# facebookresearch/seamless_communication

Hardware: AMD Instinct MI355X
Metric: S2ST utterances/sec (and real-time factor), seamlessM4T_v2_large, 10 s audio (higher is better)
Workload: dtype f32 activations x f16 weights, f32 accumulate

## Files before the change

include/seamless_hip_internal.h:

```cpp
#ifndef SEAMLESS_HIP_INTERNAL_H_
#define SEAMLESS_HIP_INTERNAL_H_

#include "seamless_hip.h"

#ifdef __cplusplus
extern "C" {
#endif

int sc_decoder_step_family(sc_model* m, int rows, int caller);

int sc_op_knob(const char* name, int dflt);

int sc_op_force_general_gemm(int on);
int sc_op_single_plane(int on);
int sc_op_layernorm(const float* d_x, const float* d_gamma, const float* d_beta, float* d_y, int32_t rows, int32_t C,
                    int32_t act);
int sc_op_linear(const float* d_x, const void* d_w_f16, const float* d_bias, const float* d_res, float* d_y,
                 int32_t M, int32_t N, int32_t K, int32_t act, float alpha, int32_t split, int32_t force_gemv);
int sc_op_skinny_linear(const float* d_x, const void* d_w_f16, const float* d_bias, const float* d_res, float* d_y,
                        int32_t M, int32_t N, int32_t K, int32_t act, float alpha);
int sc_op_skinny_res_ln(const float* d_in, const void* d_w_f16, const float* d_bias, float* d_x_inout,
                        const float* d_gamma, const float* d_beta, float* d_h, int32_t M, int32_t N, int32_t K,
                        int32_t splits);
int sc_op_skinny_argmax(const float* d_x, const void* d_w_f16, int32_t M, int32_t N, int32_t K, int32_t step,
                        int32_t min_step_for_eos, int32_t force_eos_step, int32_t pad_idx, int32_t eos_idx,
                        int32_t unk_idx, float unk_penalty, int32_t* d_idx, float* d_lprob);

int sc_op_dstep_res_ln(const float* d_in, const void* d_w_f16, const float* d_bias, float* d_x_inout, const float* d_gamma,
                       const float* d_beta, float* d_h, int32_t M, int32_t N, int32_t K, int32_t splits);
int sc_op_dstep_linear_planes(const float* d_x, const void* d_w_f16, const float* d_bias, float* d_y, int32_t M, int32_t N, int32_t K,
                              int32_t act);
int sc_op_dstep_argmax(const float* d_x, const void* d_w_f16, int32_t M, int32_t N, int32_t K, int32_t step,
                       int32_t min_step_for_eos, int32_t force_eos_step, int32_t pad_idx, int32_t eos_idx, int32_t unk_idx,
                       float unk_penalty, int32_t ntl, int32_t* d_idx, float* d_lprob);
int sc_op_dstep_attention(const float* d_proj, int32_t S, const float* d_bias, float* d_kcache, float* d_vcache, int32_t cap,
                          int32_t pos, const int32_t* d_lens, int32_t cross, int32_t nb, int32_t heads, float* d_out);
int sc_op_dstep3_gemv(int32_t mode, const float* d_x, const void* d_w_f16, const float* d_bias, const float* d_gamma,
                      const float* d_beta, const float* d_res, float* d_y, float* d_h, int32_t M, int32_t N, int32_t K, int32_t act,
                      int32_t rg, int32_t shape);
int sc_op_dstep3_argmax(const float* d_x, const void* d_w_f16, int32_t M, int32_t N, int32_t K, int32_t step,
                        int32_t min_step_for_eos, int32_t force_eos_step, int32_t pad_idx, int32_t eos_idx, int32_t unk_idx,
                        float unk_penalty, int32_t* d_idx, float* d_lprob);
int sc_op_chain_bench(int32_t kind, int32_t rows, int32_t n, int32_t reps, float* us_per_kernel);
int sc_op_conv1d(const float* d_x, const void* d_w_f16_packed, const float* d_bias, const float* d_res, float* d_y,
                 int32_t nb, int32_t t_in, int32_t cin, int32_t cout, int32_t k, int32_t stride, int32_t pad,
                 int32_t dil, const int32_t* d_in_lens, int32_t in_act, int32_t act);
int sc_op_pack_conv_weight(const void* d_w_f16, void* d_dst_f16, int32_t cout, int32_t cin, int32_t k);
int sc_op_conv_transpose1d(const float* d_x, const void* d_v_f16, const void* d_g_f16, const float* d_bias,
                           float* d_y, int32_t nb, int32_t t_in, int32_t cin, int32_t cout, int32_t k,
                           int32_t stride, int32_t pad, int32_t in_act);
int sc_op_linear_presplit(const float* d_x, const void* d_w_f16, const float* d_bias, const float* d_res, float* d_y,
                          void* d_yh_f16, void* d_yl_f16, int32_t M, int32_t N, int32_t K, int32_t act, float alpha);
int sc_op_linear_presplit_argmax(const float* d_x, const void* d_w_f16, const float* d_bias, int32_t* d_idx, int32_t M, int32_t N,
                                 int32_t K);
int sc_op_conv1d_presplit(const float* d_x, const void* d_w_f16_packed, const float* d_bias, const float* d_res, float* d_y,
                          void* d_yh_f16, void* d_yl_f16, int32_t nb, int32_t t, int32_t cin, int32_t cout, int32_t k, int32_t pad,
                          int32_t dil, const unsigned char* d_row_valid, int32_t act);
int sc_op_resblock_pair_ps(const float* d_x, const void* d_w1_packed, const float* d_b1, const void* d_w2_packed, const float* d_b2,
                           float* d_out, int32_t nb, int32_t T, int32_t C, int32_t k, int32_t dil);
int sc_op_resblock_pair(const float* d_x, const void* d_w1_packed, const float* d_b1, const void* d_w2_packed,
                        const float* d_b2, float* d_out, int32_t nb, int32_t T, int32_t C, int32_t k, int32_t dil,
                        float slope, const float* d_avg_a, const float* d_avg_b);
int sc_op_mrf_fused(const float* d_x, const void* const* d_w1_packed, const float* const* d_b1, const void* const* d_w2_packed,
                    const float* const* d_b2, float* d_out, int32_t nb, int32_t T, int32_t C, const int32_t* k, const int32_t* dil,
                    float slope);
int sc_op_attention(const float* d_q, const float* d_k, const float* d_v, float* d_out, int32_t nb, int32_t heads,
// ... 42 lines not shown
```

seamless_communication_amd/_lib.py:

```python
from __future__ import annotations

import ctypes as C
from pathlib import Path
from typing import Optional

import os

_VARIANT = os.environ.get("SC_LIB_VARIANT", "")
LIB_PATH = Path(__file__).resolve().parent / (f"libseamless_hip.{_VARIANT}.so" if _VARIANT else "libseamless_hip.so")

SC_ABI_VERSION = 10
SC_MAX_UPSAMPLES = 8
SC_MAX_RESBLOCK_KERNELS = 4
SC_MAX_RESBLOCK_DILATIONS = 4
SC_F16, SC_F32, SC_I32 = 0, 1, 2


class SeamlessHipError(RuntimeError):
    pass


class sc_tensor_desc(C.Structure):
    _fields_ = [
        ("name", C.c_char_p),
# ... 65 lines not shown


_P = C.c_void_p
_PI = C.POINTER(C.c_int32)

SIGNATURES = {
    "sc_last_error": (C.c_char_p, []),
    "sc_abi_version": (C.c_int, []),
    "sc_load": (_P, [C.POINTER(sc_tensor_desc), C.c_size_t, C.POINTER(sc_config), C.c_int]),
    "sc_fork": (_P, [_P]),
    "sc_free": (None, [_P]),
    "sc_synchronize": (C.c_int, [_P]),
    "sc_wait_stream": (C.c_int, [_P, _P]),
    "sc_decoder_step_family": (C.c_int, [_P, C.c_int, C.c_int]),
    "sc_set_nar_tables": (C.c_int, [_P, _i, _P, _P, _P, _P, _P]),
    "sc_fbank": (C.c_int, [_P, _P, _i, C.c_int64, _P, _i, _P, _i, _P]),
    "sc_fbank_rate": (C.c_int, [_P, _P, _i, C.c_int64, _P, _i, _i, _P, _i, _P]),
    "sc_fbank_frames": (_i, [C.c_int64, _i]),
    "sc_encoder_out_len": (_i, [_P, _i]),
    "sc_encode_speech": (C.c_int, [_P, _P, _i, _i, _P, _P, _P]),
    "sc_encode_text": (C.c_int, [_P, _P, C.c_int32, C.c_int32, _P, _P]),
    "sc_mma_begin": (C.c_int, [_P, _P, C.c_int32, C.c_int32]),
    "sc_mma_step": (C.c_int, [_P, _P, C.c_int32, _P, C.c_int32, _P, _P, _P]),
    "sc_text_max_len": (_i, [_P, C.POINTER(sc_gen_opts), _i]),
    "sc_generate_text": (C.c_int, [_P, _P, _i, _i, _P, C.POINTER(sc_gen_opts), _P, _i, _P, _P, _P, _P]),
    "sc_generate_text_banned": (C.c_int, [_P, _P, _i, _i, _P, C.POINTER(sc_gen_opts), _P, _i, _P, _P, _P, _P, _P, _P, _i]),
    "sc_generate_text_capture": (C.c_int, [_P, _P, _i, _i, _P, C.POINTER(sc_gen_opts), _P, _i, _P, _P, _P, _P, _P, _P]),
    "sc_decode_text": (C.c_int, [_P, _P, _i, _i, _P, _P, _i, _P]),
    "sc_engine_create": (_P, [_P, C.POINTER(sc_engine_opts)]),
    "sc_engine_free": (None, [_P]),
    "sc_engine_attach": (C.c_int, [_P, _P]),
    "sc_engine_expect": (C.c_int, [_P, _i]),
    "sc_engine_get_stats": (C.c_int, [_P, C.POINTER(sc_engine_stats), _i]),
    "sc_t2u_nar": (C.c_int, [_P, _P, _i, _i, _P, _P, C.c_float, _P, _PI, _PI]),
    "sc_get_units": (C.c_int, [_P, _P]),
    "sc_get_durations": (C.c_int, [_P, _P, _P, _P]),
    "sc_vocoder_hop": (_i, [_P]),
    "sc_vocode": (C.c_int, [_P, _P, _i, _i, _P, _P, _P]),
    "sc_vocode_ragged": (C.c_int, [_P, _P, _i, _i, _P, _P, _P, _P]),
    "sc_vocoder_durations": (C.c_int, [_P, _P, _i, _i, _P]),
    "sc_t2u_ar": (C.c_int, [_P, _P, _i, _i, _P, C.POINTER(sc_gen_opts), _P, _i, _P, _i, _P, _P]),
    "sc_t2u_ar_max_len": (_i, [_P, C.POINTER(sc_gen_opts), _i]),
    "sc_last_padding": (C.c_int, [_P, _P, _P, _P]),
    "sc_s2st": (C.c_int, [_P, _P, _i, _i, _P, C.POINTER(sc_gen_opts), _P, _i, C.c_float, _P, _P, _P, _i, _P, _P, _i, _P, _P, _P]),
    "sc_prof_enable": (C.c_int, [C.c_int]),
    "sc_prof_reset": (C.c_int, []),
    "sc_prof_report": (C.c_int64, [C.c_char_p, C.c_int64]),
    "sc_text_to_char_seqs": (C.c_int32, [C.c_int32, _P, _P, _P, _P, _P, C.c_int32, C.c_int32, C.c_int32, _P, C.c_int32, C.c_int32,
                                         _P, _P, C.c_int32, _P]),
    "sc_ngram_blocked_tokens": (C.c_int32, [_PI, C.c_int32, C.c_int32, _PI, C.c_int32]),
    "sc_banned_blocked_tokens": (C.c_int32, [_PI, C.c_int32, _PI, _PI, C.c_int32, _PI, C.c_int32]),
    "sc_op_knob": (C.c_int, [C.c_char_p, C.c_int]),
    "sc_op_force_general_gemm": (C.c_int, [C.c_int]),
    "sc_op_single_plane": (C.c_int, [C.c_int]),
    "sc_op_layernorm": (C.c_int, [_P, _P, _P, _P, _i, _i, _i]),
    "sc_op_linear": (C.c_int, [_P, _P, _P, _P, _P, _i, _i, _i, _i, C.c_float, _i, _i]),
    "sc_op_skinny_linear": (C.c_int, [_P, _P, _P, _P, _P, _i, _i, _i, _i, C.c_float]),
    "sc_op_skinny_res_ln": (C.c_int, [_P, _P, _P, _P, _P, _P, _P, _i, _i, _i, _i]),
    "sc_op_skinny_argmax": (C.c_int, [_P, _P, _i, _i, _i, _i, _i, _i, _i, _i, _i, C.c_float, _P, _P]),
    "sc_op_dstep_res_ln": (C.c_int, [_P, _P, _P, _P, _P, _P, _P, _i, _i, _i, _i]),
    "sc_op_dstep_linear_planes": (C.c_int, [_P, _P, _P, _P, _i, _i, _i, _i]),
    "sc_op_dstep_argmax": (C.c_int, [_P, _P, _i, _i, _i, _i, _i, _i, _i, _i, _i, C.c_float, _i, _P, _P]),
    "sc_op_resblock_pair_ps": (C.c_int, [_P, _P, _P, _P, _P, _P, _i, _i, _i, _i, _i]),
    "sc_op_glu_dwconv_ln": (C.c_int, [_P, _P, _P, _P, _i, _P, _P, _i, _i, _i, _i, _P, _i]),
    "sc_op_layernorm2": (C.c_int, [_P, _P, _P, _P, _P, _P, _P, _P, _i, _i, _i]),
    "sc_op_dstep3_gemv": (C.c_int, [_i, _P, _P, _P, _P, _P, _P, _P, _P, _i, _i, _i, _i, _i, _i]),
    "sc_op_dstep3_argmax": (C.c_int, [_P, _P, _i, _i, _i, _i, _i, _i, _i, _i, _i, C.c_float, _P, _P]),
    "sc_op_chain_bench": (C.c_int, [_i, _i, _i, _i, _P]),
    "sc_op_dstep_attention": (C.c_int, [_P, _i, _P, _P, _P, _i, _i, _P, _i, _i, _i, _P]),
    "sc_op_conv1d": (C.c_int, [_P, _P, _P, _P, _P, _i, _i, _i, _i, _i, _i, _i, _i, _P, _i, _i]),
    "sc_op_pack_conv_weight": (C.c_int, [_P, _P, _i, _i, _i]),
    "sc_op_conv_transpose1d": (C.c_int, [_P, _P, _P, _P, _P, _i, _i, _i, _i, _i, _i, _i, _i]),
    "sc_op_linear_presplit": (C.c_int, [_P, _P, _P, _P, _P, _P, _P, _i, _i, _i, _i, C.c_float]),
    "sc_op_linear_presplit_argmax": (C.c_int, [_P, _P, _P, _P, _i, _i, _i]),
    "sc_op_conv1d_presplit": (C.c_int, [_P, _P, _P, _P, _P, _P, _P, _i, _i, _i, _i, _i, _i, _i, _P, _i]),
    "sc_op_mrf_fused": (C.c_int, [_P, _P, _P, _P, _P, _P, _i, _i, _i, _P, _P, C.c_float]),
    "sc_op_resblock_pair": (C.c_int, [_P, _P, _P, _P, _P, _P, _i, _i, _i, _i, _i, C.c_float, _P, _P]),
    "sc_op_attention": (C.c_int, [_P, _P, _P, _P, _i, _i, _i, _i, C.c_int64, C.c_int64, C.c_int64, C.c_int64, _P, _i,
                                  _P, _i, _i]),
    "sc_op_attention_ex": (C.c_int, [_P, _P, _P, _P, _i, _i, _i, _i, C.c_int64, C.c_int64, C.c_int64, C.c_int64, _P, _i,
                                     _P, _i, _i, _P, _P, C.c_int64, _P, _P, _P, _P, C.c_int64]),
    "sc_op_glu_dwconv": (C.c_int, [_P, _P, _P, _i, _i, _i, _i, _P]),
    "sc_op_argmax": (C.c_int, [_P, _i, _i, _P, _P]),
    "sc_op_beam_candidates": (C.c_int, [_P, C.c_int64, _i, _i, _i, _P, _i, _i, _i, _i, _i, _i, C.c_float, _i, _P, _P, _P, _i, _i, _i,
                                        _P, _P, _i]),
    "sc_op_beam_candidates_banned": (C.c_int, [_P, C.c_int64, _i, _i, _i, _P, _i, _i, _i, _i, _i, _i, C.c_float, _i, _P, _P, _P, _i, _i,
                                               _i, _P, _P, _i, _P, _P, _i]),
    "sc_op_beam_select": (C.c_int, [_P, _P, _P, _P, _P, _P, _P, _P, _P, _P, _P, _P, _P, _P, _i, _P, _P, _i, _i, _i, _i, _i, _i, _i, _i,
                                    _i, C.c_float]),
    "sc_op_beam_compact": (C.c_int, [_P, _P, _P, _P, _P, _P, _P, _P, _P, _i, _i, _i, _i, _i, _i]),
    "sc_op_gather_cache": (C.c_int, [_P, _P, _P, _i, _i, _i, _i, _i, C.c_int64]),
    "sc_op_row_token_lprob": (C.c_int, [_P, C.c_int64, _i, _i, _i, _i, _P]),
}

_lib: Optional[C.CDLL] = None


def load_library() -> C.CDLL:
    global _lib
    if _lib is not None:
        return _lib
    if not LIB_PATH.exists():
        raise SeamlessHipError(
            f"{LIB_PATH} is missing: build it with `python -m seamless_communication_amd.build` "
            "(there is no CPU fallback for the HIP path)"
        )
# ... 79 lines not shown
```

seamless_communication_amd/csrc/api.hip:

```cpp
#include <atomic>
#include <cstring>
#include <map>
#include <mutex>
#include <set>

#include "../../include/seamless_hip_internal.h"
#include "engine.h"
#include "model.h"

using namespace sc;

struct sc_model {
    Model m;
};

struct sc_engine {
    std::unique_ptr<Engine> e;
    int device = 0;
    const void* weights = nullptr;
    std::set<sc_model*> attached;
};

static std::mutex g_attach_mu;
static std::map<Engine*, sc_engine*> g_engine_owner;
// ... 496 lines not shown
                 "sc_text_to_char_seqs: null argument");
        return text_to_char_seqs_host(vocab, h_tok_len, h_starts_space, h_is_punct, h_char_offsets, h_char_ids, pad_idx, unk_idx,
                                      eos_idx, h_text_seqs, n, s_text, h_char_lens, h_out_char_ids, cap, h_char_seq_lens);
    } catch (const sc::Error& e) {
        return e.code;
    } catch (const std::exception& e) {
        sc::set_error("unexpected C++ exception: %s", e.what());
        return SC_ERR_INTERNAL;
    }
}

int32_t sc_ngram_blocked_tokens(const int32_t* h_seq, int32_t len, int32_t ngram_size, int32_t* h_out, int32_t cap) {
    try {
        SC_CHECK(len >= 0 && ngram_size >= 1 && cap >= 0 && (h_seq || len == 0) && (h_out || cap == 0),
                 "sc_ngram_blocked_tokens: bad argument");
        std::vector<int32_t> out;
        sc::ngram_blocked_tokens(h_seq, len, ngram_size, out);
        for (size_t i = 0; i < out.size() && i < (size_t)cap; ++i) h_out[i] = out[i];
        return (int32_t)out.size();
    } catch (const sc::Error& e) {
        return e.code;
    } catch (const std::exception& e) {
        sc::set_error("unexpected C++ exception: %s", e.what());
        return SC_ERR_INTERNAL;
    }
}

int32_t sc_banned_blocked_tokens(const int32_t* h_seq, int32_t len, const int32_t* h_banned_tokens, const int32_t* h_banned_offsets,
                                 int32_t n_banned, int32_t* h_out, int32_t cap) {
    try {
        SC_CHECK(len >= 0 && cap >= 0 && (h_seq || len == 0) && (h_out || cap == 0), "sc_banned_blocked_tokens: bad argument");
        sc::validate_banned_host(h_banned_tokens, h_banned_offsets, n_banned, -1, nullptr);
        sc::BannedHost b;
        b.tokens = h_banned_tokens, b.offsets = h_banned_offsets, b.n = n_banned;
        std::vector<int32_t> out;
        sc::banned_blocked_tokens(h_seq, len, b, out);
        for (size_t i = 0; i < out.size() && i < (size_t)cap; ++i) h_out[i] = out[i];
        return (int32_t)out.size();
    } catch (const sc::Error& e) {
        return e.code;
    } catch (const std::exception& e) {
        sc::set_error("unexpected C++ exception: %s", e.what());
        return SC_ERR_INTERNAL;
    }
}

int sc_op_knob(const char* name, int dflt) { return sc::knob::known(name) ? sc::knob::value(name, dflt) : dflt; }

static std::atomic<int> g_op_single{0};
int sc_op_single_plane(int on) {
    g_op_single.store(on ? 1 : 0);
    return SC_OK;
}

int sc_op_force_general_gemm(int on) {
    sc::g_force_general_gemm.store(on ? 1 : 0);
    return SC_OK;
}

int sc_op_layernorm(const float* d_x, const float* d_gamma, const float* d_beta, float* d_y, int32_t rows, int32_t C,
                    int32_t act) {
    SC_API_BEGIN
    launch_layernorm(d_x, C, d_gamma, d_beta, d_y, C, rows, C, act, nullptr, 1, g_op_stream);
    SC_HIP(hipStreamSynchronize(g_op_stream));
    SC_API_END
}

int sc_op_linear(const float* d_x, const void* d_w_f16, const float* d_bias, const float* d_res, float* d_y, int32_t M,
                 int32_t N, int32_t K, int32_t act, float alpha, int32_t split, int32_t force_gemv) {
    SC_API_BEGIN
    if (force_gemv) {
        launch_gemv(d_x, K, static_cast<const __half*>(d_w_f16), K, d_bias, d_res, N, d_y, N, M, N, K, act, alpha, g_op_stream);
    } else {
        GemmArgs a;
        a.A = d_x;
        a.lda = K;
        a.W = static_cast<const __half*>(d_w_f16);
        a.ldw = K;
        a.bias = d_bias;
        a.res = d_res;
        a.ldr = N;
        a.C = d_y;
        a.ldc = N;
        a.M = M;
        a.N = N;
        a.K = K;
        a.rows_per_batch = M;
        a.t_in = M;
        a.t_out = M;
        a.taps = 1;
        a.cin = K;
        a.act = act;
        a.alpha = alpha;
        a.split = split;
        launch_gemm(a, g_op_stream);
    }
    SC_HIP(hipStreamSynchronize(g_op_stream));
    SC_API_END
}

int sc_op_skinny_linear(const float* d_x, const void* d_w_f16, const float* d_bias, const float* d_res, float* d_y,
                        int32_t M, int32_t N, int32_t K, int32_t act, float alpha) {
    SC_API_BEGIN
    SkinnyArgs a;
    a.A = d_x;
    a.lda = K;
// ... 919 lines not shown
```

seamless_communication_amd/csrc/common.cpp:

```cpp
#include "common.h"
#include <cstdlib>
#include <cstring>

namespace sc {

static thread_local char g_err[1024] = "";

void set_error(const char* fmt, ...) {
    va_list ap;
    va_start(ap, fmt);
    vsnprintf(g_err, sizeof(g_err), fmt, ap);
    va_end(ap);
}

const char* get_error() { return g_err; }

namespace knob {
namespace {
struct Knob {
    const char* name;
    int kind;
    const char* what;
};
const Knob knob_table[] = {
    {"SC_DEBUG_NUMERICS", 0, "honour the switches that change results"},
    {"SC_DEBUG_FILL", 0, "fill fresh scratch blocks with NaN (tests)"},
    {"SC_SPLIT_MODE", 1, "1: Conformer products on the hi fp16 plane only (precision study)"},
    {"SC_DECODER_GEN1", 1, "decoder step on the first-generation kernels"},
    {"SC_DECODER_GEN2", 1, "decoder step on the second-generation chain"},
    {"SC_DECODE_STEPWISE", 1, "teacher-forced pass step by step instead of one batched forward"},
    {"SC_VOC_SPLIT", 1, "vocoder ResBlock products on both fp16 planes of their activations again (bit 0 wide stages, bit 2 narrow stages); default: hi plane only"},
    {"SC_GEMM_GENERAL", 0, "general GEMM kernel instead of the fast path"}, {"SC_GEMM_PF2", 0, "GEMM prefetch depth"},
    {"SC_GEMM_GROUP_M", 0, "GEMM workgroup order"}, {"SC_GEMM_TILE", 0, "GEMM tile override"},
    {"SC_PS_TILE", 0, "DMA GEMM: largest tile"}, {"SC_PS_MIN256", 0, "DMA GEMM: tiles needed for 256 x 256"},
    {"SC_PS_MIN128", 0, "DMA GEMM: tiles needed for 128 x 128"},
    {"SC_PRESPLIT", 0, "0: Conformer operands split on the fly"}, {"SC_ENC_FUSE", 0, "0: separate Conformer element-wise launches"},
    {"SC_D3_RG_SMALL", 0, "decoder step: rows per row group, N = 1024 products"}, {"SC_D3_RG_FFN", 0, "decoder step: rows per row group, FFN-in"},
    {"SC_G3_STATIONARY", 0, "row-group products of wide steps: 0 one workgroup per row group, n = workgroup budget of the weight-stationary launch"},
    {"SC_G3_TILES", 0, "0: FFN-out of wide steps on the weight-stationary row-group walk instead of tile-owning waves"},
    {"SC_G3_TOUCH", 0, "weight-stationary products: bit 0 cooperative L2 touch of the activations, bit 1 K slices per XCD (FFN-out); default 3"},
    {"SC_D3_FFN_IN", 0, "decoder step: FFN-in workgroup shape"}, {"SC_D3_FFN_OUT", 0, "decoder step: FFN-out workgroup shape"},
    {"SC_T2U_GROUPS", 0, "NAR T2U: length buckets"}, {"SC_T2U_PACKED", 0, "0: NAR decoder on padded buckets"},
    {"SC_VOC_PS", 0, "0: vocoder wide stages on the register-staged convolution"}, {"SC_VOC_MRF", 0, "0: narrow vocoder stages as nine pair launches"},
    {"SC_VOC_GROUPS", 0, "vocoder: length buckets"}, {"SC_VOC_GROUP_OVERHEAD", 0, "vocoder: bucket planning overhead rows"},
    {"SC_VOC_STREAMS", 0, "vocoder: side chains"},
    {"SC_ENGINE_RG_SMALL", 0, "decode engine: rows per row group, N = 1024 products"},
    {"SC_BEAM_COMPACT", 2, "0: beam search keeps finished utterances' slots"},
    {"SC_GREEDY_COMPACT", 2, "0: greedy generation keeps finished rows in their slots"}, {"SC_GREEDY_POLL", 2, "steps between looks at the finished flags"},
};
constexpr int N_KNOBS = sizeof(knob_table) / sizeof(knob_table[0]);
struct State {
    bool set[N_KNOBS];
    int val[N_KNOBS];
    bool numerics = false;
};
const State& state() {
    static const State st = [] {
        State s{};
        const char* dn = getenv("SC_DEBUG_NUMERICS");
        s.numerics = dn && atoi(dn) != 0;
        for (int i = 0; i < N_KNOBS; ++i) {
            const char* e = getenv(knob_table[i].name);
            s.set[i] = e != nullptr && (knob_table[i].kind != 1 || s.numerics);
            s.val[i] = e ? atoi(e) : 0;
        }
        return s;
    }();
    return st;
}
int lookup(const char* name) {
    for (int i = 0; i < N_KNOBS; ++i)
        if (strcmp(knob_table[i].name, name) == 0) return i;
    return -1;
}
int find(const char* name) {
    const int i = lookup(name);
    if (i >= 0) return i;
    fprintf(stderr, "libseamless_hip: switch %s is not in the knob table (common.cpp)\n", name);
    abort();
}
}

bool known(const char* name) { return name && lookup(name) >= 0; }

int value(const char* name, int dflt) {
    const int i = find(name);
    return state().set[i] ? state().val[i] : dflt;
}
bool is_set(const char* name) { return state().set[find(name)]; }
int live(const char* name, int dflt) {
    (void)find(name);
    const char* e = getenv(name);
    return e ? atoi(e) : dflt;
}
void report_once() {
    static const bool done = [] {
        const State& s = state();
        for (int i = 0; i < N_KNOBS; ++i) {
// ... 16 lines not shown
```

seamless_communication_amd/csrc/k_gemm.hip:

```cpp
#include <atomic>
#include <cstdlib>

#include "kernels.h"

namespace sc {

std::atomic<int> g_force_general_gemm{0};

typedef _Float16 half8_t __attribute__((ext_vector_type(8)));
typedef _Float16 half4_t __attribute__((ext_vector_type(4)));
typedef float float16_t __attribute__((ext_vector_type(16)));

static constexpr int BK = 32;
static constexpr int LDS_LD = 40;

__device__ __forceinline__ float apply_act(float v, int act) {
    if (act == ACT_RELU) return v > 0.f ? v : 0.f;
    if (act == ACT_SILU) return v / (1.f + expf(-v));
    if (act == ACT_TANH) return tanhf(v);
    return v;
}

__device__ __forceinline__ float apply_in_act(float v, int in_act) {
    if (in_act == IN_LRELU_01) return v > 0.f ? v : 0.1f * v;
    if (in_act == IN_LRELU_001) return v > 0.f ? v : 0.01f * v;
    return v;
}

template <int BM, int BN, int WGM, int WGN, int AMODE, bool SPLIT>
__global__ __launch_bounds__(256) void gemm_kernel(GemmArgs p) {
    static_assert(WGM * WGN == 4, "4 waves per block");
    constexpr int WM = BM / WGM, WN = BN / WGN;
    constexpr int TM = WM / 32, TN = WN / 32;
    static_assert(TM >= 1 && TN >= 1, "wave tile must hold a 32x32 fragment");
    constexpr int A_IT = BM / 32;
    constexpr int B_IT = (BN * 4 + 255) / 256;

    __shared__ __attribute__((aligned(16))) _Float16 sAh[BM * LDS_LD];
    __shared__ __attribute__((aligned(16))) _Float16 sAl[SPLIT ? BM * LDS_LD : 8];
    __shared__ __attribute__((aligned(16))) _Float16 sB[BN * LDS_LD];

    const int tid = threadIdx.x;
    const int lane = tid & 63;
    const int wave = tid >> 6;
    const int wm = wave / WGN, wn = wave % WGN;
    const int m0 = blockIdx.y * BM;
    const int n0 = blockIdx.x * BN;
    const int phase = blockIdx.z;
    const __half* __restrict__ W = p.W + (int64_t)phase * p.w_phase_stride;
    const int out_off = p.out_off + phase * p.out_off_phase_step;

    const int a_kq = tid & 7;
    const int a_r = tid >> 3;
    int a_n[A_IT], a_q[A_IT], a_len[A_IT];
#pragma unroll
    for (int i = 0; i < A_IT; ++i) {
        const int m = m0 + a_r + 32 * i;
        if (m < p.M) {
            const int n = m / p.rows_per_batch;
            a_n[i] = n;
            a_q[i] = m - n * p.rows_per_batch;
            a_len[i] = p.in_lens ? min(p.in_lens[n], p.t_in) : p.t_in;
        } else {
            a_n[i] = 0;
            a_q[i] = 0;
            a_len[i] = -1;
        }
    }
    const int b_r = tid >> 2;
    const int b_kc = tid & 3;

    float4 a_reg[A_IT];
    uint4 b_reg[B_IT];

    auto load_tile = [&](int k0) {
        if (AMODE == 1) {
            const int tap = k0 / p.cin;
            const int c0 = k0 - tap * p.cin + a_kq * 4;
            const bool tap_ok = tap < p.taps;
#pragma unroll
            for (int i = 0; i < A_IT; ++i) {
                const int src_t = a_q[i] * p.stride + tap * p.dil - p.pad;
                float4 v = make_float4(0.f, 0.f, 0.f, 0.f);
                if (tap_ok && src_t >= 0 && src_t < a_len[i]) {
                    v = *reinterpret_cast<const float4*>(
                        p.A + ((int64_t)a_n[i] * p.t_in + src_t) * p.lda + c0);
                }
                a_reg[i] = v;
            }
        } else if (AMODE == 2) {
            const int kk = k0 + a_kq * 4;
            const int tap = kk / p.cin;
            const int c0 = kk - tap * p.cin;
            const bool tap_ok = tap < p.taps;
#pragma unroll
            for (int i = 0; i < A_IT; ++i) {
                const int src_t = a_q[i] * p.stride + tap * p.dil - p.pad;
                float4 v = make_float4(0.f, 0.f, 0.f, 0.f);
                if (tap_ok && src_t >= 0 && src_t < a_len[i]) {
                    v = *reinterpret_cast<const float4*>(
                        p.A + ((int64_t)a_n[i] * p.t_in + src_t) * p.lda + c0);
                }
                a_reg[i] = v;
            }
        } else {
#pragma unroll
            for (int i = 0; i < A_IT; ++i) {
                float e[4];
#pragma unroll
                for (int j = 0; j < 4; ++j) {
                    const int kk = k0 + a_kq * 4 + j;
                    const int tap = kk / p.cin;
                    const int c = kk - tap * p.cin;
                    const int src_t = a_q[i] * p.stride + tap * p.dil - p.pad;
                    float v = 0.f;
                    if (tap < p.taps && src_t >= 0 && src_t < a_len[i]) {
                        v = p.A[((int64_t)a_n[i] * p.t_in + src_t) * p.lda + c];
                    }
                    e[j] = v;
                }
                a_reg[i] = make_float4(e[0], e[1], e[2], e[3]);
            }
        }
#pragma unroll
        for (int i = 0; i < B_IT; ++i) {
            const int row = b_r + 64 * i;
            uint4 v = make_uint4(0u, 0u, 0u, 0u);
            if (row < BN && n0 + row < p.N) {
                v = *reinterpret_cast<const uint4*>(W + (int64_t)(n0 + row) * p.ldw + k0 + b_kc * 8);
            }
            b_reg[i] = v;
        }
    };

    auto store_tile = [&]() {
#pragma unroll
        for (int i = 0; i < A_IT; ++i) {
            float x[4] = {a_reg[i].x, a_reg[i].y, a_reg[i].z, a_reg[i].w};
            half4_t hi, lo;
#pragma unroll
            for (int j = 0; j < 4; ++j) {
                const float v = apply_in_act(x[j], p.in_act);
                const _Float16 h = (_Float16)v;
                hi[j] = h;
                lo[j] = (_Float16)(v - (float)h);
            }
            const int off = (a_r + 32 * i) * LDS_LD + a_kq * 4;
            *reinterpret_cast<half4_t*>(&sAh[off]) = hi;
            if (SPLIT) *reinterpret_cast<half4_t*>(&sAl[off]) = lo;
        }
#pragma unroll
        for (int i = 0; i < B_IT; ++i) {
            const int row = b_r + 64 * i;
            if (row < BN) *reinterpret_cast<uint4*>(&sB[row * LDS_LD + b_kc * 8]) = b_reg[i];
        }
    };

    float16_t acc[TM][TN];
#pragma unroll
    for (int i = 0; i < TM; ++i)
#pragma unroll
        for (int j = 0; j < TN; ++j)
#pragma unroll
            for (int r = 0; r < 16; ++r) acc[i][j][r] = 0.f;

    const int frag_row = lane & 31;
    const int frag_k = (lane >> 5) * 8;

    load_tile(0);
    for (int k0 = 0; k0 < p.K; k0 += BK) {
        store_tile();
        __syncthreads();
        if (k0 + BK < p.K) load_tile(k0 + BK);
#pragma unroll
        for (int kb = 0; kb < BK; kb += 16) {
            half8_t ah[TM], al[TM], bf[TN];
#pragma unroll
            for (int i = 0; i < TM; ++i) {
                const int off = (wm * WM + i * 32 + frag_row) * LDS_LD + kb + frag_k;
                ah[i] = *reinterpret_cast<const half8_t*>(&sAh[off]);
                if (SPLIT) al[i] = *reinterpret_cast<const half8_t*>(&sAl[off]);
            }
#pragma unroll
            for (int j = 0; j < TN; ++j) {
                const int off = (wn * WN + j * 32 + frag_row) * LDS_LD + kb + frag_k;
                bf[j] = *reinterpret_cast<const half8_t*>(&sB[off]);
            }
#pragma unroll
            for (int i = 0; i < TM; ++i)
#pragma unroll
                for (int j = 0; j < TN; ++j) {
                    acc[i][j] = __builtin_amdgcn_mfma_f32_32x32x16_f16(ah[i], bf[j], acc[i][j], 0, 0, 0);
                    if (SPLIT)
                        acc[i][j] = __builtin_amdgcn_mfma_f32_32x32x16_f16(al[i], bf[j], acc[i][j], 0, 0, 0);
                }
        }
        __syncthreads();
    }

    const bool plain_rows = (p.rows_per_batch == p.M) && p.out_mul == 1 && out_off == 0 && p.t_out == p.M;
#pragma unroll
    for (int i = 0; i < TM; ++i) {
#pragma unroll
        for (int r = 0; r < 16; ++r) {
            const int m = m0 + wm * WM + i * 32 + (r & 3) + 8 * (r >> 2) + 4 * (lane >> 5);
            if (m >= p.M) continue;
            int64_t row;
            if (plain_rows) {
                row = m;
            } else {
                const int n = m / p.rows_per_batch;
                const int q = m - n * p.rows_per_batch;
                const int dst_t = q * p.out_mul + out_off;
                if (dst_t < 0 || dst_t >= p.t_out) continue;
                row = (int64_t)n * p.t_out + dst_t;
            }
#pragma unroll
            for (int j = 0; j < TN; ++j) {
                const int col = n0 + wn * WN + j * 32 + (lane & 31);
                if (col >= p.N) continue;
                float v = acc[i][j][r];
                if (p.bias) v += p.bias[col];
                v = apply_act(v, p.act) * p.alpha;
                if (p.res) v += p.res[row * p.ldr + col];
                p.C[row * p.ldc + col] = v;
            }
        }
    }
}

template <int BM, int BN, int WGM, int WGN>
static void launch_cfg(const GemmArgs& a, hipStream_t s) {
    dim3 grid(cdiv(a.N, BN), cdiv(a.M, BM), a.phases);
    const bool vec_ok = (a.lda % 4 == 0) && ((reinterpret_cast<uintptr_t>(a.A) & 15) == 0);
    const int amode = (vec_ok && a.cin % 32 == 0) ? 1 : (vec_ok && a.cin % 4 == 0) ? 2 : 0;
    char name[64];
    snprintf(name, sizeof(name), "gemm_%dx%d_%s_%s", BM, BN, amode == 1 ? "vecA" : amode == 2 ? "vec4A" : "genA",
             a.split ? "split" : "f16");
    const double kreal = (double)a.taps * a.cin;
    const double flops = a.algo_flops > 0 ? a.algo_flops : 2.0 * a.M * a.N * kreal * a.phases;
    const double bytes = 4.0 * a.M * (double)a.cin * (a.stride < a.taps ? 1.0 : (double)a.taps) +
                         2.0 * a.N * (double)a.K * a.phases + 4.0 * a.M * (double)a.N * (a.res ? 2.0 : 1.0);
    prof::Scope scope(name, flops, bytes, s);
#define SC_GEMM_LAUNCH(AM, SP) hipLaunchKernelGGL((gemm_kernel<BM, BN, WGM, WGN, AM, SP>), grid, dim3(256), 0, s, a)
    if (a.split) {
        if (amode == 1) SC_GEMM_LAUNCH(1, true);
        else if (amode == 2) SC_GEMM_LAUNCH(2, true);
        else SC_GEMM_LAUNCH(0, true);
    } else {
        if (amode == 1) SC_GEMM_LAUNCH(1, false);
        else if (amode == 2) SC_GEMM_LAUNCH(2, false);
        else SC_GEMM_LAUNCH(0, false);
    }
#undef SC_GEMM_LAUNCH
}

void launch_gemm(const GemmArgs& a, hipStream_t s) {
    SC_CHECK(a.K % BK == 0, "gemm: K=%d must be a multiple of %d", a.K, BK);
    SC_CHECK(a.ldw % 8 == 0, "gemm: ldw=%lld must be a multiple of 8", (long long)a.ldw);
    SC_CHECK(a.M > 0 && a.N > 0, "gemm: empty problem M=%d N=%d", a.M, a.N);
    SC_CHECK(a.rows_per_batch > 0 && a.cin > 0, "gemm: rows_per_batch/cin unset");
    static const bool env_general = knob::is_set("SC_GEMM_GENERAL");
// ... 99 lines not shown
```

seamless_communication_amd/csrc/k_gemm2.hip:

```cpp
#include <algorithm>
#include <cstdlib>

#include "kernels.h"

namespace sc {

typedef _Float16 half8_t __attribute__((ext_vector_type(8)));
typedef _Float16 half4_t __attribute__((ext_vector_type(4)));
typedef float float16_t __attribute__((ext_vector_type(16)));
typedef float f32x4_t __attribute__((ext_vector_type(4)));
typedef unsigned int u32x4_t __attribute__((ext_vector_type(4)));

namespace {

constexpr int GEMM_GROUP_M_DEFAULT = 1;
constexpr int GEMM_PF2_DEFAULT = 1;
constexpr int FBK = 32;
constexpr int FLD = 40;

template <int ACT>
__device__ __forceinline__ float act_fn(float v) {
    if (ACT == ACT_RELU) return v > 0.f ? v : 0.f;
    if (ACT == ACT_SILU) return v / (1.f + expf(-v));
    if (ACT == ACT_TANH) return tanhf(v);
    return v;
}

template <int TM, int TN, int WM, int WN, int ACT, bool HAS_RES>
__device__ __forceinline__ void epilogue(const GemmArgs& p, float16_t (&acc)[TM][TN], int m0w, int n0w, int lane,
                                         int out_off, bool plain_rows) {
    float bcol[TN];
    int col[TN];
#pragma unroll
    for (int j = 0; j < TN; ++j) {
        col[j] = n0w + j * 32 + (lane & 31);
        bcol[j] = (p.bias && col[j] < p.N) ? p.bias[col[j]] : 0.f;
    }
#pragma unroll
    for (int i = 0; i < TM; ++i) {
#pragma unroll
        for (int r = 0; r < 16; ++r) {
            const int m = m0w + i * 32 + (r & 3) + 8 * (r >> 2) + 4 * (lane >> 5);
            if (m >= p.M) continue;
            int64_t row;
            if (plain_rows) {
                row = m;
            } else {
                const int n = m / p.rows_per_batch;
                const int q = m - n * p.rows_per_batch;
                const int dst_t = q * p.out_mul + out_off;
                if (dst_t < 0 || dst_t >= p.t_out) continue;
                row = (int64_t)n * p.t_out + dst_t;
            }
#pragma unroll
            for (int j = 0; j < TN; ++j) {
                if (col[j] >= p.N) continue;
                float v = act_fn<ACT>(acc[i][j][r] + bcol[j]) * p.alpha;
                if (HAS_RES) v += p.res[row * p.ldr + col[j]];
                p.C[row * p.ldc + col[j]] = v;
            }
        }
    }
}

template <int TM, int TN, int WN, int EP_LD, int ACT, bool HAS_RES>
__device__ __forceinline__ void epilogue_lds(const GemmArgs& p, float16_t (&acc)[TM][TN], float* ep, int m0w, int n0w, int lane,
                                             int out_off, bool plain_rows) {
    constexpr int LPR = WN / 4;
    constexpr int RPG = 16 / LPR;
    constexpr int RPI = 4 * RPG;
    const int l5 = lane & 31;
    const bool g1 = (l5 >= 4 && l5 < 12) || (l5 >= 16 && l5 < 20) || l5 >= 28;
    const int rank = g1 ? (l5 < 12 ? l5 - 4 : l5 < 20 ? l5 - 8 : l5 - 16) : (l5 < 4 ? l5 : l5 < 16 ? l5 - 8 : l5 - 12);
    const int grp = (lane >> 5) * 2 + (g1 ? 1 : 0);
    const int row_in = grp * RPG + rank / LPR;
    const int c0 = (rank % LPR) * 4;
    const int col = n0w + c0;
    const bool vec_ok = (col + 3 < p.N) && (p.ldc % 4 == 0) && (!HAS_RES || p.ldr % 4 == 0) &&
                        ((reinterpret_cast<uintptr_t>(p.C) | (HAS_RES ? reinterpret_cast<uintptr_t>(p.res) : 0)) & 15) == 0;
    f32x4_t b4 = {0.f, 0.f, 0.f, 0.f};
    if (p.bias) {
#pragma unroll
        for (int e = 0; e < 4; ++e) b4[e] = (col + e < p.N) ? p.bias[col + e] : 0.f;
    }
#pragma unroll
    for (int i = 0; i < TM; ++i) {
#pragma unroll
        for (int j = 0; j < TN; ++j)
#pragma unroll
            for (int r = 0; r < 16; ++r) ep[((r & 3) + 8 * (r >> 2) + 4 * (lane >> 5)) * EP_LD + j * 32 + (lane & 31)] = acc[i][j][r];
#pragma unroll
        for (int it = 0; it < 32 / RPI; ++it) {
            const int rr = it * RPI + row_in;
            const int m = m0w + i * 32 + rr;
            const f32x4_t a = *reinterpret_cast<const f32x4_t*>(ep + rr * EP_LD + c0);
            if (m >= p.M || col >= p.N) continue;
            int64_t row;
            if (plain_rows) {
                row = m;
            } else {
                const int n = m / p.rows_per_batch;
                const int q = m - n * p.rows_per_batch;
                const int dst_t = q * p.out_mul + out_off;
                if (dst_t < 0 || dst_t >= p.t_out) continue;
                row = (int64_t)n * p.t_out + dst_t;
            }
            f32x4_t v;
#pragma unroll
            for (int e = 0; e < 4; ++e) v[e] = act_fn<ACT>(a[e] + b4[e]) * p.alpha;
            if (vec_ok) {
                if (HAS_RES) v += *reinterpret_cast<const f32x4_t*>(p.res + row * p.ldr + col);
                *reinterpret_cast<f32x4_t*>(p.C + row * p.ldc + col) = v;
            } else {
#pragma unroll
                for (int e = 0; e < 4; ++e) {
                    if (col + e >= p.N) continue;
                    float x = v[e];
                    if (HAS_RES) x += p.res[row * p.ldr + col + e];
                    p.C[row * p.ldc + col + e] = x;
                }
            }
        }
    }
}

template <int BM, int BN, int WGM, int WGN, bool IN_ACT, bool CONV>
__global__ __launch_bounds__(256) void gemm_fast_kernel(GemmArgs p, int tiles_n, int tiles_mn, int tiles_total,
                                                        int tiles_per_xcd, float in_slope, int group_m) {
    static_assert(WGM * WGN == 4, "4 waves per block");
    constexpr int WM = BM / WGM, WN = BN / WGN;
    constexpr int TM = WM / 32, TN = WN / 32;
    static_assert(TM >= 1 && TN >= 1, "wave tile must hold a 32x32 fragment");
    constexpr int A_IT = BM / 32;
    constexpr int B_IT = (BN * 4 + 255) / 256;

    __shared__ __attribute__((aligned(16))) _Float16 sAh[2][BM * FLD];
    __shared__ __attribute__((aligned(16))) _Float16 sAl[2][BM * FLD];
    __shared__ __attribute__((aligned(16))) _Float16 sB[2][BN * FLD];

    const int bid = blockIdx.x;
    const int tile = (bid & 7) * tiles_per_xcd + (bid >> 3);
    if (tile >= tiles_total) return;
    const int phase = tile / tiles_mn;
    const int rem = tile - phase * tiles_mn;
    int tm, tn;
    {
        const int per_group = group_m * tiles_n;
        const int g = rem / per_group;
        const int in_g = rem - g * per_group;
        const int tiles_m = tiles_mn / tiles_n;
        const int gm = min(group_m, tiles_m - g * group_m);
        tn = in_g / gm;
        tm = g * group_m + (in_g - tn * gm);
    }

    const int tid = threadIdx.x;
    const int lane = tid & 63;
    const int wave = tid >> 6;
    const int wm = wave / WGN, wn = wave % WGN;
    const int m0 = tm * BM;
    const int n0 = tn * BN;
    const __half* __restrict__ W = p.W + (int64_t)phase * p.w_phase_stride;
    const int out_off = p.out_off + phase * p.out_off_phase_step;

    const int a_kq = tid & 7;
    const int a_r = tid >> 3;
    const float* a_base[A_IT];
    int a_t0[A_IT], a_len[A_IT];
#pragma unroll
    for (int i = 0; i < A_IT; ++i) {
        const int m = m0 + a_r + 32 * i;
        if (m < p.M) {
            const int n = m / p.rows_per_batch;
            const int q = m - n * p.rows_per_batch;
            a_base[i] = p.A + (int64_t)n * p.t_in * p.lda + a_kq * 4;
            a_t0[i] = q * p.stride - p.pad;
            a_len[i] = p.in_lens ? min(p.in_lens[n], p.t_in) : p.t_in;
        } else {
            a_base[i] = p.A + a_kq * 4;
            a_t0[i] = 0;
            a_len[i] = 0;
        }
    }
    const int b_r = tid >> 2;
    const int b_kc = tid & 3;
    const __half* b_ptr[B_IT];
#pragma unroll
    for (int i = 0; i < B_IT; ++i) {
        const int row = min(n0 + b_r + 64 * i, p.N - 1);
        b_ptr[i] = W + (int64_t)row * p.ldw + b_kc * 8;
    }

    const float* a_ptr[A_IT];
    bool a_ok[A_IT];
    auto set_tap = [&](int tap) {
#pragma unroll
        for (int i = 0; i < A_IT; ++i) {
            const int src_t = a_t0[i] + tap * p.dil;
            a_ok[i] = src_t >= 0 && src_t < a_len[i];
            a_ptr[i] = a_base[i] + (int64_t)(a_ok[i] ? src_t : 0) * p.lda;
        }
    };

    f32x4_t a_reg[A_IT];
    u32x4_t b_reg[B_IT];
    constexpr bool B_GUARD = (BN % 64) != 0;

    float16_t acc[TM][TN];
#pragma unroll
    for (int i = 0; i < TM; ++i)
#pragma unroll
        for (int j = 0; j < TN; ++j)
#pragma unroll
            for (int r = 0; r < 16; ++r) acc[i][j][r] = 0.f;

    const int frag_row = lane & 31;
    const int frag_k = (lane >> 5) * 8;
    const int a_frag = (wm * WM + frag_row) * FLD + frag_k;
    const int b_frag = (wn * WN + frag_row) * FLD + frag_k;

#define SC_LOAD_SLAB(C0, K0)                                                                    \
    do {                                                                                        \
        _Pragma("unroll") for (int i = 0; i < A_IT; ++i)                                        \
            a_reg[i] = *reinterpret_cast<const f32x4_t*>(a_ptr[i] + (C0));                       \
        _Pragma("unroll") for (int i = 0; i < B_IT; ++i)                                        \
// ... 18 lines not shown
        }                                                                                       \
        _Pragma("unroll") for (int i = 0; i < B_IT; ++i) {                                      \
            const int row = b_r + 64 * i;                                                       \
            if (!B_GUARD || row < BN) *reinterpret_cast<u32x4_t*>(&sB[ST][row * FLD + b_kc * 8]) = b_reg[i]; \
        }                                                                                       \
    } while (0)

#define SC_COMPUTE_SLAB(ST)                                                                     \
    do {                                                                                        \
        _Pragma("unroll") for (int kb = 0; kb < FBK; kb += 16) {                                \
            half8_t ah[TM], al[TM], bf[TN];                                                     \
            _Pragma("unroll") for (int i = 0; i < TM; ++i) {                                    \
                ah[i] = *reinterpret_cast<const half8_t*>(&sAh[ST][a_frag + i * 32 * FLD + kb]); \
                al[i] = *reinterpret_cast<const half8_t*>(&sAl[ST][a_frag + i * 32 * FLD + kb]); \
            }                                                                                   \
            _Pragma("unroll") for (int j = 0; j < TN; ++j)                                      \
                bf[j] = *reinterpret_cast<const half8_t*>(&sB[ST][b_frag + j * 32 * FLD + kb]); \
            _Pragma("unroll") for (int i = 0; i < TM; ++i)                                      \
                _Pragma("unroll") for (int j = 0; j < TN; ++j) {                                \
                    acc[i][j] = __builtin_amdgcn_mfma_f32_32x32x16_f16(ah[i], bf[j], acc[i][j], 0, 0, 0); \
                    acc[i][j] = __builtin_amdgcn_mfma_f32_32x32x16_f16(al[i], bf[j], acc[i][j], 0, 0, 0); \
                }                                                                               \
        }                                                                                       \
    } while (0)

    const int nslab = p.K / FBK;
    const int slabs_per_tap = p.cin / FBK;
    int tap = 0, cs = 0;
    set_tap(0);
    SC_LOAD_SLAB(0, 0);
    SC_STORE_SLAB(0);
    __syncthreads();
    for (int s = 0; s + 1 < nslab; ++s) {
        const int st = s & 1;
        if (++cs == slabs_per_tap) {
            cs = 0;
            set_tap(++tap);
        }
        SC_LOAD_SLAB(cs * FBK, (s + 1) * FBK);
        __builtin_amdgcn_sched_barrier(0);
        SC_COMPUTE_SLAB(st);
        __builtin_amdgcn_sched_barrier(0);
        SC_STORE_SLAB(st ^ 1);
        __syncthreads();
    }
    {
        const int st = (nslab - 1) & 1;
        SC_COMPUTE_SLAB(st);
    }
#undef SC_LOAD_SLAB
#undef SC_STORE_SLAB
#undef SC_COMPUTE_SLAB

    const bool plain_rows = (p.rows_per_batch == p.M) && p.out_mul == 1 && out_off == 0 && p.t_out == p.M;
    const int m0w = m0 + wm * WM, n0w = n0 + wn * WN;
#define SC_EPI(ACT)                                                                               \
    do {                                                                                          \
        if (p.res) epilogue<TM, TN, WM, WN, ACT, true>(p, acc, m0w, n0w, lane, out_off, plain_rows); \
        else epilogue<TM, TN, WM, WN, ACT, false>(p, acc, m0w, n0w, lane, out_off, plain_rows);    \
    } while (0)
    if (p.act == ACT_NONE) SC_EPI(ACT_NONE);
    else if (p.act == ACT_RELU) SC_EPI(ACT_RELU);
    else if (p.act == ACT_SILU) SC_EPI(ACT_SILU);
    else SC_EPI(ACT_TANH);
#undef SC_EPI
}

__device__ __forceinline__ __amdgpu_buffer_rsrc_t make_rsrc(const void* base, uint32_t bytes) {
    return __builtin_amdgcn_make_buffer_rsrc(const_cast<void*>(base), 0, bytes, 0x00020000);
}

template <int BM, int BN, int WGM, int WGN, bool IN_ACT>
__global__ __launch_bounds__(256) void gemm_fast2_kernel(GemmArgs p, int tiles_n, int tiles_mn, int tiles_total,
                                                         int tiles_per_xcd, float in_slope, uint32_t a_bytes, uint32_t w_bytes) {
    static_assert(WGM * WGN == 4, "4 waves per block");
    constexpr int WM = BM / WGM, WN = BN / WGN;
    constexpr int TM = WM / 32, TN = WN / 32;
    constexpr int A_IT = BM / 32;
    constexpr int B_IT = (BN * 4 + 255) / 256;
    constexpr uint32_t OOB = 0x80000000u;

    constexpr int EP_LD = WN + 4;
    static_assert(4 * 32 * EP_LD * 4 <= (4 * BM + 2 * BN) * FLD * 2, "epilogue tiles must fit in the stage memory");
    __shared__ __attribute__((aligned(16))) _Float16 smem_all[(4 * BM + 2 * BN) * FLD];
    _Float16(*sAh)[BM * FLD] = reinterpret_cast<_Float16(*)[BM * FLD]>(smem_all);
    _Float16(*sAl)[BM * FLD] = reinterpret_cast<_Float16(*)[BM * FLD]>(smem_all + 2 * BM * FLD);
    _Float16(*sB)[BN * FLD] = reinterpret_cast<_Float16(*)[BN * FLD]>(smem_all + 4 * BM * FLD);

    const int bid = blockIdx.x;
    const int tile = (bid & 7) * tiles_per_xcd + (bid >> 3);
    if (tile >= tiles_total) return;
    const int phase = tile / tiles_mn;
    const int rem = tile - phase * tiles_mn;
    const int tm = rem / tiles_n;
    const int tn = rem - tm * tiles_n;

    const int tid = threadIdx.x;
    const int lane = tid & 63;
    const int wave = tid >> 6;
    const int wm = wave / WGN, wn = wave % WGN;
    const int m0 = tm * BM;
    const int n0 = tn * BN;
    const int out_off = p.out_off + phase * p.out_off_phase_step;
    const __amdgpu_buffer_rsrc_t ra = make_rsrc(p.A, a_bytes);
    const __amdgpu_buffer_rsrc_t rb = make_rsrc(p.W + (int64_t)phase * p.w_phase_stride, w_bytes);

    const int a_kq = tid & 7;
    const int a_r = tid >> 3;
    int a_row0[A_IT], a_t0[A_IT], a_len[A_IT];
#pragma unroll
    for (int i = 0; i < A_IT; ++i) {
        const int m = m0 + a_r + 32 * i;
        if (m < p.M) {
            const int n = m / p.rows_per_batch;
            const int q = m - n * p.rows_per_batch;
            a_row0[i] = n * p.t_in;
            a_t0[i] = q * p.stride - p.pad;
            a_len[i] = p.in_lens ? min(p.in_lens[n], p.t_in) : p.t_in;
        } else {
            a_row0[i] = 0;
            a_t0[i] = 0;
            a_len[i] = 0;
        }
    }
    const int b_r = tid >> 2;
    const int b_kc = tid & 3;
    uint32_t b_voff[B_IT];
#pragma unroll
    for (int i = 0; i < B_IT; ++i) {
        const int row = n0 + b_r + 64 * i;
        b_voff[i] = row < p.N ? (uint32_t)(((int64_t)row * p.ldw + b_kc * 8) * 2) : OOB;
    }
    uint32_t a_voff[A_IT];
    auto set_tap = [&](int tap) {
#pragma unroll
        for (int i = 0; i < A_IT; ++i) {
            const int src_t = a_t0[i] + tap * p.dil;
            const bool ok = src_t >= 0 && src_t < a_len[i];
            a_voff[i] = ok ? (uint32_t)((((int64_t)a_row0[i] + src_t) * p.lda + a_kq * 4) * 4) : OOB;
        }
    };

    f32x4_t a_reg0[A_IT], a_reg1[A_IT];
    u32x4_t b_reg0[B_IT], b_reg1[B_IT];
    constexpr bool B_GUARD = (BN % 64) != 0;

    float16_t acc[TM][TN];
#pragma unroll
    for (int i = 0; i < TM; ++i)
#pragma unroll
        for (int j = 0; j < TN; ++j)
#pragma unroll
            for (int r = 0; r < 16; ++r) acc[i][j][r] = 0.f;

    const int frag_row = lane & 31;
    const int frag_k = (lane >> 5) * 8;
    const int a_frag = (wm * WM + frag_row) * FLD + frag_k;
    const int b_frag = (wn * WN + frag_row) * FLD + frag_k;

#define SC2_LOAD(AR, BR, ASOFF, BSOFF, KILL)                                                                  \
    do {                                                                                                      \
        _Pragma("unroll") for (int i = 0; i < A_IT; ++i)                                                      \
            AR[i] = __builtin_bit_cast(f32x4_t, __builtin_amdgcn_raw_buffer_load_b128(ra, a_voff[i] | (KILL), (ASOFF), 0)); \
        _Pragma("unroll") for (int i = 0; i < B_IT; ++i)                                                      \
            BR[i] = __builtin_amdgcn_raw_buffer_load_b128(rb, b_voff[i] | (KILL), (BSOFF), 0);                \
    } while (0)
// ... 25 lines not shown
            half8_t ah[TM], al[TM], bf[TN];                                                     \
            _Pragma("unroll") for (int i = 0; i < TM; ++i) {                                    \
                ah[i] = *reinterpret_cast<const half8_t*>(&sAh[ST][a_frag + i * 32 * FLD + kb]); \
                al[i] = *reinterpret_cast<const half8_t*>(&sAl[ST][a_frag + i * 32 * FLD + kb]); \
            }                                                                                   \
            _Pragma("unroll") for (int j = 0; j < TN; ++j)                                      \
                bf[j] = *reinterpret_cast<const half8_t*>(&sB[ST][b_frag + j * 32 * FLD + kb]); \
            _Pragma("unroll") for (int i = 0; i < TM; ++i)                                      \
                _Pragma("unroll") for (int j = 0; j < TN; ++j) {                                \
                    acc[i][j] = __builtin_amdgcn_mfma_f32_32x32x16_f16(ah[i], bf[j], acc[i][j], 0, 0, 0); \
                    acc[i][j] = __builtin_amdgcn_mfma_f32_32x32x16_f16(al[i], bf[j], acc[i][j], 0, 0, 0); \
                }                                                                               \
        }                                                                                       \
    } while (0)

    const int nslab = p.K / FBK;
    const int slabs_per_tap = p.cin / FBK;
    int tap = 0, cs = 0;
#define SC2_ADVANCE()                \
    do {                             \
        if (++cs == slabs_per_tap) { \
            cs = 0;                  \
            set_tap(++tap);          \
        }                            \
    } while (0)
#define SC2_STEP(S, AFREE, BFREE, ANEXT, BNEXT)                                   \
    do {                                                                          \
        const bool more2 = (S) + 2 < nslab;                                       \
        if (more2) SC2_ADVANCE();                                                 \
        SC2_LOAD(AFREE, BFREE, cs * (FBK * 4), more2 ? ((S) + 2) * (FBK * 2) : 0, more2 ? 0u : OOB); \
        __builtin_amdgcn_sched_barrier(0);                                        \
        SC2_COMPUTE((S) & 1);                                                     \
        __builtin_amdgcn_sched_barrier(0);                                        \
        if ((S) + 1 < nslab) SC2_STORE(ANEXT, BNEXT, ((S) + 1) & 1);              \
        __syncthreads();                                                          \
    } while (0)

    set_tap(0);
    SC2_LOAD(a_reg0, b_reg0, 0, 0, 0u);
    SC2_STORE(a_reg0, b_reg0, 0);
    SC2_ADVANCE();
    SC2_LOAD(a_reg1, b_reg1, cs * (FBK * 4), FBK * 2, 0u);
    __syncthreads();
    for (int s = 0; s < nslab; s += 2) {
        SC2_STEP(s, a_reg0, b_reg0, a_reg1, b_reg1);
        SC2_STEP(s + 1, a_reg1, b_reg1, a_reg0, b_reg0);
    }
#undef SC2_STEP
#undef SC2_ADVANCE
#undef SC2_LOAD
#undef SC2_STORE
#undef SC2_COMPUTE

    const bool plain_rows = (p.rows_per_batch == p.M) && p.out_mul == 1 && out_off == 0 && p.t_out == p.M;
    const int m0w = m0 + wm * WM, n0w = n0 + wn * WN;
    float* ep = reinterpret_cast<float*>(smem_all) + wave * (32 * EP_LD);
#define SC_EPI(ACT)                                                                                             \
    do {                                                                                                        \
        if (p.res) epilogue_lds<TM, TN, WN, EP_LD, ACT, true>(p, acc, ep, m0w, n0w, lane, out_off, plain_rows);  \
        else epilogue_lds<TM, TN, WN, EP_LD, ACT, false>(p, acc, ep, m0w, n0w, lane, out_off, plain_rows);       \
    } while (0)
    if (p.act == ACT_NONE) SC_EPI(ACT_NONE);
    else if (p.act == ACT_RELU) SC_EPI(ACT_RELU);
    else if (p.act == ACT_SILU) SC_EPI(ACT_SILU);
    else SC_EPI(ACT_TANH);
#undef SC_EPI
}

template <int BM, int BN, int WGM, int WGN>
void launch_fast_cfg(const GemmArgs& a, hipStream_t s) {
    const int tiles_m = cdiv(a.M, BM), tiles_n = cdiv(a.N, BN);
    const int tiles_mn = tiles_m * tiles_n;
    const int64_t total64 = (int64_t)tiles_mn * a.phases;
    SC_CHECK(total64 < (1ll << 30), "gemm: %lld tiles", (long long)total64);
    const int tiles_total = (int)total64;
    const int tiles_per_xcd = cdiv(tiles_total, 8);
    char name[64];
    snprintf(name, sizeof(name), "gemm_%dx%d_fast_split", BM, BN);
    const double kreal = (double)a.taps * a.cin;
    const double flops = a.algo_flops > 0 ? a.algo_flops : 2.0 * a.M * a.N * kreal * a.phases;
    const double bytes = 4.0 * a.M * (double)a.cin * (a.stride < a.taps ? 1.0 : (double)a.taps) +
                         2.0 * a.N * (double)a.K * a.phases + 4.0 * a.M * (double)a.N * (a.res ? 2.0 : 1.0);
    prof::Scope scope(name, flops, bytes, s);
    const dim3 grid(tiles_per_xcd * 8);
    static const int env_pf2 = knob::value("SC_GEMM_PF2", GEMM_PF2_DEFAULT);
    const int64_t a_bytes64 = (int64_t)(a.M / a.rows_per_batch) * a.t_in * a.lda * 4;
    const int64_t w_bytes64 = (int64_t)a.N * a.ldw * 2;
    if (env_pf2 && a.K % (2 * FBK) == 0 && a.M % a.rows_per_batch == 0 && a_bytes64 < (1ll << 31) && w_bytes64 < (1ll << 31)) {
        const float slope = a.in_act == IN_LRELU_01 ? 0.1f : a.in_act == IN_LRELU_001 ? 0.01f : 0.f;
        if (a.in_act == IN_NONE)
            hipLaunchKernelGGL((gemm_fast2_kernel<BM, BN, WGM, WGN, false>), grid, dim3(256), 0, s, a, tiles_n, tiles_mn,
                               tiles_total, tiles_per_xcd, slope, (uint32_t)a_bytes64, (uint32_t)w_bytes64);
        else
            hipLaunchKernelGGL((gemm_fast2_kernel<BM, BN, WGM, WGN, true>), grid, dim3(256), 0, s, a, tiles_n, tiles_mn,
                               tiles_total, tiles_per_xcd, slope, (uint32_t)a_bytes64, (uint32_t)w_bytes64);
        return;
    }
    static const int env_gm = knob::value("SC_GEMM_GROUP_M", 0);
    const int group_m = std::max(1, std::min(env_gm > 0 ? env_gm : GEMM_GROUP_M_DEFAULT, tiles_m));
    const bool conv = a.taps != 1 || a.stride != 1 || a.pad != 0 || a.in_lens != nullptr;
    if (a.in_act == IN_NONE) {
        if (conv)
            hipLaunchKernelGGL((gemm_fast_kernel<BM, BN, WGM, WGN, false, true>), grid, dim3(256), 0, s, a, tiles_n,
                               tiles_mn, tiles_total, tiles_per_xcd, 0.f, group_m);
        else
            hipLaunchKernelGGL((gemm_fast_kernel<BM, BN, WGM, WGN, false, false>), grid, dim3(256), 0, s, a, tiles_n,
                               tiles_mn, tiles_total, tiles_per_xcd, 0.f, group_m);
    } else {
        const float slope = a.in_act == IN_LRELU_01 ? 0.1f : 0.01f;
        hipLaunchKernelGGL((gemm_fast_kernel<BM, BN, WGM, WGN, true, true>), grid, dim3(256), 0, s, a, tiles_n, tiles_mn,
                           tiles_total, tiles_per_xcd, slope, group_m);
    }
}

}

bool gemm_fast_eligible(const GemmArgs& a) {
    return a.split == 1 && a.cin % FBK == 0 && a.K == a.taps * a.cin && a.lda % 4 == 0 &&
           (reinterpret_cast<uintptr_t>(a.A) & 15) == 0 && a.ldw % 8 == 0 && a.M > 32 &&
           a.N > 32 &&
           (a.in_act == IN_NONE || a.in_act == IN_LRELU_01 || a.in_act == IN_LRELU_001);
}

void launch_gemm_fast(const GemmArgs& a, hipStream_t s) {
    const int64_t tiles128 = (int64_t)cdiv(a.M, 128) * cdiv(a.N, 128) * a.phases;
    if (a.N <= 32) {
        if ((int64_t)cdiv(a.M, 256) * a.phases >= 512) launch_fast_cfg<256, 32, 4, 1>(a, s);
        else launch_fast_cfg<128, 32, 4, 1>(a, s);
    } else if (a.N <= 64) {
        if ((int64_t)cdiv(a.M, 128) * a.phases >= 512) launch_fast_cfg<128, 64, 2, 2>(a, s);
        else launch_fast_cfg<64, 64, 2, 2>(a, s);
    } else if (tiles128 >= 256) {
        static const int env_tile = knob::value("SC_GEMM_TILE", 0);
        if (env_tile == 1) launch_fast_cfg<128, 64, 2, 2>(a, s);
        else if (env_tile == 2) launch_fast_cfg<64, 64, 2, 2>(a, s);
        else launch_fast_cfg<128, 128, 2, 2>(a, s);
    } else {
        launch_fast_cfg<64, 64, 2, 2>(a, s);
    }
    SC_LAUNCH_CHECK();
}
// ... 3 lines not shown
```

seamless_communication_amd/csrc/k_misc.hip:

```cpp
#include "kernels.h"

namespace sc {

__global__ __launch_bounds__(256) void embed_tokens_kernel(const int* __restrict__ tokens, int rows,
                                                           const __half* __restrict__ emb, int M,
                                                           float scale, const float* __restrict__ pos_table,
                                                           const int* __restrict__ d_pos, int t_per_batch,
                                                           float* __restrict__ out, int64_t ldo) {
    const int row = blockIdx.x;
    const int tok = tokens[row];
    const int pos = (d_pos ? *d_pos : 0) + (t_per_batch > 0 ? row % t_per_batch : 0);
    const __half* e = emb + (int64_t)tok * M;
    const float* pe = pos_table + (int64_t)pos * M;
    for (int c = threadIdx.x; c < M; c += 256) out[(int64_t)row * ldo + c] = __half2float(e[c]) * scale + pe[c];
}

void launch_embed_tokens(const int* tokens, int rows, const __half* emb, int M, float scale,
                         const float* pos_table, const int* d_pos, int t_per_batch, float* out, int64_t ldo,
                         hipStream_t s) {
    if (rows <= 0) return;
    hipLaunchKernelGGL(embed_tokens_kernel, dim3(rows), dim3(256), 0, s, tokens, rows, emb, M, scale, pos_table,
                       d_pos, t_per_batch, out, ldo);
    SC_LAUNCH_CHECK();
}
// ... 290 lines not shown
void launch_pos_add_rows(float* seqs, int64_t ld, const float* pos_table, const int* row_t, float alpha, int rows, int M, hipStream_t s) {
    if (rows <= 0) return;
    hipLaunchKernelGGL(pos_add_rows_kernel, dim3(rows), dim3(256), 0, s, seqs, ld, pos_table, row_t, alpha, M);
    SC_LAUNCH_CHECK();
}
void launch_pos_add(float* seqs, int64_t ld, const float* pos_table, int t_per_batch, float alpha, int rows, int M,
                    hipStream_t s) {
    if (rows <= 0) return;
    hipLaunchKernelGGL(pos_add_kernel, dim3(rows), dim3(256), 0, s, seqs, ld, pos_table, t_per_batch, alpha, M);
    SC_LAUNCH_CHECK();
}

__global__ __launch_bounds__(256) void durations_kernel(const float* __restrict__ h, int64_t ld,
                                                        const float* __restrict__ w, const float* __restrict__ b,
                                                        int rows, int H, int t_per_batch,
                                                        const int* __restrict__ lens, float duration_factor,
                                                        int min_dur, int* __restrict__ durations) {
    const int lane = threadIdx.x & 63;
    const int row = blockIdx.x * 4 + (threadIdx.x >> 6);
    if (row >= rows) return;
    const float* hr = h + (int64_t)row * ld;
    float acc = 0.f;
    for (int c = lane; c < H; c += 64) acc = fmaf(hr[c], w[c], acc);
#pragma unroll
    for (int o = 32; o > 0; o >>= 1) acc += __shfl_xor(acc, o);
    if (lane == 0) {
        const int n = row / t_per_batch, t = row - n * t_per_batch;
        int d = 0;
        if (!lens || t < lens[n]) {
            const float x = acc + b[0];
            const float r = rintf((expf(x) - 1.0f) * duration_factor);
            long long dl = (long long)r;
            if (dl < (long long)min_dur) dl = min_dur;
            if (dl > 1000000) dl = 1000000;
            d = (int)dl;
        }
        durations[row] = d;
    }
}
void launch_durations(const float* h, int64_t ld, const float* w, const float* b, int rows, int H, int t_per_batch,
                      const int* lens, float duration_factor, int min_dur, int* durations, hipStream_t s) {
    if (rows <= 0) return;
    hipLaunchKernelGGL(durations_kernel, dim3(cdiv(rows, 4)), dim3(256), 0, s, h, ld, w, b, rows, H, t_per_batch, lens,
                       duration_factor, min_dur, durations);
    SC_LAUNCH_CHECK();
}

__global__ __launch_bounds__(256) void vocoder_embed_kernel(const int* __restrict__ units, int T,
                                                            const __half* __restrict__ dict, int E,
                                                            const __half* __restrict__ lang, int Lg,
                                                            const int* __restrict__ lang_idx,
                                                            const __half* __restrict__ spkr, int Sp,
                                                            const int* __restrict__ spkr_idx,
                                                            float* __restrict__ out) {
    const int row = blockIdx.x;
    const int n = row / T;
    const int C = Lg + E + Sp;
    const __half* l = lang + (int64_t)lang_idx[n] * Lg;
    const __half* d = dict + (int64_t)units[row] * E;
    const __half* sp = spkr + (int64_t)spkr_idx[n] * Sp;
    float* o = out + (int64_t)row * C;
    for (int c = threadIdx.x; c < C; c += 256) {
        __half v;
        if (c < Lg) v = l[c];
        else if (c < Lg + E) v = d[c - Lg];
        else v = sp[c - Lg - E];
        o[c] = __half2float(v);
    }
}
void launch_vocoder_embed(const int* units, int nb, int T, const __half* dict, int E, const __half* lang, int Lg,
                          const int* lang_idx, const __half* spkr, int Sp, const int* spkr_idx, float* out,
                          hipStream_t s) {
    if (nb * T <= 0) return;
    hipLaunchKernelGGL(vocoder_embed_kernel, dim3(nb * T), dim3(256), 0, s, units, T, dict, E, lang, Lg, lang_idx, spkr,
                       Sp, spkr_idx, out);
    SC_LAUNCH_CHECK();
}

__global__ void avg3_kernel(const float* __restrict__ a, const float* __restrict__ b, const float* __restrict__ c,
                            float* __restrict__ out, int64_t n) {
    for (int64_t i = (int64_t)blockIdx.x * blockDim.x + threadIdx.x; i < n; i += (int64_t)gridDim.x * blockDim.x)
        out[i] = ((a[i] + b[i]) + c[i]) / 3.0f;
}
__global__ void split_f32_kernel(const float* __restrict__ x, __half* __restrict__ hi, __half* __restrict__ lo, int64_t n4) {
    typedef _Float16 h4_t __attribute__((ext_vector_type(4)));
    typedef float f4_t __attribute__((ext_vector_type(4)));
    for (int64_t i = (int64_t)blockIdx.x * blockDim.x + threadIdx.x; i < n4; i += (int64_t)gridDim.x * blockDim.x) {
        const f4_t v = reinterpret_cast<const f4_t*>(x)[i];
        const h4_t h = __builtin_convertvector(v, h4_t);
        reinterpret_cast<h4_t*>(hi)[i] = h;
        reinterpret_cast<h4_t*>(lo)[i] = __builtin_convertvector(v - __builtin_convertvector(h, f4_t), h4_t);
    }
}
void launch_split_f32(const float* x, __half* hi, __half* lo, int64_t n, hipStream_t s) {
    SC_CHECK(n % 4 == 0, "split_f32: n must be a multiple of 4");
    if (n <= 0) return;
    hipLaunchKernelGGL(split_f32_kernel, dim3(grid_for(n / 4)), dim3(256), 0, s, x, hi, lo, n / 4);
    SC_LAUNCH_CHECK();
}

__global__ void lrelu_split_f32_kernel(const float* __restrict__ x, float neg_slope, __half* __restrict__ hi, __half* __restrict__ lo,
                                       int64_t n4) {
    typedef _Float16 h4_t __attribute__((ext_vector_type(4)));
    typedef float f4_t __attribute__((ext_vector_type(4)));
    for (int64_t i = (int64_t)blockIdx.x * blockDim.x + threadIdx.x; i < n4; i += (int64_t)gridDim.x * blockDim.x) {
        f4_t v = reinterpret_cast<const f4_t*>(x)[i];
#pragma unroll
        for (int e = 0; e < 4; ++e) v[e] = fmaxf(v[e], 0.f) + neg_slope * fminf(v[e], 0.f);
        const h4_t h = __builtin_convertvector(v, h4_t);
        reinterpret_cast<h4_t*>(hi)[i] = h;
        if (lo) reinterpret_cast<h4_t*>(lo)[i] = __builtin_convertvector(v - __builtin_convertvector(h, f4_t), h4_t);
    }
}
void launch_lrelu_split_f32(const float* x, float neg_slope, __half* hi, __half* lo, int64_t n, hipStream_t s) {
    SC_CHECK(n % 4 == 0, "lrelu_split_f32: n must be a multiple of 4");
    if (n <= 0) return;
    hipLaunchKernelGGL(lrelu_split_f32_kernel, dim3(grid_for(n / 4)), dim3(256), 0, s, x, neg_slope, hi, lo, n / 4);
    SC_LAUNCH_CHECK();
}

void launch_avg3(const float* a, const float* b, const float* c, float* out, int64_t n, hipStream_t s) {
    if (n <= 0) return;
    hipLaunchKernelGGL(avg3_kernel, dim3(grid_for(n)), dim3(256), 0, s, a, b, c, out, n);
    SC_LAUNCH_CHECK();
}

template <int C, int K>
__global__ __launch_bounds__(256) void conv_to_mono_kernel(const float* __restrict__ x, const __half* __restrict__ w, const float* __restrict__ bias,
                                                           float slope, int act, float* __restrict__ y, int T) {
    constexpr int RS = C + 4, ROWS = 256 + K - 1, VPR = C / 4;
    typedef float f4_t __attribute__((ext_vector_type(4)));
    __shared__ __attribute__((aligned(16))) float tile[ROWS * RS];
    __shared__ __attribute__((aligned(16))) float sw[K * C];
    const int tid = threadIdx.x, n = blockIdx.y;
    const int t0 = blockIdx.x * 256;
    const float* __restrict__ xn = x + (int64_t)n * T * C;
    for (int i = tid; i < ROWS * VPR; i += 256) {
        const int r = i / VPR, c4 = i - r * VPR;
        const int t = t0 - K / 2 + r;
        f4_t v = {0.f, 0.f, 0.f, 0.f};
        if (t >= 0 && t < T) v = *reinterpret_cast<const f4_t*>(xn + (int64_t)t * C + c4 * 4);
#pragma unroll
        for (int j = 0; j < 4; ++j) v[j] = v[j] > 0.f ? v[j] : slope * v[j];
        *reinterpret_cast<f4_t*>(tile + r * RS + c4 * 4) = v;
    }
    for (int i = tid; i < K * C; i += 256) sw[i] = __half2float(w[i]);
    __syncthreads();
    const int t = t0 + tid;
    if (t >= T) return;
    float acc = 0.f;
#pragma unroll
    for (int tap = 0; tap < K; ++tap)
#pragma unroll
        for (int c4 = 0; c4 < VPR; ++c4) {
            const f4_t xv = *reinterpret_cast<const f4_t*>(tile + (tid + tap) * RS + c4 * 4);
            const f4_t wv = *reinterpret_cast<const f4_t*>(sw + tap * C + c4 * 4);
#pragma unroll
            for (int j = 0; j < 4; ++j) acc = fmaf(xv[j], wv[j], acc);
        }
    acc += bias ? bias[0] : 0.f;
    y[(int64_t)n * T + t] = act == ACT_TANH ? tanhf(acc) : acc;
}

bool conv_to_mono_supported(int cin, int cout, int k, int stride, int pad, int dil, int act) {
    return cout == 1 && cin == 16 && k == 7 && stride == 1 && dil == 1 && 2 * pad == k - 1 && (act == ACT_NONE || act == ACT_TANH);
}

void launch_conv_to_mono(const float* x, const __half* w_packed, const float* bias, int nb, int T, int cin, int k, float in_slope, int act,
                         float* y, hipStream_t s) {
    SC_CHECK(conv_to_mono_supported(cin, 1, k, 1, (k - 1) / 2, 1, act), "conv_to_mono: unsupported cin=%d k=%d act=%d", cin, k, act);
    if (nb <= 0 || T <= 0) return;
    prof::Scope scope("conv_to_mono", 2.0 * nb * (double)T * cin * k, 4.0 * nb * (double)T * (cin + 1), s);
    hipLaunchKernelGGL((conv_to_mono_kernel<16, 7>), dim3(cdiv(T, 256), nb), dim3(256), 0, s, x, w_packed, bias, in_slope, act, y, T);
    SC_LAUNCH_CHECK();
}

__global__ void fill_i32_kernel(int* p, int v, int n) {
    for (int i = blockIdx.x * blockDim.x + threadIdx.x; i < n; i += gridDim.x * blockDim.x) p[i] = v;
}
void launch_fill_i32(int* p, int v, int n, hipStream_t s) {
    if (n <= 0) return;
    hipLaunchKernelGGL(fill_i32_kernel, dim3(grid_for(n)), dim3(256), 0, s, p, v, n);
    SC_LAUNCH_CHECK();
}
__global__ void add_i32_kernel(int* p, int v) { *p += v; }
void launch_add_i32(int* p, int v, hipStream_t s) {
    hipLaunchKernelGGL(add_i32_kernel, dim3(1), dim3(1), 0, s, p, v);
    SC_LAUNCH_CHECK();
}

__global__ void step_update_kernel(int* __restrict__ next_tok, int* __restrict__ hist, int hist_ld,
                                   int* __restrict__ finished, int* __restrict__ out_len,
                                   const float* __restrict__ lprob, float* __restrict__ score, int nb,
                                   const int* __restrict__ d_pos, int pad_idx, int eos_idx,
                                   int* __restrict__ n_unfinished) {
    const int pos = *d_pos;
    int unfinished = 0;
    for (int b = threadIdx.x; b < nb; b += blockDim.x) {
        int tok = next_tok[b];
        if (finished[b]) {
            tok = pad_idx;
        } else {
            if (score) score[b] += lprob[b];
            if (tok == eos_idx) {
                finished[b] = 1;
                out_len[b] = pos + 2;
            } else {
                unfinished = 1;
            }
        }
        next_tok[b] = tok;
        hist[(int64_t)b * hist_ld + pos + 1] = tok;
    }
    if (unfinished && n_unfinished) atomicOr(n_unfinished, 1);
}
void launch_step_update(int* next_tok, int* hist, int hist_ld, int* finished, int* out_len, const float* lprob,
                        float* score, int nb, const int* d_pos, int pad_idx, int eos_idx, int* n_unfinished,
                        hipStream_t s) {
    hipLaunchKernelGGL(step_update_kernel, dim3(1), dim3(256), 0, s, next_tok, hist, hist_ld, finished, out_len, lprob,
                       score, nb, d_pos, pad_idx, eos_idx, n_unfinished);
    SC_LAUNCH_CHECK();
}

__global__ __launch_bounds__(256) void row_swap_kernel(RowSwapArgs a) {
    const int i = blockIdx.x, j = blockIdx.y;
    const int src = a.src[i], dst = a.dst[i];
// ... 50 lines not shown
```

seamless_communication_amd/csrc/k_resblock.hip:

```cpp
#include <algorithm>

#include "kernels.h"

namespace sc {

typedef _Float16 half8_t __attribute__((ext_vector_type(8)));
typedef _Float16 half4_t __attribute__((ext_vector_type(4)));
typedef float float16_t __attribute__((ext_vector_type(16)));
typedef float f32x4_t __attribute__((ext_vector_type(4)));

namespace {

constexpr int RB_M1 = 128;

__device__ __forceinline__ float lrelu(float v, float slope) { return v > 0.f ? v : slope * v; }

template <int C, int NF>
__device__ __forceinline__ void conv_from_lds(const _Float16* __restrict__ ah_plane, const _Float16* __restrict__ al_plane,
                                              int a_row0, int tap_step, int k, const __half* __restrict__ W, int64_t ldw,
                                              int lane, float16_t (&acc)[NF]) {
    constexpr int CS = C + 8;
    constexpr int CPT = C / 16;
    const int koff = (lane >> 5) * 8;
    const int a_base = (a_row0 + (lane & 31)) * CS + koff;
// ... 61 lines not shown
#pragma unroll
            for (int nf = 0; nf < NF; ++nf) {
                const half8_t b = wok[nf] ? *reinterpret_cast<const half8_t*>(sW + w_base[nf] + (t * CPT + cc) * 16) : zero8;
                acc[nf] = __builtin_amdgcn_mfma_f32_32x32x16_f16(ah, b, acc[nf], 0, 0, 0);
                if (!SINGLE) acc[nf] = __builtin_amdgcn_mfma_f32_32x32x16_f16(al, b, acc[nf], 0, 0, 0);
            }
        }
    }
}

template <int C>
__device__ __forceinline__ void stage_weights(const __half* __restrict__ W, int64_t ldw, int k0, int width, _Float16* sW, int ldb,
                                              int tid) {
    const int vpr = width >> 3;
    for (int i = tid; i < C * vpr; i += 256) {
        const int col = i / vpr, v = i - col * vpr;
        *reinterpret_cast<half8_t*>(sW + col * ldb + v * 8) = *reinterpret_cast<const half8_t*>(W + (int64_t)col * ldw + k0 + v * 8);
    }
}

template <int C>
struct TapRegs {
    static constexpr int N = (C * (C / 8) + 255) / 256;
    half8_t v[N];
};
template <int C>
__device__ __forceinline__ void tap_load(const __half* __restrict__ W, int64_t ldw, int k0, int tid, TapRegs<C>& r) {
    constexpr int VPR = C / 8;
#pragma unroll
    for (int j = 0; j < TapRegs<C>::N; ++j) {
        const int i = tid + 256 * j;
        const int col = i / VPR, v = i - col * VPR;
        if (i < C * VPR) r.v[j] = *reinterpret_cast<const half8_t*>(W + (int64_t)col * ldw + k0 + v * 8);
    }
}
template <int C>
__device__ __forceinline__ void tap_store(const TapRegs<C>& r, _Float16* sW, int ldb, int tid) {
    constexpr int VPR = C / 8;
#pragma unroll
    for (int j = 0; j < TapRegs<C>::N; ++j) {
        const int i = tid + 256 * j;
        const int col = i / VPR, v = i - col * VPR;
        if (i < C * VPR) *reinterpret_cast<half8_t*>(sW + col * ldb + v * 8) = r.v[j];
    }
}

template <int C, bool SINGLE = false>
__global__ __launch_bounds__(256) void resblock_pair_kernel(ResPairArgs p, int tiles) {
    constexpr int CS = C + 8;
    constexpr int NF = (C + 31) / 32;
    constexpr int VPR = C / 4;
    extern __shared__ __attribute__((aligned(16))) unsigned char rb_smem[];

    const int k = p.k, dil = p.dil, T = p.T;
    const int H2 = (k - 1) / 2, H1 = dil * (k - 1) / 2;
    const int TT = RB_M1 - 2 * H2;
    const int R0 = RB_M1 + 2 * H1;
    _Float16* xh = reinterpret_cast<_Float16*>(rb_smem);
    _Float16* xl = SINGLE ? xh : xh + R0 * CS;
    _Float16* th = xh;
    _Float16* tl = xl;
    constexpr bool PER_TAP = C > 32;
    _Float16* sW = SINGLE ? xh + max(R0 * CS, RB_M1 * (C + 4) * 2) : xl + R0 * CS;
    const int ldb = (PER_TAP ? C : k * C) + 8;

    const int tid = threadIdx.x, lane = tid & 63, wave = tid >> 6;
    const int n = blockIdx.x / tiles;
    const int t0 = (blockIdx.x - n * tiles) * TT;
    const float* __restrict__ xn = p.x + (int64_t)n * T * C;
    const float slope = p.slope;

    for (int i = tid; i < R0 * VPR; i += 256) {
        const int r = i / VPR, c4 = i - r * VPR;
        const int t = t0 - H2 - H1 + r;
        f32x4_t v = {0.f, 0.f, 0.f, 0.f};
        if (t >= 0 && t < T) v = *reinterpret_cast<const f32x4_t*>(xn + (int64_t)t * C + c4 * 4);
#pragma unroll
        for (int j = 0; j < 4; ++j) v[j] = lrelu(v[j], slope);
        const half4_t hi = __builtin_convertvector(v, half4_t);
        *reinterpret_cast<half4_t*>(xh + r * CS + c4 * 4) = hi;
        if (!SINGLE) {
            const f32x4_t back = __builtin_convertvector(hi, f32x4_t);
            const half4_t lo = __builtin_convertvector(v - back, half4_t);
            *reinterpret_cast<half4_t*>(xl + r * CS + c4 * 4) = lo;
        }
    }
    if (PER_TAP) stage_weights<C>(p.w1, p.ldw1, 0, C, sW, ldb, tid);
    else stage_weights<C>(p.w1, p.ldw1, 0, k * C, sW, ldb, tid);
    __syncthreads();

    {
        float16_t acc[NF];
#pragma unroll
        for (int nf = 0; nf < NF; ++nf)
#pragma unroll
            for (int r = 0; r < 16; ++r) acc[nf][r] = 0.f;
        if (PER_TAP) {
            TapRegs<C> wr;
            for (int t = 0; t < k; ++t) {
                if (t + 1 < k) tap_load<C>(p.w1, p.ldw1, (t + 1) * C, tid, wr);
                conv_from_lds_w<C, NF, SINGLE>(xh, xl, 32 * wave, dil, t, 1, sW + (t & 1) * C * ldb, ldb, lane, acc);
                if (t + 1 < k) tap_store<C>(wr, sW + ((t + 1) & 1) * C * ldb, ldb, tid);
                __syncthreads();
            }
        } else {
            conv_from_lds_w<C, NF, SINGLE>(xh, xl, 32 * wave, dil, 0, k, sW, ldb, lane, acc);
            __syncthreads();
        }
        if (PER_TAP) stage_weights<C>(p.w2, p.ldw2, 0, C, sW, ldb, tid);
        else stage_weights<C>(p.w2, p.ldw2, 0, k * C, sW, ldb, tid);
#pragma unroll
        for (int nf = 0; nf < NF; ++nf) {
            const int col = nf * 32 + (lane & 31);
            if (col >= C) continue;
            const float b = p.b1 ? p.b1[col] : 0.f;
#pragma unroll
            for (int r = 0; r < 16; ++r) {
                const int j = 32 * wave + (r & 3) + 8 * (r >> 2) + 4 * (lane >> 5);
                const int t = t0 - H2 + j;
                float v = (t >= 0 && t < T) ? (acc[nf][r] + b) * 1.0f : 0.f;
                v = lrelu(v, slope);
                const _Float16 h = (_Float16)v;
                th[j * CS + col] = h;
                if (!SINGLE) tl[j * CS + col] = (_Float16)(v - (float)h);
            }
        }
    }
    __syncthreads();

    {
        float16_t acc[NF];
#pragma unroll
        for (int nf = 0; nf < NF; ++nf)
#pragma unroll
            for (int r = 0; r < 16; ++r) acc[nf][r] = 0.f;
        if (PER_TAP) {
            TapRegs<C> wr;
            for (int t = 0; t < k; ++t) {
                if (t + 1 < k) tap_load<C>(p.w2, p.ldw2, (t + 1) * C, tid, wr);
                conv_from_lds_w<C, NF, SINGLE>(th, tl, 32 * wave, 1, t, 1, sW + (t & 1) * C * ldb, ldb, lane, acc);
                if (t + 1 < k) {
                    tap_store<C>(wr, sW + ((t + 1) & 1) * C * ldb, ldb, tid);
                    __syncthreads();
                }
            }
        } else {
            conv_from_lds_w<C, NF, SINGLE>(th, tl, 32 * wave, 1, 0, k, sW, ldb, lane, acc);
        }
        __syncthreads();
        constexpr int EPS = C + 4;
        float* ep = reinterpret_cast<float*>(rb_smem);
#pragma unroll
        for (int nf = 0; nf < NF; ++nf) {
            const int col = nf * 32 + (lane & 31);
            if (col >= C) continue;
            const float b = p.b2 ? p.b2[col] : 0.f;
#pragma unroll
            for (int r = 0; r < 16; ++r) {
                const int i = 32 * wave + (r & 3) + 8 * (r >> 2) + 4 * (lane >> 5);
                ep[i * EPS + col] = (acc[nf][r] + b) * 1.0f;
            }
        }
        __syncthreads();
        float* __restrict__ outn = p.out + (int64_t)n * T * C;
        for (int idx = tid; idx < TT * VPR; idx += 256) {
            const int i = idx / VPR, c4 = idx - i * VPR;
            const int t = t0 + i;
            if (t >= T) continue;
            const int64_t off = (int64_t)t * C + c4 * 4;
            f32x4_t v = *reinterpret_cast<const f32x4_t*>(ep + i * EPS + c4 * 4) + *reinterpret_cast<const f32x4_t*>(xn + off);
            if (p.avg_a) {
                const int64_t g = (int64_t)n * T * C + off;
                v = ((*reinterpret_cast<const f32x4_t*>(p.avg_a + g) + *reinterpret_cast<const f32x4_t*>(p.avg_b + g)) + v) / 3.0f;
            }
            *reinterpret_cast<f32x4_t*>(outn + off) = v;
        }
    }
}


constexpr int MRF_R = 512;
constexpr int MRF_G = 32;
constexpr int MRF_THREADS = 1024;
constexpr int MRF_KMAX = 11;

typedef int mrf_i32x4_t __attribute__((ext_vector_type(4)));
#define MRF_LDS_PTR(p) ((__attribute__((address_space(3))) void*)(p))

template <int C>
__device__ __forceinline__ void mrf_w_dma(const __half* __restrict__ W, int64_t ldw, int k, _Float16* sW, int lane, int wave) {
    constexpr int NI = (C * (MRF_KMAX * C / 8 + 1) + 64 * (MRF_THREADS / 64) - 1) / (64 * (MRF_THREADS / 64));
    const int vpr1 = k * C / 8 + 1;
    const int slots = C * vpr1;
    const uint64_t base = reinterpret_cast<uint64_t>(W);
    mrf_i32x4_t rsrc;
    rsrc[0] = __builtin_amdgcn_readfirstlane((int)(uint32_t)base);
    rsrc[1] = __builtin_amdgcn_readfirstlane((int)(uint32_t)((base >> 32) & 0xffff));
    rsrc[2] = __builtin_amdgcn_readfirstlane((int)(uint32_t)(C * ldw * 2));
    rsrc[3] = 0x00020000;
#pragma unroll
    for (int i = 0; i < NI; ++i) {
        const int chunk = i * (MRF_THREADS / 64) + wave;
        if (chunk * 64 < slots) {
            const int P = chunk * 64 + lane;
            const int row = P / vpr1, seg = P - row * vpr1;
            const uint32_t voff = (row < C && seg < vpr1 - 1) ? (uint32_t)((row * ldw + seg * 8) * 2) : 0x80000000u;
            asm volatile("s_mov_b32 m0, %0\n\tbuffer_load_dwordx4 %1, %2, 0 offen lds"
                         :
                         : "s"(__builtin_amdgcn_readfirstlane((int)(uint32_t)(uintptr_t)MRF_LDS_PTR(sW + chunk * 512))), "v"(voff), "s"(rsrc)
                         : "memory");
        }
    }
}

template <int C, bool SINGLE = false>
__device__ __forceinline__ void mrf_conv(const _Float16* __restrict__ ph, const _Float16* __restrict__ pl, int a_row0, int tap_step, int k,
                                         const _Float16* __restrict__ sW, int ldb, int lane, float16_t& acc) {
    constexpr int CS = C + 8;
    constexpr int CPT = C / 16;
    const int koff = (lane >> 5) * 8;
    const int a_base = (a_row0 + (lane & 31)) * CS + koff;
    const int a_step = tap_step * CS;
    const int b_base = ((lane & 31) % C) * ldb + koff;
    const int nch = k * CPT;
    half8_t h0, l0 = {0, 0, 0, 0, 0, 0, 0, 0}, b0, h1, l1 = l0, b1;
#define MRF_LD(CH, H, L, B)                                                              \
    do {                                                                                 \
        const int ao_ = a_base + ((CH) / CPT) * a_step + ((CH) % CPT) * 16;              \
        H = *reinterpret_cast<const half8_t*>(ph + ao_);                                 \
        if (!SINGLE) L = *reinterpret_cast<const half8_t*>(pl + ao_);                    \
        B = *reinterpret_cast<const half8_t*>(sW + b_base + (CH) * 16);                  \
    } while (0)
    MRF_LD(0, h0, l0, b0);
    for (int ch = 0; ch < nch; ++ch) {
        if (ch + 1 < nch) MRF_LD(ch + 1, h1, l1, b1);
        acc = __builtin_amdgcn_mfma_f32_32x32x16_f16(h0, b0, acc, 0, 0, 0);
        if (!SINGLE) acc = __builtin_amdgcn_mfma_f32_32x32x16_f16(l0, b0, acc, 0, 0, 0);
        h0 = h1, l0 = l1, b0 = b1;
    }
#undef MRF_LD
}

template <bool SINGLE = false>
__device__ __forceinline__ void mrf_put(_Float16* __restrict__ ph, _Float16* __restrict__ pl, int idx, float v, float slope) {
    v = fmaxf(v, slope * v);
    const _Float16 h = (_Float16)v;
    ph[idx] = h;
    if (!SINGLE) pl[idx] = (_Float16)(v - (float)h);
}

template <int C, bool EDGE, bool SINGLE>
__device__ __forceinline__ void mrf_tile(const MrfArgs& p, _Float16* __restrict__ ph, _Float16* __restrict__ pl, _Float16* __restrict__ sW1,
                                         _Float16* __restrict__ sW2, const float* __restrict__ sBias, int n, int t_first, int lane, int wave) {
    constexpr int CS = C + 8;
    const int T = p.T, halo = p.halo;
    const int TT = MRF_R - 2 * halo;
    const float slope = p.slope;
    const float* __restrict__ xn = p.x + (int64_t)n * T * C;
    const int col = lane & 31;
    const bool colok = col < C;
    const int jbase = 32 * wave + 4 * (lane >> 5);
    const int w_lo = 32 * wave, w_hi = 32 * wave + 32;
    const int pbase = (MRF_G + jbase) * CS + col;
    uint32_t inside = 0xffffu;
    if (EDGE) {
        inside = 0;
#pragma unroll
        for (int r = 0; r < 16; ++r) {
            const int t = t_first + jbase + (r & 3) + 8 * (r >> 2);
            inside |= (t >= 0 && t < T) ? (1u << r) : 0u;
        }
    }

    float sum[16];
#pragma unroll
    for (int r = 0; r < 16; ++r) sum[r] = 0.f;

    for (int br = 0; br < 3; ++br) {
        const int k = p.k[br], hk = (k - 1) / 2, ldb = k * C + 8;
        int ext = hk * (p.dil[br * 3 + 0] + p.dil[br * 3 + 1] + p.dil[br * 3 + 2] + 3);

        float xr[16];
        if (w_hi > halo - ext && w_lo < halo + TT + ext && colok) {
            if (EDGE) {
#pragma unroll
                for (int r = 0; r < 16; ++r) {
                    const int t = min(max(t_first + jbase + (r & 3) + 8 * (r >> 2), 0), T - 1);
                    xr[r] = xn[(int64_t)t * C + col];
                }
            } else {
                const float* __restrict__ xb = xn + (int64_t)(t_first + jbase) * C + col;
#pragma unroll
                for (int r = 0; r < 16; ++r) xr[r] = xb[((r & 3) + 8 * (r >> 2)) * C];
            }
#pragma unroll
            for (int r = 0; r < 16; ++r) {
                if (EDGE && !((inside >> r) & 1)) xr[r] = 0.f;
                mrf_put<SINGLE>(ph, pl, pbase + ((r & 3) + 8 * (r >> 2)) * CS, xr[r], slope);
            }
        } else {
#pragma unroll
            for (int r = 0; r < 16; ++r) xr[r] = 0.f;
        }
        __syncthreads();

        for (int d = 0; d < 3; ++d) {
            const int q = br * 3 + d;
            const int dil = p.dil[q];
            const bool more = q + 1 < 9;
            const int qn = more ? q + 1 : q;
            const int kn = p.k[qn / 3];
// ... 2 lines not shown
                ext -= hk * dil;
                const bool act = w_hi > halo - ext && w_lo < halo + TT + ext;
                float16_t acc[1];
#pragma unroll
                for (int r = 0; r < 16; ++r) acc[0][r] = 0.f;
                if (act) mrf_conv<C, SINGLE>(ph, pl, MRF_G + 32 * wave - hk * dil, dil, k, sW1, ldb, lane, acc[0]);
                asm volatile("s_waitcnt vmcnt(0)" ::: "memory");
                __syncthreads();
                if (more) mrf_w_dma<C>(p.w1[qn], p.ldw1[qn], kn, sW1, lane, wave);
                if (act && colok) {
                    const float b = sBias[(2 * q) * C + col];
#pragma unroll
                    for (int r = 0; r < 16; ++r) {
                        float v = (acc[0][r] + b) * 1.0f;
                        if (EDGE && !((inside >> r) & 1)) v = 0.f;
                        mrf_put<SINGLE>(ph, pl, pbase + ((r & 3) + 8 * (r >> 2)) * CS, v, slope);
                    }
                }
                __syncthreads();
            }
            {
                ext -= hk;
                const bool act = w_hi > halo - ext && w_lo < halo + TT + ext;
                float16_t acc[1];
#pragma unroll
                for (int r = 0; r < 16; ++r) acc[0][r] = 0.f;
                if (act) mrf_conv<C, SINGLE>(ph, pl, MRF_G + 32 * wave - hk, 1, k, sW2, ldb, lane, acc[0]);
                asm volatile("s_waitcnt vmcnt(0)" ::: "memory");
                __syncthreads();
                if (more) mrf_w_dma<C>(p.w2[qn], p.ldw2[qn], kn, sW2, lane, wave);
                if (act && colok) {
                    const float b = sBias[(2 * q + 1) * C + col];
#pragma unroll
                    for (int r = 0; r < 16; ++r) {
                        float v = (acc[0][r] + b) * 1.0f + xr[r];
                        if (EDGE && !((inside >> r) & 1)) v = 0.f;
                        xr[r] = v;
                        if (d < 2) mrf_put<SINGLE>(ph, pl, pbase + ((r & 3) + 8 * (r >> 2)) * CS, v, slope);
                    }
                }
                if (d < 2) __syncthreads();
            }
        }
        if (br < 2) {
#pragma unroll
            for (int r = 0; r < 16; ++r) sum[r] = br == 0 ? xr[r] : sum[r] + xr[r];
        } else {
#pragma unroll
            for (int r = 0; r < 16; ++r) sum[r] = (sum[r] + xr[r]) / 3.0f;
        }
    }

    if (colok) {
        float* __restrict__ outb = p.out + (int64_t)n * T * C + (int64_t)(t_first + jbase) * C + col;
#pragma unroll
        for (int r = 0; r < 16; ++r) {
            const int j = jbase + (r & 3) + 8 * (r >> 2);
            if (j >= halo && j < halo + TT && (!EDGE || t_first + j < T)) outb[((r & 3) + 8 * (r >> 2)) * C] = sum[r];
        }
    }
}

template <int C>
constexpr int mrf_w_halfs() {
    return (C * (MRF_KMAX * C / 8 + 1) + 63) / 64 * 512;
}

template <int C, bool SINGLE = false>
__global__ __launch_bounds__(MRF_THREADS) void mrf_fused_kernel(MrfArgs p, int tiles) {
    constexpr int CS = C + 8;
    constexpr int PR = MRF_R + 2 * MRF_G;
    constexpr int NPL = SINGLE ? 1 : 2;
    extern __shared__ __attribute__((aligned(16))) unsigned char rb_smem[];
    _Float16* const ph = reinterpret_cast<_Float16*>(rb_smem);
    _Float16* const pl = SINGLE ? ph : ph + PR * CS;
    _Float16* const sW1 = ph + NPL * PR * CS;
    _Float16* const sW2 = sW1 + mrf_w_halfs<C>();
    float* const sBias = reinterpret_cast<float*>(sW2 + mrf_w_halfs<C>());

    const int tid = threadIdx.x, lane = tid & 63;
    const int wave = __builtin_amdgcn_readfirstlane(tid >> 6);
    const int n = blockIdx.x / tiles;
    const int tile = blockIdx.x - n * tiles;
    const int t_first = tile * (MRF_R - 2 * p.halo) - p.halo;

    mrf_w_dma<C>(p.w1[0], p.ldw1[0], p.k[0], sW1, lane, wave);
    mrf_w_dma<C>(p.w2[0], p.ldw2[0], p.k[0], sW2, lane, wave);
    if (tid < C) {
        float v[18];
#pragma unroll
        for (int q = 0; q < 9; ++q) {
            v[2 * q] = p.b1[q] ? p.b1[q][tid] : 0.f;
            v[2 * q + 1] = p.b2[q] ? p.b2[q][tid] : 0.f;
        }
#pragma unroll
        for (int i = 0; i < 18; ++i) sBias[i * C + tid] = v[i];
    }
    {
        const half8_t z = {0, 0, 0, 0, 0, 0, 0, 0};
        for (int i = tid; i < NPL * PR * CS / 8; i += MRF_THREADS) reinterpret_cast<half8_t*>(ph)[i] = z;
    }
    asm volatile("s_waitcnt vmcnt(0)" ::: "memory");
    __syncthreads();
    if (t_first < 0 || t_first + MRF_R > p.T) mrf_tile<C, true, SINGLE>(p, ph, pl, sW1, sW2, sBias, n, t_first, lane, wave);
    else mrf_tile<C, false, SINGLE>(p, ph, pl, sW1, sW2, sBias, n, t_first, lane, wave);
}

}
static size_t weights_lds_bytes(int C, int k) {
    return C > 32 ? (size_t)2 * C * (C + 8) * sizeof(_Float16) : (size_t)C * (k * C + 8) * sizeof(_Float16);
}
namespace {

template <int C, bool SINGLE>
void launch_cfg(const ResPairArgs& a, hipStream_t s) {
    static bool attr_set = false;
    if (!attr_set) {
        SC_HIP(hipFuncSetAttribute(reinterpret_cast<const void*>(&resblock_pair_kernel<C, SINGLE>),
                                   hipFuncAttributeMaxDynamicSharedMemorySize, 120 * 1024));
        attr_set = true;
    }
    const int H2 = (a.k - 1) / 2, H1 = a.dil * (a.k - 1) / 2;
    const int TT = RB_M1 - 2 * H2;
    const int tiles = cdiv(a.T, TT);
    const size_t act_halfs = SINGLE ? std::max<size_t>((size_t)(RB_M1 + 2 * H1) * (C + 8), (size_t)RB_M1 * (C + 4) * 2)
                                    : (size_t)2 * (RB_M1 + 2 * H1) * (C + 8);
    const size_t lds = act_halfs * sizeof(_Float16) + weights_lds_bytes(C, a.k);
    SC_CHECK(lds <= 120 * 1024, "resblock pair: %zu bytes of LDS (C=%d k=%d dil=%d)", lds, C, a.k, a.dil);
    char name[48];
    snprintf(name, sizeof(name), "resblock_pair_c%d", C);
    const double rows = (double)a.nb * a.T;
    prof::Scope scope(name, 2.0 * 2.0 * rows * C * (double)C * a.k,
                      4.0 * rows * C * (a.avg_a ? 4.0 : 2.0) + 2.0 * 2.0 * C * (double)C * a.k, s);
    hipLaunchKernelGGL((resblock_pair_kernel<C, SINGLE>), dim3((unsigned)(a.nb * tiles)), dim3(256), lds, s, a, tiles);
}

}

bool resblock_pair_supported(int C, int k, int dil) {
    if (!(C == 16 || C == 32 || C == 64) || k < 1 || (k & 1) == 0 || dil < 1) return false;
    const int H1 = dil * (k - 1) / 2;
    const size_t lds = (size_t)2 * (RB_M1 + 2 * H1) * (C + 8) * sizeof(_Float16) + weights_lds_bytes(C, k);
    return RB_M1 - (k - 1) >= 32 && lds <= 120 * 1024;
}

void launch_resblock_pair(const ResPairArgs& a, hipStream_t s) {
    SC_CHECK(resblock_pair_supported(a.C, a.k, a.dil), "resblock pair: unsupported C=%d k=%d dil=%d", a.C, a.k, a.dil);
    SC_CHECK(a.nb > 0 && a.T > 0, "resblock pair: empty problem");
    SC_CHECK(a.ldw1 % 8 == 0 && a.ldw2 % 8 == 0 && a.ldw1 >= (int64_t)a.k * a.C && a.ldw2 >= (int64_t)a.k * a.C,
             "resblock pair: packed weight rows too short");
    SC_CHECK((a.avg_a == nullptr) == (a.avg_b == nullptr), "resblock pair: avg_a/avg_b must be given together");
    SC_CHECK((int64_t)a.nb * cdiv(a.T, RB_M1 - (a.k - 1)) < (1ll << 31), "resblock pair: grid too large");
    if (a.single) {
        if (a.C == 16) launch_cfg<16, true>(a, s);
        else if (a.C == 32) launch_cfg<32, true>(a, s);
        else launch_cfg<64, true>(a, s);
    } else {
        if (a.C == 16) launch_cfg<16, false>(a, s);
        else if (a.C == 32) launch_cfg<32, false>(a, s);
        else launch_cfg<64, false>(a, s);
    }
    SC_LAUNCH_CHECK();
}

static int mrf_halo(const MrfArgs& a) {
    int halo = 0;
    for (int j = 0; j < 3; ++j) halo = std::max(halo, (a.k[j] - 1) / 2 * (a.dil[j * 3] + a.dil[j * 3 + 1] + a.dil[j * 3 + 2] + 3));
    return halo;
}

bool mrf_fused_supported(int C, const int* k, const int* dil) {
    if (C != 16 && C != 32) return false;
    int halo = 0;
    for (int j = 0; j < 3; ++j) {
        if (k[j] < 1 || (k[j] & 1) == 0 || k[j] > MRF_KMAX) return false;
        int sum = 3;
        for (int d = 0; d < 3; ++d) {
            if (dil[j * 3 + d] < 1 || (k[j] - 1) / 2 * dil[j * 3 + d] > MRF_G) return false;
            sum += dil[j * 3 + d];
        }
        halo = std::max(halo, (k[j] - 1) / 2 * sum);
    }
    return MRF_R - 2 * halo >= 128;
}

namespace {
template <int C, bool SINGLE>
void launch_mrf_cfg(MrfArgs a, hipStream_t s) {
    constexpr size_t LDS = ((size_t)(SINGLE ? 1 : 2) * (MRF_R + 2 * MRF_G) * (C + 8) + (size_t)2 * mrf_w_halfs<C>()) * sizeof(_Float16) + 18 * C * sizeof(float);
    static_assert(LDS <= 160 * 1024, "planes + two weight buffers must fit in the CU's LDS");
    static bool attr_set = false;
    if (!attr_set) {
        SC_HIP(hipFuncSetAttribute(reinterpret_cast<const void*>(&mrf_fused_kernel<C, SINGLE>), hipFuncAttributeMaxDynamicSharedMemorySize, (int)LDS));
        attr_set = true;
    }
    a.halo = mrf_halo(a);
    const int TT = MRF_R - 2 * a.halo;
    const int tiles = cdiv(a.T, TT);
    SC_CHECK((int64_t)a.nb * tiles < (1ll << 31), "mrf: grid too large");
    char name[48];
    snprintf(name, sizeof(name), "mrf_fused_c%d", C);
    const double rows = (double)a.nb * a.T;
    double flops = 0.0, wbytes = 0.0;
    for (int j = 0; j < 3; ++j) {
        flops += 3.0 * 2.0 * 2.0 * rows * C * (double)C * a.k[j];
        wbytes += 3.0 * 2.0 * 2.0 * C * (double)C * a.k[j];
    }
    prof::Scope scope(name, flops, 4.0 * rows * C * 2.0 + wbytes, s);
    hipLaunchKernelGGL((mrf_fused_kernel<C, SINGLE>), dim3((unsigned)(a.nb * tiles)), dim3(MRF_THREADS), LDS, s, a, tiles);
}
}

void launch_mrf_fused(const MrfArgs& a, hipStream_t s) {
    SC_CHECK(mrf_fused_supported(a.C, a.k, a.dil), "mrf: unsupported C=%d k=(%d,%d,%d)", a.C, a.k[0], a.k[1], a.k[2]);
    SC_CHECK(a.nb > 0 && a.T > 0 && a.x && a.out && a.x != a.out, "mrf: empty problem or in-place call");
    for (int q = 0; q < 9; ++q) {
        const int k = a.k[q / 3];
        SC_CHECK(a.w1[q] && a.w2[q] && a.ldw1[q] % 8 == 0 && a.ldw2[q] % 8 == 0 && a.ldw1[q] >= (int64_t)k * a.C && a.ldw2[q] >= (int64_t)k * a.C,
                 "mrf: packed weight rows of pair %d missing or too short", q);
    }
    if (a.single) {
        if (a.C == 16) launch_mrf_cfg<16, true>(a, s);
        else launch_mrf_cfg<32, true>(a, s);
    } else {
        if (a.C == 16) launch_mrf_cfg<16, false>(a, s);
        else launch_mrf_cfg<32, false>(a, s);
    }
    SC_LAUNCH_CHECK();
}

}
```

seamless_communication_amd/csrc/kernels.h:

```cpp
#pragma once
#include <atomic>

#include "common.h"
#include "prof.h"

namespace sc {

enum Act { ACT_NONE = 0, ACT_RELU = 1, ACT_SILU = 2, ACT_TANH = 3 };
enum InAct { IN_NONE = 0, IN_LRELU_01 = 1, IN_LRELU_001 = 2 };

struct GemmArgs {
    const float* A = nullptr;
    int64_t lda = 0;
    const __half* W = nullptr;
    int64_t ldw = 0;
    int64_t w_phase_stride = 0;
    const float* bias = nullptr;
    const float* res = nullptr;
    int64_t ldr = 0;
    float* C = nullptr;
    int64_t ldc = 0;
    int M = 0;
    int N = 0;
    int K = 0;
    int rows_per_batch = 0;
    int t_in = 0;
    int t_out = 0;
    int taps = 1, cin = 0, dil = 0, stride = 1, pad = 0;
    int out_mul = 1, out_off = 0, out_off_phase_step = 0;
    const int* in_lens = nullptr;
    int in_act = IN_NONE;
    int act = ACT_NONE;
    float alpha = 1.0f;
    int phases = 1;
    int split = 1;
    double algo_flops = 0;
};

void launch_gemm(const GemmArgs& a, hipStream_t s);
extern std::atomic<int> g_force_general_gemm;
bool gemm_fast_eligible(const GemmArgs& a);
void launch_gemm_fast(const GemmArgs& a, hipStream_t s);

struct GemmPsArgs {
    const __half* Ah = nullptr;
    const __half* Al = nullptr;
    int64_t lda = 0;
    const __half* W = nullptr;
    int64_t ldw = 0;
    const float* bias = nullptr;
    const float* res = nullptr;
    int64_t ldr = 0;
    float* C = nullptr;
    int64_t ldc = 0;
    __half* Ch = nullptr;
    __half* Cl = nullptr;
    int64_t ldcs = 0;
    int M = 0, N = 0, K = 0;
    int act = ACT_NONE;
    float alpha = 1.0f;
    int split = 1;
    float plane_neg_slope = 1.0f;
    int conv_taps = 0, conv_cin = 0, conv_dil = 1, conv_pad = 0, rows_per_item = 0;
    const unsigned char* row_valid = nullptr;
    const int2* row_pos = nullptr;
    float2* amax = nullptr;
    int amax_ld = 0;
};
void launch_gemm_presplit(const GemmPsArgs& a, hipStream_t s);
int gemm_presplit_amax_chunks(int M, int N);
void launch_amax_finish(const float2* part, int ld, int rows, int* out_idx, hipStream_t s);

struct ResPairArgs {
    const float* x = nullptr;
    float* out = nullptr;
    const __half* w1 = nullptr;
    int64_t ldw1 = 0;
    const float* b1 = nullptr;
    const __half* w2 = nullptr;
    int64_t ldw2 = 0;
    const float* b2 = nullptr;
    int nb = 0, T = 0, C = 0, k = 0, dil = 1;
    float slope = 0.1f;
    const float* avg_a = nullptr;
    const float* avg_b = nullptr;
    int single = 0;
};
bool resblock_pair_supported(int C, int k, int dil);
void launch_resblock_pair(const ResPairArgs& a, hipStream_t s);

struct MrfArgs {
    const float* x = nullptr;
    float* out = nullptr;
    int nb = 0, T = 0, C = 0;
    float slope = 0.1f;
    int halo = 0;
    int k[3] = {0, 0, 0};
    int dil[9] = {1, 1, 1, 1, 1, 1, 1, 1, 1};
    const __half* w1[9] = {};
    const __half* w2[9] = {};
    int64_t ldw1[9] = {};
    int64_t ldw2[9] = {};
    const float* b1[9] = {};
    const float* b2[9] = {};
    int single = 0;
};
bool mrf_fused_supported(int C, const int* k, const int* dil);
void launch_mrf_fused(const MrfArgs& a, hipStream_t s);

void launch_gemv(const float* x, int64_t ldx, const __half* W, int64_t ldw, const float* bias,
                 const float* res, int64_t ldr, float* out, int64_t ldo, int M, int N, int K,
                 int act, float alpha, hipStream_t s);

struct SkinnyArgs {
    const float* A = nullptr;
    int64_t lda = 0;
    const __half* W = nullptr;
    int64_t ldw = 0;
    const float* bias = nullptr;
    const float* res = nullptr;
    int64_t ldr = 0;
    float* C = nullptr;
    int64_t ldc = 0;
    float* partial = nullptr;
    int M = 0, N = 0, K = 0;
    int act = ACT_NONE;
    float alpha = 1.0f;
    int splits = 1;
    int kc = 0;
    float4* am_part = nullptr;
    int am_tiles_cap = 0;
    int am_tiles = 0;
    float* am_eos_logit = nullptr;
    const int* am_pos = nullptr;
    int am_min_step_for_eos = 0, am_force_eos_step = -1;
    int am_pad_idx = -1, am_eos_idx = -1, am_unk_idx = -1;
    float am_unk_penalty = 0.f;
};
int skinny_argmax_tiles(int M, int N);
void launch_argmax_finalize(const float4* part, int tiles, int nb, const float* eos_logit, const int* d_pos,
                            int force_eos_step, int pad_idx, int eos_idx, int* next_tok, int* hist, int hist_ld,
                            int* finished, int* out_len, float* score, hipStream_t s);
void launch_skinny(const SkinnyArgs& a, hipStream_t s);
int skinny_splits(int M, int N, int K, int want_split);
void launch_reduce_res_ln(const float* partial, int splits, const float* bias, float* x, const float* gamma,
                          const float* beta, float* h, int rows, int C, hipStream_t s);

int64_t packed_weight_halfs(int N, int K);
void launch_pack_weight(const __half* w, int64_t ldw, int N, int K, __half* dst, hipStream_t s);
enum GemvEpilogue {
    EPI_PARTIAL = 0,
    EPI_PLANES = 1,
    EPI_ARGMAX = 2,
};
struct GemvPArgs {
    const __half* Wp = nullptr;
    const __half* Ah = nullptr;
    const __half* Al = nullptr;
    int RB = 32;
    int M = 0, N = 0, K = 0;
// ... 247 lines not shown
    const int* done = nullptr;
    int* slot_utt = nullptr;
    int* d_slots = nullptr;
    int* d_rows = nullptr;
    int* seqs = nullptr;
    float* cum = nullptr;
    int* tok = nullptr;
    int* enc_lens = nullptr;
    int* anc = nullptr;
    int n = 0, beams = 0, max_len = 0, anc_ld = 0;
    int seq_len = 0, anc_len = 0;
};
void launch_beam_compact(const BeamCompactArgs& a, hipStream_t s);
void launch_row_token_lprob(const float* logits, int64_t ld, int rows, int V, int row_stride, int token, float* out, hipStream_t s);
void launch_gather_cache(const float* src, float* dst, const int* src_row, int rows, int len, int cap, int M, int layers,
                         int64_t layer_stride, hipStream_t s);

void launch_fbank(const float* wav, int64_t wav_stride, const int* num_samples, int nb, float* out,
                  int t_rows , const float* consts, float scale, hipStream_t s);
void launch_fbank_any(const float* wav, int64_t wav_stride, const int* num_samples, int nb, float* out, int t_rows, const float* consts,
                      float scale, int frame_len, int frame_shift, int nfft, hipStream_t s);
void launch_standardize(float* feat, int nb, int t_rows, const int* num_frames, int C, hipStream_t s);

void launch_embed_tokens(const int* tokens, int rows, const __half* emb, int M, float scale,
                         const float* pos_table, const int* d_pos, int t_per_batch, float* out,
                         int64_t ldo, hipStream_t s);
void launch_step_update(int* next_tok, int* hist, int hist_ld, int* finished, int* out_len,
                        const float* lprob, float* score, int nb, const int* d_pos, int pad_idx,
                        int eos_idx, int* n_unfinished, hipStream_t s);
void launch_argmax_rows(const float* logits, int64_t ld, int rows, int V, const int* d_pos,
                        int min_pos_for_eos, int force_eos_pos, int pad_idx, int eos_idx, int unk_idx,
                        float unk_penalty, int* out_idx, float* out_lprob, hipStream_t s);
void launch_cvt_f16_f32(const __half* src, float* dst, int64_t n, hipStream_t s);
void launch_cvt_f32_f16(const float* src, __half* dst, int64_t n, hipStream_t s);
void launch_pack_conv_weight(const __half* w , __half* dst , int Co,
                             int Ci, int k, int Kpad, hipStream_t s);
void launch_pack_convT_weight(const float* w , __half* dst ,
                              int Ci, int Co, int k, int stride, int Kpad, hipStream_t s);
void launch_weight_norm_fold(const __half* v, const __half* g, float* out, int d0, int inner,
                             hipStream_t s);
void launch_gather_rows(const float* src, int64_t lds, const int* row_idx , float* dst,
                        int64_t ldd, int rows, int C, hipStream_t s);
void launch_char_embed_add(float* seqs , int64_t ld, const int* char_ids,
                           const __half* embed_char, const float* pos_table, int t_per_batch,
                           float alpha, float scale, int rows, int M, hipStream_t s);
void launch_pos_add_rows(float* seqs, int64_t ld, const float* pos_table, const int* row_t, float alpha, int rows, int M, hipStream_t s);
void launch_pos_add(float* seqs, int64_t ld, const float* pos_table, int t_per_batch, float alpha,
                    int rows, int M, hipStream_t s);
void launch_durations(const float* h , int64_t ld, const float* w, const float* b,
                      int rows, int H, int t_per_batch, const int* lens, float duration_factor,
                      int min_dur, int* durations, hipStream_t s);
void launch_vocoder_embed(const int* units, int nb, int T, const __half* dict, int E,
                          const __half* lang, int Lg, const int* lang_idx, const __half* spkr, int Sp,
                          const int* spkr_idx, float* out , hipStream_t s);
void launch_avg3(const float* a, const float* b, const float* c, float* out, int64_t n, hipStream_t s);
bool conv_to_mono_supported(int cin, int cout, int k, int stride, int pad, int dil, int act);
void launch_conv_to_mono(const float* x, const __half* w_packed, const float* bias, int nb, int T, int cin, int k, float in_slope, int act,
                         float* y, hipStream_t s);
void launch_fill_i32(int* p, int v, int n, hipStream_t s);
void launch_add_i32(int* p, int v, hipStream_t s);

constexpr int ROWSWAP_MAX_LAYERS = 32;
constexpr int ROWSWAP_MAX_PAIRS = 64;
struct RowSwapArgs {
    float* k[ROWSWAP_MAX_LAYERS];
    float* v[ROWSWAP_MAX_LAYERS];
    float* cross[ROWSWAP_MAX_LAYERS];
    int layers = 0, pairs = 0;
    unsigned char src[ROWSWAP_MAX_PAIRS], dst[ROWSWAP_MAX_PAIRS];
    int M = 0, cap = 0, s_enc = 0, filled = 0;
    int* tok = nullptr;
    int* finished = nullptr;
    int* out_len = nullptr;
    int* enc_lens = nullptr;
    float* lprob = nullptr;
    float* score = nullptr;
    int* hist = nullptr;
    float* hidden = nullptr;
};
void launch_row_swap(const RowSwapArgs& a, hipStream_t s);

constexpr int XCAP_MAX_HEADS = 16;
struct XattnCapArgs {
    const float* q = nullptr;
    const float* kv = nullptr;
    const int* enc_lens = nullptr;
    const int* d_pos = nullptr;
    const int* d_rows = nullptr;
    const int* finished = nullptr;
    const int* out_len = nullptr;
    const int* slot_utt = nullptr;
    const float4* am_part = nullptr;
    int am_tiles = 0;
    const float* eos_logit = nullptr;
    int force_eos_step = -1;
    float* xattn = nullptr;
    float* lprob = nullptr;
    int nb = 0, s_enc = 0, heads = 0, cap = 0;
};
void launch_xattn_capture(const XattnCapArgs& a, hipStream_t s);

struct EngineRows {
    int* tok = nullptr;
    int* pos = nullptr;
    int* finished = nullptr;
    int* out_len = nullptr;
    int* limit = nullptr;
    int* prefix_len = nullptr;
    int* enc_lens = nullptr;
    float* score = nullptr;
    int* hist = nullptr;
// ... 28 lines not shown
```

seamless_communication_amd/csrc/model.h:

```cpp
#pragma once
#include <map>
#include <functional>
#include <memory>
#include <string>
#include <unordered_map>
#include <vector>

#include "../../include/seamless_hip.h"
#include "kernels.h"

namespace sc {

class DevicePool {
   public:
    ~DevicePool();
    void* get(size_t bytes);
    void put(void* p);
    void release_all();
    void trim();
    void set_stream(hipStream_t s) { stream_ = s; }
    void set_oom_hook(std::function<void()> f) { oom_hook_ = std::move(f); }

   private:
    std::function<void()> oom_hook_;
    void* debug_filled(void* p, size_t bytes);
    hipStream_t stream_ = nullptr;
    std::multimap<size_t, void*> free_;
    std::unordered_map<void*, size_t> size_;
    size_t cached_bytes_ = 0;
};

template <typename T>
class Buf {
   public:
    Buf() = default;
    Buf(DevicePool* pool, size_t n) : pool_(pool), n_(n) { p_ = n ? static_cast<T*>(pool->get(n * sizeof(T))) : nullptr; }
    Buf(const Buf&) = delete;
    Buf& operator=(const Buf&) = delete;
    Buf(Buf&& o) noexcept : pool_(o.pool_), p_(o.p_), n_(o.n_) { o.p_ = nullptr; }
    Buf& operator=(Buf&& o) noexcept {
        if (this != &o) {
            reset();
            pool_ = o.pool_;
            p_ = o.p_;
            n_ = o.n_;
            o.p_ = nullptr;
        }
        return *this;
    }
    ~Buf() { reset(); }
    void reset() {
        if (p_) pool_->put(p_);
        p_ = nullptr;
// ... 133 lines not shown
    LNorm vdp_ln1, vdp_ln2;
    const float* vdp_proj_w = nullptr;
    const float* vdp_proj_b = nullptr;
    const float* dp_proj_w = nullptr;
    const float* dp_proj_b = nullptr;
    std::vector<FFTLayer> t2u_dec;
    LNorm t2u_dec_ln;
    std::vector<int32_t> tok_len;
    std::vector<uint8_t> starts_space, is_punct;
    std::vector<int64_t> char_offsets;
    std::vector<int32_t> char_ids;
    const __half* voc_dict = nullptr;
    const __half* voc_lang = nullptr;
    const __half* voc_spkr = nullptr;
    Conv voc_pre, voc_post;
    std::vector<ConvT> voc_ups;
    std::vector<ResBlock> voc_res;
};

struct DecodeSession;
void delete_decode_session(DecodeSession* s);
class Engine;

struct MmaState {
    int s_enc = 0, cap = 0, pos = 0;
    int cap_enc = 0;
    Buf<float> kv, cross, kenergy, work, pchoose;
    Buf<int> ints;
    Buf<__half> planes;
};

struct Model : ModelData {
    hipStream_t stream = nullptr;
    hipEvent_t order_event = nullptr;
    DevicePool pool;
    struct SideChain {
        hipStream_t stream = nullptr;
        hipEvent_t done = nullptr;
        DevicePool pool;
    };
    std::vector<std::unique_ptr<SideChain>> side;
    hipEvent_t side_fork = nullptr;
    void trim_all_pools();
    void hook_pool(DevicePool& p) { p.set_oom_hook([this] { trim_all_pools(); }); }
    DevicePool* pool_override = nullptr;
    DevicePool* pp() { return pool_override ? pool_override : &pool; }
    SideChain& side_chain(int k);
    std::vector<void*> owned;

    std::vector<int32_t> last_units, last_durations, last_char_ids, last_char_seq_lens;
    int last_n = 0, last_su = 0, last_sc = 0;
    int64_t last_padded_unit_rows = 0;
    int64_t last_vocoder_unit_rows = 0;

    std::unique_ptr<MmaState> mma;

    struct FbankRate {
        float* consts = nullptr;
        int frame_len = 0, frame_shift = 0, nfft = 0;
    };
    std::map<int, FbankRate> fbank_rates;


    std::unique_ptr<DecodeSession, void (*)(DecodeSession*)> dec_session{nullptr, delete_decode_session};

    Engine* engine = nullptr;
    int engine_announced = 0;

    Model() = default;
    Model(const Model&) = delete;
    Model& operator=(const Model&) = delete;
    ~Model();
};

struct SideScope {
    Model& m;
    hipStream_t saved;
    SideScope(Model& mm, int k) : SideScope(mm, mm.side_chain(k)) {}
    SideScope(Model& mm, Model::SideChain& c) : m(mm), saved(mm.stream) {
        m.stream = c.stream;
        m.pool_override = &c.pool;
    }
    ~SideScope() {
        m.stream = saved;
        m.pool_override = nullptr;
    }
    SideScope(const SideScope&) = delete;
    SideScope& operator=(const SideScope&) = delete;
};

void load_model(Model& m, const sc_tensor_desc* t, size_t n);
void run_fbank(Model& m, const float* d_wav, int n, int64_t wav_stride, const int32_t* h_ns, int standardize,
               float* d_out, int t_rows, int32_t* h_frames, int sample_rate = 16000);
int fbank_num_frames(int64_t num_samples, int sample_rate);
int encoder_out_len(const Model& m, int t_frames);
void run_encode_speech(Model& m, const float* d_fbank, int n, int t_frames, const int32_t* h_lens, float* d_out,
                       int32_t* h_out_lens);
void run_mma_begin(Model& m, const float* d_enc, int s_enc, int max_len);
void run_mma_step(Model& m, const int32_t* h_tokens, int n_tokens, const int32_t* h_blocked, int n_blocked, int32_t* out_index,
                  float* h_pchoose, float* d_features);
int text_to_char_seqs_host(int vocab, const int32_t* tok_len, const uint8_t* starts_space, const uint8_t* is_punct,
                           const int64_t* offs, const int32_t* ids, int pad_idx, int unk_idx, int eos_idx, const int32_t* text_seqs,
                           int n, int s_text, int32_t* out_char_lens, int32_t* out_char_ids, int cap, int32_t* out_seq_lens);
void run_encode_text(Model& m, const int32_t* h_tokens, int n, int s_text, const int32_t* h_lens, float* d_out);
int text_max_len(const Model& m, const sc_gen_opts& o, int s_enc);
int decoder_step_family(const Model& m, int rows, int caller);
void ngram_blocked_tokens(const int32_t* seq, int S, int G, std::vector<int32_t>& out);
struct XattnCapture {
    float* d_xattn = nullptr;
    float* h_step_lprob = nullptr;
};
struct BannedHost {
    const int32_t* tokens = nullptr;
    const int32_t* offsets = nullptr;
    int n = 0;
};
void banned_blocked_tokens(const int32_t* seq, int S, const BannedHost& b, std::vector<int32_t>& out);
void run_generate_text(Model& m, const float* d_enc, int n, int s_enc, const int32_t* h_enc_lens,
                       const sc_gen_opts& o, const int32_t* h_prefix, int prefix_len, int32_t* h_out_ids,
                       int32_t* h_out_lens, float* h_scores, float* d_dec_hidden, const int32_t* h_forced_tokens,
                       int forced_len, const XattnCapture* xcap = nullptr, const BannedHost* banned = nullptr);
void run_t2u_nar(Model& m, const float* d_dec_hidden, int n, int s_text, const int32_t* h_text_lens,
                 const int32_t* h_text_seqs, float duration_factor, int32_t* h_unit_lens, int32_t* out_su,
                 int32_t* out_sc);
void conv1d_presplit(Model& m, const __half* xh, const __half* xl, const Conv& c, const float* res, float* C, __half* Ch, __half* Cl,
                     int nb, int t, int pad, int dil, const unsigned char* row_valid, int act, int rows_total = 0,
                     const int2* row_pos = nullptr, float plane_neg_slope = 1.0f, int split = 1);
void run_vocoder_durations(Model& m, const int32_t* h_units, int n, int s_units, int32_t* h_durations);
void run_t2u_ar(Model& m, const float* d_dec_hidden, int n, int s_text, const int32_t* h_text_lens, const sc_gen_opts& o,
                const int32_t* h_prefix, int prefix_len, int32_t* h_out_ids, int32_t* h_out_lens, float* h_scores);
void run_t2u_encoder(Model& m, const float* d_dec_hidden, int n, int s_text, const int* d_text_lens, float* d_out);
void run_generate_beam(Model& m, const DecStack& W, const float* d_enc, int n, int s_enc, const int32_t* h_enc_lens, const sc_gen_opts& o,
                       const int32_t* h_prefix, int prefix_len, int32_t* h_out_ids, int32_t* h_out_lens, float* h_scores,
                       float* d_dec_hidden, int max_len, const BannedHost* banned = nullptr);
void run_vocode(Model& m, const int32_t* h_units, int n, int s_units, const int32_t* h_lang, const int32_t* h_spkr,
                float* d_wav, const int32_t* h_unit_lens = nullptr);
std::vector<std::vector<int>> plan_length_groups(const std::vector<int>& lens, int overhead_rows, int max_groups);

void linear(Model& m, const float* x, int64_t ldx, const Linear& L, const float* res, int64_t ldr, float* y,
            int64_t ldy, int rows, int act, float alpha, bool row_independent = false);
inline void project_cross_kv(Model& m, const float* d_enc, const Linear& L, float* out, int rows) {
    linear(m, d_enc, L.in, L, nullptr, 0, out, L.out, rows, ACT_NONE, 1.f, true);
}
void layernorm(Model& m, const float* x, const LNorm& L, float* y, int rows, int act = ACT_NONE,
               const int* lens = nullptr, int t_per_batch = 1);
void conv1d(Model& m, const float* x, const Conv& c, const float* res, float* y, int nb, int t_in, int stride, int pad,
            int dil, const int* d_in_lens, int in_act, int act);
void conv_transpose1d(Model& m, const float* x, const ConvT& c, float* y, int nb, int t_in, int in_act);

}
```

seamless_communication_amd/csrc/model_load.hip:

```cpp
#include <cmath>
#include <cstring>

#include <cstdlib>

#include "model.h"

namespace sc {

DevicePool::~DevicePool() { release_all(); }

static int debug_fill_byte() {
    static const int v = [] {
        (void)knob::is_set("SC_DEBUG_FILL");
        const char* e = getenv("SC_DEBUG_FILL");
        return e && *e ? (int)strtol(e, nullptr, 0) & 0xff : -1;
    }();
    return v;
}

void* DevicePool::debug_filled(void* p, size_t bytes) {
    const int v = debug_fill_byte();
    if (v >= 0 && p && stream_) {
        hipStreamCaptureStatus st = hipStreamCaptureStatusNone;
        if (hipStreamIsCapturing(stream_, &st) == hipSuccess && st == hipStreamCaptureStatusNone)
// ... 588 lines not shown
void linear(Model& m, const float* x, int64_t ldx, const Linear& L, const float* res, int64_t ldr, float* y,
            int64_t ldy, int rows, int act, float alpha, bool row_independent) {
    if (rows <= 0) return;
    if (!row_independent && rows <= 64 && L.in % 64 == 0 && ldx % 4 == 0 && (reinterpret_cast<uintptr_t>(x) & 15) == 0) {
        SkinnyArgs a;
        a.A = x;
        a.lda = ldx;
        a.W = L.w;
        a.ldw = L.ldw;
        a.bias = L.b;
        a.res = res;
        a.ldr = ldr;
        a.C = y;
        a.ldc = ldy;
        a.M = rows;
        a.N = L.out;
        a.K = L.in;
        a.act = act;
        a.alpha = alpha;
        launch_skinny(a, m.stream);
        return;
    }
    GemmArgs a;
    a.A = x;
    a.lda = ldx;
    a.W = L.w;
    a.ldw = L.ldw;
    a.bias = L.b;
    a.res = res;
    a.ldr = ldr;
    a.C = y;
    a.ldc = ldy;
    a.M = rows;
    a.N = L.out;
    a.K = L.kpad;
    a.rows_per_batch = rows;
    a.t_in = rows;
    a.t_out = rows;
    a.taps = 1;
    a.cin = L.kpad;
    a.dil = 0;
    a.stride = 1;
    a.pad = 0;
    a.act = act;
    a.alpha = alpha;
    launch_gemm(a, m.stream);
}

void layernorm(Model& m, const float* x, const LNorm& L, float* y, int rows, int act, const int* lens, int t_per_batch) {
    launch_layernorm(x, L.dim, L.g, L.b, y, L.dim, rows, L.dim, act, lens, t_per_batch, m.stream);
}

void conv1d(Model& m, const float* x, const Conv& c, const float* res, float* y, int nb, int t_in, int stride, int pad,
            int dil, const int* d_in_lens, int in_act, int act) {
    const int t_out = (t_in + 2 * pad - dil * (c.k - 1) - 1) / stride + 1;
    if (nb <= 0 || t_out <= 0) return;
    if (!res && !d_in_lens && g_force_general_gemm.load(std::memory_order_relaxed) == 0 &&
        conv_to_mono_supported(c.cin, c.cout, c.k, stride, pad, dil, act)) {
        const float slope = in_act == IN_LRELU_01 ? 0.1f : in_act == IN_LRELU_001 ? 0.01f : 1.0f;
        launch_conv_to_mono(x, c.w, c.b, nb, t_in, c.cin, c.k, slope, act, y, m.stream);
        return;
    }
    GemmArgs a;
    a.A = x;
    a.lda = c.cin;
    a.W = c.w;
    a.ldw = c.kpad;
    a.bias = c.b;
    a.res = res;
    a.ldr = c.cout;
    a.C = y;
    a.ldc = c.cout;
    a.M = nb * t_out;
    a.N = c.cout;
    a.K = c.kpad;
    a.rows_per_batch = t_out;
    a.t_in = t_in;
    a.t_out = t_out;
    a.taps = c.k;
    a.cin = c.cin;
    a.dil = dil;
    a.stride = stride;
    a.pad = pad;
    a.in_lens = d_in_lens;
    a.in_act = in_act;
    a.act = act;
    launch_gemm(a, m.stream);
}

void conv1d_presplit(Model& m, const __half* xh, const __half* xl, const Conv& c, const float* res, float* C, __half* Ch, __half* Cl,
                     int nb, int t, int pad, int dil, const unsigned char* row_valid, int act, int rows_total, const int2* row_pos,
                     float plane_neg_slope, int split) {
    SC_CHECK(c.kpad == c.cin * c.k && 2 * pad == dil * (c.k - 1), "conv1d_presplit: needs an unpadded weight row and 'same' padding");
    if (row_pos ? rows_total <= 0 : (nb <= 0 || t <= 0)) return;
    GemmPsArgs a;
    a.Ah = xh;
    a.Al = xl;
    a.lda = c.cin;
    a.W = c.w;
    a.ldw = c.kpad;
    a.bias = c.b;
    a.res = res;
    a.ldr = c.cout;
    a.C = C;
    a.ldc = c.cout;
    a.Ch = Ch;
    a.Cl = Cl;
    a.ldcs = c.cout;
    a.M = row_pos ? rows_total : nb * t;
    a.N = c.cout;
    a.K = c.kpad;
    a.act = act;
    a.conv_taps = c.k;
    a.conv_cin = c.cin;
    a.conv_dil = dil;
    a.conv_pad = pad;
    a.rows_per_item = row_pos ? 0 : t;
    a.row_pos = row_pos;
    a.row_valid = row_valid;
    a.plane_neg_slope = plane_neg_slope;
    a.split = split;
    launch_gemm_presplit(a, m.stream);
}

void conv_transpose1d(Model& m, const float* x, const ConvT& c, float* y, int nb, int t_in, int in_act) {
    if (nb <= 0 || t_in <= 0) return;
    GemmArgs a;
    a.A = x;
    a.lda = c.cin;
    a.W = c.w;
    a.ldw = c.kpad;
    a.w_phase_stride = (int64_t)c.cout * c.kpad;
    a.bias = c.b;
    a.C = y;
    a.ldc = c.cout;
    a.rows_per_batch = t_in + 1;
    a.M = nb * (t_in + 1);
    a.N = c.cout;
    a.K = c.kpad;
    a.t_in = t_in;
    a.t_out = t_in * c.stride;
    a.taps = c.taps;
    a.cin = c.cin;
    a.dil = -1;
    a.stride = 1;
    a.pad = 0;
    a.out_mul = c.stride;
    a.out_off = -c.pad;
    a.out_off_phase_step = 1;
    a.phases = c.stride;
    a.in_act = in_act;
    a.algo_flops = 2.0 * nb * (double)t_in * c.cin * c.cout * c.k;
    launch_gemm(a, m.stream);
}

}
```

seamless_communication_amd/csrc/model_t2u.hip:

```cpp
#include <cstdlib>

#include "model.h"

namespace sc {

namespace {

void attention_self(Model& m, const float* qkv, int M, float* out, int nb, int S, const int* d_lens) {
    AttnArgs a;
    a.q = qkv;
    a.k = qkv + M;
    a.v = qkv + 2 * M;
    a.out = out;
    a.ldq = a.ldk = a.ldv = 3 * M;
    a.ldo = M;
    a.nb = nb;
    a.heads = m.cfg.num_heads;
    a.Sq = S;
    a.Skv = S;
    a.kv_lens = d_lens;
    launch_attention(a, m.stream);
}

void text_to_char_seqs(const Model& m, const int32_t* text_seqs, int n, int s_text, std::vector<int32_t>& char_lens,
// ... 380 lines not shown
        for (int gi = 0; gi < ng; ++gi) {
            const int b = grp[gi];
            glens[gi] = ulens[b];
            int pos = 0;
            for (int k = 0; k < Sc; ++k)
                for (int r = 0; r < dur[(size_t)b * Sc + k]; ++r) uidx[(size_t)gi * Lg + pos++] = b * Sc + k;
        }
        Buf<int> d_uidx(m.pp(), grows), d_glens(m.pp(), ng);
        id_bufs.emplace_back(m.pp(), grows);
        int* d_ids = id_bufs.back();
        SC_HIP(hipMemcpyAsync(d_uidx.get(), uidx.data(), (size_t)grows * 4, hipMemcpyHostToDevice, m.stream));
        SC_HIP(hipMemcpyAsync(d_glens.get(), glens.data(), (size_t)ng * 4, hipMemcpyHostToDevice, m.stream));
        Buf<float> u(m.pp(), (size_t)grows * M), y(m.pp(), (size_t)grows * M), att(m.pp(), (size_t)grows * M),
            wide(m.pp(), (size_t)grows * wideN);
        launch_gather_rows(cs, M, d_uidx, u, M, grows, M, m.stream);
        launch_pos_add(u, M, m.unit_pos, Lg, m.pos_alpha, grows, M, m.stream);
        const int K = c.t2u_conv_kernel;
        for (const FFTLayer& l : m.t2u_dec) {
            linear(m, u, M, l.qkv, nullptr, 0, wide, 3 * M, grows, ACT_NONE, 1.f);
            attention_self(m, wide, M, att, ng, Lg, d_glens);
            linear(m, att, M, l.attn_out, u, M, y, M, grows, ACT_NONE, 1.f);
            layernorm(m, y, l.attn_ln, y, grows);
            conv1d(m, y, l.conv1, nullptr, wide, ng, Lg, 1, K / 2, 1, d_glens, IN_NONE, ACT_RELU);
            conv1d(m, wide, l.conv2, y, u, ng, Lg, 1, K / 2, 1, d_glens, IN_NONE, ACT_NONE);
            layernorm(m, u, l.conv_ln, u, grows);
        }
        layernorm(m, u, m.t2u_dec_ln, u, grows);
        Buf<float> logits(m.pp(), (size_t)grows * c.unit_vocab_size);
        Linear proj;
        proj.w = m.unit_embed;
        proj.ldw = M;
        proj.kpad = M;
        proj.in = M;
        proj.out = c.unit_vocab_size;
        linear(m, u, M, proj, nullptr, 0, logits, c.unit_vocab_size, grows, ACT_NONE, 1.f);
        launch_argmax_rows(logits, c.unit_vocab_size, grows, c.unit_vocab_size, nullptr, -1, -1, -1, -1, -1, 0.f, d_ids, nullptr,
                           m.stream);
        keep_alive.emplace_back((size_t)grows);
        SC_HIP(hipMemcpyAsync(keep_alive.back().data(), d_ids, (size_t)grows * 4, hipMemcpyDeviceToHost, m.stream));
    }
    SC_HIP(hipStreamSynchronize(m.stream));
    for (size_t g = 0; g < groups.size(); ++g) {
        const std::vector<int>& grp = groups[g];
        const std::vector<int32_t>& gids = keep_alive[3 * g + 2];
        const int Lg = (int)(gids.size() / grp.size());
        for (size_t gi = 0; gi < grp.size(); ++gi)
            for (int t = 0; t < ulens[grp[gi]]; ++t) ids[(size_t)grp[gi] * Su + t] = gids[gi * Lg + t];
    }
    finish(ids, rows_done);
}

namespace {

void vocode_batch(Model& m, const int* d_units, const int* d_lang, const int* d_spkr, int n, int T, float* d_wav) {
    const sc_config& c = m.cfg;
    const int E = c.voc_embedding_dim, Lg = c.voc_lang_embedding_dim, Sp = c.voc_spkr_embedding_dim;
    int ch = c.voc_upsample_initial_channel;
    int t = T;
    Buf<float> x;
    {
        Buf<float> in(m.pp(), (size_t)n * T * (E + Lg + Sp));
        launch_vocoder_embed(d_units, n, T, m.voc_dict, E, m.voc_lang, Lg, d_lang, m.voc_spkr, Sp, d_spkr, in, m.stream);
        x = Buf<float>(m.pp(), (size_t)n * T * ch);
        conv1d(m, in, m.voc_pre, nullptr, x, n, T, 1, 3, 1, nullptr, IN_NONE, ACT_NONE);
    }
    const int nk = c.voc_num_resblock_kernels;
    SC_CHECK(nk == 3, "sc_vocode: %d resblock kernels (only 3 is implemented)", nk);
    static const int voc_split = knob::value("SC_VOC_SPLIT", 0);
    const int voc_single = (voc_split & 1 ? 0 : 1) | (voc_split & 4 ? 0 : 4);
    for (int i = 0; i < c.voc_num_upsamples; ++i) {
        const ConvT& up = m.voc_ups[i];
        const int t2 = t * up.stride;
        ch = up.cout;
        const size_t sz = (size_t)n * t2 * ch;
        Buf<float> y(m.pp(), sz), tmp(m.pp(), sz), ra(m.pp(), sz), rb(m.pp(), sz);
        Buf<float> rout[3] = {Buf<float>(m.pp(), sz), Buf<float>(m.pp(), sz), Buf<float>(m.pp(), sz)};
        conv_transpose1d(m, x, up, y, n, t, IN_LRELU_01);
        bool fused_avg = false;
        x = Buf<float>(m.pp(), sz);
        static const bool voc_ps = knob::value("SC_VOC_PS", 1) != 0;
        bool wide_ps = voc_ps && g_force_general_gemm.load(std::memory_order_relaxed) == 0 && ch >= 128 && ch % 32 == 0 &&
                       (int64_t)n * t2 * ch * 2 < (1ll << 31);
        for (int j = 0; j < nk && wide_ps; ++j) {
            const ResBlock& r = m.voc_res[i * nk + j];
            for (size_t d = 0; d < r.dil.size(); ++d)
                wide_ps = wide_ps && r.convs1[d].cin == ch && r.convs1[d].cout == ch && r.convs2[d].cin == ch && r.convs2[d].cout == ch &&
                          r.convs1[d].kpad == ch * r.convs1[d].k && r.convs2[d].kpad == ch * r.convs2[d].k && (r.convs1[d].k & 1) &&
                          (r.convs2[d].k & 1);
        }
        if (wide_ps) {
            const bool one_plane = (voc_single & 1) != 0;
            Buf<__half> planes(m.pp(), (one_plane ? 3 : 6) * sz);
            __half* py_h = planes.get();
            __half* pt_h = py_h + sz;
            __half* pn_h = pt_h + sz;
            __half* py_l = one_plane ? nullptr : pn_h + sz;
            __half* pt_l = one_plane ? nullptr : py_l + sz;
            __half* pn_l = one_plane ? nullptr : pt_l + sz;
            launch_lrelu_split_f32(y, 0.1f, py_h, py_l, (int64_t)sz, m.stream);
            for (int j = 0; j < nk; ++j) {
                const ResBlock& r = m.voc_res[i * nk + j];
                const float* cur = y;
                const __half *ch_ = py_h, *cl_ = py_l;
                const int nd = (int)r.dil.size();
                for (int d = 0; d < nd; ++d) {
                    const int k = r.convs1[d].k, k2 = r.convs2[d].k;
                    const bool last = d == nd - 1;
                    float* dst = last ? rout[j].get() : ((d & 1) ? rb.get() : ra.get());
                    const int split = one_plane ? 0 : 1;
                    conv1d_presplit(m, ch_, cl_, r.convs1[d], nullptr, nullptr, pt_h, pt_l, n, t2, (k * r.dil[d] - r.dil[d]) / 2, r.dil[d], nullptr,
                                    ACT_NONE, 0, nullptr, 0.1f, split);
                    conv1d_presplit(m, pt_h, pt_l, r.convs2[d], cur, dst, last ? nullptr : pn_h, last ? nullptr : pn_l, n, t2, (k2 - 1) / 2, 1,
                                    nullptr, ACT_NONE, 0, nullptr, 0.1f, split);
                    cur = dst;
                    ch_ = pn_h;
                    cl_ = pn_l;
                }
            }
            launch_avg3(rout[0], rout[1], rout[2], x, (int64_t)sz, m.stream);
            t = t2;
            continue;
        }
        static const bool voc_mrf = knob::value("SC_VOC_MRF", 1) != 0;
        if (voc_mrf && g_force_general_gemm.load(std::memory_order_relaxed) == 0) {
            MrfArgs a;
            bool ok = true;
            for (int j = 0; j < nk && ok; ++j) {
                const ResBlock& r = m.voc_res[i * nk + j];
                ok = r.dil.size() == 3;
                for (int d = 0; d < 3 && ok; ++d) {
                    const Conv &c1 = r.convs1[d], &c2 = r.convs2[d];
                    ok = c1.k == r.convs1[0].k && c2.k == c1.k && c1.cin == ch && c1.cout == ch && c2.cin == ch && c2.cout == ch;
                    const int q = j * 3 + d;
                    a.dil[q] = r.dil[d];
                    a.w1[q] = c1.w, a.ldw1[q] = c1.kpad, a.b1[q] = c1.b;
                    a.w2[q] = c2.w, a.ldw2[q] = c2.kpad, a.b2[q] = c2.b;
                }
                if (ok) a.k[j] = r.convs1[0].k;
            }
            if (ok && mrf_fused_supported(ch, a.k, a.dil)) {
                a.x = y.get();
                a.out = x.get();
                a.nb = n;
                a.T = t2;
                a.C = ch;
                a.slope = 0.1f;
                a.single = (voc_single & 4) ? 1 : 0;
                launch_mrf_fused(a, m.stream);
                t = t2;
                continue;
            }
        }
        for (int j = 0; j < nk; ++j) {
            const ResBlock& r = m.voc_res[i * nk + j];
            const float* cur = y;
            const int nd = (int)r.dil.size();
            for (int d = 0; d < nd; ++d) {
                const int k = r.convs1[d].k;
                float* dst = (d == nd - 1) ? rout[j].get() : ((d & 1) ? rb.get() : ra.get());
                const bool fuse = g_force_general_gemm.load(std::memory_order_relaxed) == 0 && r.convs2[d].k == k &&
                                  r.convs1[d].cin == ch && r.convs1[d].cout == ch && r.convs2[d].cin == ch &&
                                  r.convs2[d].cout == ch && resblock_pair_supported(ch, k, r.dil[d]);
                if (fuse) {
                    ResPairArgs a;
                    a.x = cur;
                    a.w1 = r.convs1[d].w;
                    a.ldw1 = r.convs1[d].kpad;
                    a.b1 = r.convs1[d].b;
                    a.w2 = r.convs2[d].w;
                    a.ldw2 = r.convs2[d].kpad;
                    a.b2 = r.convs2[d].b;
                    a.nb = n;
                    a.T = t2;
                    a.C = ch;
                    a.k = k;
                    a.dil = r.dil[d];
                    a.slope = 0.1f;
                    a.single = (voc_single & 4) ? 1 : 0;
                    if (j == nk - 1 && d == nd - 1) {
                        a.avg_a = rout[0];
                        a.avg_b = rout[1];
                        dst = x.get();
                        fused_avg = true;
                    }
                    a.out = dst;
                    launch_resblock_pair(a, m.stream);
                } else {
                    conv1d(m, cur, r.convs1[d], nullptr, tmp, n, t2, 1, (k * r.dil[d] - r.dil[d]) / 2, r.dil[d], nullptr,
                           IN_LRELU_01, ACT_NONE);
                    conv1d(m, tmp, r.convs2[d], cur, dst, n, t2, 1, (k - 1) / 2, 1, nullptr, IN_LRELU_01, ACT_NONE);
                }
                cur = dst;
            }
        }
        if (!fused_avg) launch_avg3(rout[0], rout[1], rout[2], x, (int64_t)sz, m.stream);
        t = t2;
    }
    conv1d(m, x, m.voc_post, nullptr, d_wav, n, t, 1, 3, 1, nullptr, IN_LRELU_001, ACT_TANH);
}

int vocoder_halo_units(const Model& m) {
    const sc_config& c = m.cfg;
    double halo = 3.0, rate = 1.0;
    for (int i = 0; i < c.voc_num_upsamples; ++i) {
        const ConvT& up = m.voc_ups[i];
        halo += (double)up.taps / rate;
        rate *= up.stride;
        int widest = 0;
        for (int j = 0; j < c.voc_num_resblock_kernels; ++j) {
            const ResBlock& r = m.voc_res[i * c.voc_num_resblock_kernels + j];
            int reach = 0;
            for (size_t d = 0; d < r.dil.size(); ++d) reach += (r.convs1[d].k - 1) * r.dil[d] / 2 + (r.convs2[d].k - 1) / 2;
            widest = std::max(widest, reach);
        }
        halo += (double)widest / rate;
    }
    halo += 3.0 / rate;
    return (int)halo + 8;
}

}

__global__ void embed_rows_f16_kernel(const int* __restrict__ idx, const __half* __restrict__ table, int E, float* __restrict__ out) {
    const int r = blockIdx.x;
    const __half* src = table + (int64_t)idx[r] * E;
    for (int c = threadIdx.x; c < E; c += blockDim.x) out[(int64_t)r * E + c] = __half2float(src[c]);
}

void run_vocoder_durations(Model& m, const int32_t* h_units, int n, int T, int32_t* h_durations) {
    const sc_config& c = m.cfg;
    SC_CHECK(c.has_vocoder && m.vdp_proj_w, "sc_vocoder_durations: the model was loaded without the vocoder's duration predictor");
    SC_CHECK(n > 0 && T > 0, "sc_vocoder_durations: empty batch");
    prof::set_tag("voc");
    const int E = c.voc_embedding_dim, H = c.voc_dur_pred_hidden_dim, K = c.voc_dur_pred_kernel_size;
    const int rows = n * T;
    for (int i = 0; i < rows; ++i)
        SC_CHECK(h_units[i] >= 0 && h_units[i] < c.voc_num_embeddings, "sc_vocoder_durations: unit %d outside the vocoder dictionary", h_units[i]);
    Buf<int> d_units(m.pp(), rows), d_dur(m.pp(), rows);
    SC_HIP(hipMemcpyAsync(d_units.get(), h_units, (size_t)rows * 4, hipMemcpyHostToDevice, m.stream));
    Buf<float> x(m.pp(), (size_t)rows * E), a(m.pp(), (size_t)rows * H), b(m.pp(), (size_t)rows * H);
    hipLaunchKernelGGL(embed_rows_f16_kernel, dim3(rows), dim3(256), 0, m.stream, d_units.get(), m.voc_dict, E, x.get());
    SC_LAUNCH_CHECK();
    conv1d(m, x, m.vdp_conv1, nullptr, a, n, T, 1, K / 2, 1, nullptr, IN_NONE, ACT_RELU);
    layernorm(m, a, m.vdp_ln1, b, rows);
    conv1d(m, b, m.vdp_conv2, nullptr, a, n, T, 1, K / 2, 1, nullptr, IN_NONE, ACT_RELU);
    layernorm(m, a, m.vdp_ln2, b, rows);
    launch_durations(b, H, m.vdp_proj_w, m.vdp_proj_b, rows, H, T, nullptr, 1.0f, 1, d_dur, m.stream);
    SC_HIP(hipMemcpyAsync(h_durations, d_dur.get(), (size_t)rows * 4, hipMemcpyDeviceToHost, m.stream));
    SC_HIP(hipStreamSynchronize(m.stream));
}

void run_vocode(Model& m, const int32_t* h_units, int n, int T, const int32_t* h_lang, const int32_t* h_spkr, float* d_wav,
                const int32_t* h_unit_lens) {
    const sc_config& c = m.cfg;
    SC_CHECK(c.has_vocoder, "sc_vocode: the model was loaded without a vocoder");
    prof::set_tag("voc");
    SC_CHECK(n > 0 && T > 0, "sc_vocode: empty batch");
    for (int i = 0; i < n; ++i) {
        SC_CHECK(h_lang[i] >= 0 && h_lang[i] < c.voc_num_langs, "sc_vocode: lang index %d out of range", h_lang[i]);
        SC_CHECK(h_spkr[i] >= 0 && h_spkr[i] < c.voc_num_spkrs, "sc_vocode: speaker index %d out of range", h_spkr[i]);
        SC_CHECK(!h_unit_lens || (h_unit_lens[i] >= 0 && h_unit_lens[i] <= T), "sc_vocode: unit_lens[%d]=%d outside [0,%d]", i,
                 h_unit_lens ? h_unit_lens[i] : 0, T);
    }
    for (int64_t i = 0; i < (int64_t)n * T; ++i)
        SC_CHECK(h_units[i] >= 0 && h_units[i] < c.voc_num_embeddings, "sc_vocode: unit %d out of range [0,%d)", h_units[i],
                 c.voc_num_embeddings);
    int hop = 1;
    for (const ConvT& up : m.voc_ups) hop *= up.stride;
    static const int max_groups = std::max(1, knob::value("SC_VOC_GROUPS", 8));
    if (!h_unit_lens || max_groups == 1) {
        Buf<int> d_units(m.pp(), (size_t)n * T), d_ls(m.pp(), 2 * n);
        SC_HIP(hipMemcpyAsync(d_units.get(), h_units, (size_t)n * T * 4, hipMemcpyHostToDevice, m.stream));
        SC_HIP(hipMemcpyAsync(d_ls.get(), h_lang, (size_t)n * 4, hipMemcpyHostToDevice, m.stream));
        SC_HIP(hipMemcpyAsync(d_ls.get() + n, h_spkr, (size_t)n * 4, hipMemcpyHostToDevice, m.stream));
        vocode_batch(m, d_units, d_ls, d_ls.get() + n, n, T, d_wav);
        m.last_vocoder_unit_rows = (int64_t)n * T;
        SC_HIP(hipStreamSynchronize(m.stream));
        return;
    }
    const int halo = vocoder_halo_units(m);
    std::vector<int> need(n);
    for (int i = 0; i < n; ++i) need[i] = std::min(T, h_unit_lens[i] + halo);
    static const int group_overhead = std::max(0, knob::value("SC_VOC_GROUP_OVERHEAD", 250));
    const std::vector<std::vector<int>> groups = plan_length_groups(need, group_overhead, max_groups);
    SC_HIP(hipMemsetAsync(d_wav, 0, (size_t)n * T * hop * sizeof(float), m.stream));
    static const int max_chains = std::max(1, std::min(8, knob::value("SC_VOC_STREAMS", 3)));
    const int chains = std::min<int>(max_chains, (int)groups.size());
    if (chains > 1) {
        m.side_chain(chains - 1);
        SC_HIP(hipEventRecord(m.side_fork, m.stream));
        for (int k = 0; k < chains; ++k) SC_HIP(hipStreamWaitEvent(m.side[k]->stream, m.side_fork, 0));
    }
    struct Join {
        Model& m;
        int chains;
        bool joined = false;
        ~Join() {
            if (joined || chains <= 1) return;
            for (int k = 0; k < chains && k < (int)m.side.size(); ++k) (void)hipStreamSynchronize(m.side[k]->stream);
        }
    } join{m, chains};
    std::vector<std::vector<int32_t>> staging;
    staging.reserve(2 * groups.size());
    int64_t rows_done = 0;
    for (size_t g = 0; g < groups.size(); ++g) {
        const std::vector<int>& grp = groups[g];
        std::unique_ptr<SideScope> scope;
        if (chains > 1) scope.reset(new SideScope(m, (int)(g % chains)));
        const int ng = (int)grp.size();
        int Lg = 0;
        for (int b : grp) Lg = std::max(Lg, need[b]);
        rows_done += (int64_t)ng * Lg;
        staging.emplace_back((size_t)ng * Lg);
        std::vector<int32_t>& gu = staging.back();
        staging.emplace_back((size_t)2 * ng);
        std::vector<int32_t>& gls = staging.back();
        for (int gi = 0; gi < ng; ++gi) {
            const int b = grp[gi];
            std::copy(h_units + (size_t)b * T, h_units + (size_t)b * T + Lg, gu.begin() + (size_t)gi * Lg);
            gls[gi] = h_lang[b];
            gls[ng + gi] = h_spkr[b];
        }
        Buf<int> d_units(m.pp(), (size_t)ng * Lg), d_ls(m.pp(), 2 * ng);
        SC_HIP(hipMemcpyAsync(d_units.get(), gu.data(), (size_t)ng * Lg * 4, hipMemcpyHostToDevice, m.stream));
        SC_HIP(hipMemcpyAsync(d_ls.get(), gls.data(), (size_t)2 * ng * 4, hipMemcpyHostToDevice, m.stream));
        Buf<float> gw(m.pp(), (size_t)ng * Lg * hop);
        vocode_batch(m, d_units, d_ls, d_ls.get() + ng, ng, Lg, gw);
        for (int gi = 0; gi < ng; ++gi)
            SC_HIP(hipMemcpyAsync(d_wav + (size_t)grp[gi] * T * hop, gw.get() + (size_t)gi * Lg * hop, (size_t)Lg * hop * sizeof(float),
                                  hipMemcpyDeviceToDevice, m.stream));
    }
    for (int k = 0; k < chains && chains > 1; ++k) {
        SC_HIP(hipEventRecord(m.side[k]->done, m.side[k]->stream));
        SC_HIP(hipStreamWaitEvent(m.stream, m.side[k]->done, 0));
    }
// ... 7 lines not shown
```

Measured before the change: 331.2.

## Pack ragged vocoder batches into one varlen pass instead of length buckets

Adds a packed (varlen) path to the vocoder: utterances of different lengths are concatenated back to back using per-item offsets, and the GEMM, conv and embed kernels resolve each row's owning item through a cursor and per-stage tile tables. This replaces the bucketed side-chain scheme, which padded every utterance in a group to the group's longest length and spread groups over several streams. The aim is to stop computing on padding rows and to cut launch count. The cost is per-row item lookup inside the kernels, host-side table building, and a scatter back to the padded output. It also gives up overlap across side streams.

Result: faster. 338.9 (median of 6 runs) (+2.3%).

```diff
diff --git a/include/seamless_hip_internal.h b/include/seamless_hip_internal.h
--- a/include/seamless_hip_internal.h
+++ b/include/seamless_hip_internal.h
@@ -12,6 +12,9 @@
 int sc_op_knob(const char* name, int dflt);
 
 int sc_op_force_general_gemm(int on);
+int32_t sc_op_voc_pack_plan(const int32_t* h_need, int32_t n, int64_t budget_rows, int32_t* h_group_first, int32_t cap);
+int32_t sc_op_voc_tile_first(const int32_t* h_off, int32_t n, int32_t mul, int32_t tile_rows, int32_t* h_first);
+int32_t sc_op_last_vocoder_packed_groups(sc_model* m);
 int sc_op_single_plane(int on);
 int sc_op_layernorm(const float* d_x, const float* d_gamma, const float* d_beta, float* d_y, int32_t rows, int32_t C,
                     int32_t act);
diff --git a/seamless_communication_amd/_lib.py b/seamless_communication_amd/_lib.py
--- a/seamless_communication_amd/_lib.py
+++ b/seamless_communication_amd/_lib.py
@@ -141,6 +141,9 @@
     "sc_banned_blocked_tokens": (C.c_int32, [_PI, C.c_int32, _PI, _PI, C.c_int32, _PI, C.c_int32]),
     "sc_op_knob": (C.c_int, [C.c_char_p, C.c_int]),
     "sc_op_force_general_gemm": (C.c_int, [C.c_int]),
+    "sc_op_voc_pack_plan": (C.c_int32, [_PI, C.c_int32, C.c_int64, _PI, C.c_int32]),
+    "sc_op_voc_tile_first": (C.c_int32, [_PI, C.c_int32, C.c_int32, C.c_int32, _PI]),
+    "sc_op_last_vocoder_packed_groups": (C.c_int32, [_P]),
     "sc_op_single_plane": (C.c_int, [C.c_int]),
     "sc_op_layernorm": (C.c_int, [_P, _P, _P, _P, _i, _i, _i]),
     "sc_op_linear": (C.c_int, [_P, _P, _P, _P, _P, _i, _i, _i, _i, C.c_float, _i, _i]),
diff --git a/seamless_communication_amd/csrc/api.hip b/seamless_communication_amd/csrc/api.hip
--- a/seamless_communication_amd/csrc/api.hip
+++ b/seamless_communication_amd/csrc/api.hip
@@ -572,6 +572,28 @@
     g_op_single.store(on ? 1 : 0);
     return SC_OK;
 }
+
+int32_t sc_op_voc_pack_plan(const int32_t* h_need, int32_t n, int64_t budget_rows, int32_t* h_group_first, int32_t cap) {
+    try {
+        SC_CHECK(h_need && n > 0 && budget_rows > 0 && (h_group_first || cap == 0) && cap >= 0, "sc_op_voc_pack_plan: bad argument");
+        const std::vector<int> first = sc::plan_packed_groups(std::vector<int>(h_need, h_need + n), budget_rows);
+        for (size_t i = 0; i < first.size() && i < (size_t)cap; ++i) h_group_first[i] = first[i];
+        return (int32_t)first.size() - 1;
+    } catch (const sc::Error& e) {
+        return e.code;
+    }
+}
+int32_t sc_op_voc_tile_first(const int32_t* h_off, int32_t n, int32_t mul, int32_t tile_rows, int32_t* h_first) {
+    try {
+        SC_CHECK(h_off && h_first && n > 0 && mul > 0 && tile_rows > 0, "sc_op_voc_tile_first: bad argument");
+        const std::vector<int> first = sc::packed_tile_first(std::vector<int>(h_off, h_off + n + 1), mul, tile_rows);
+        for (int i = 0; i <= n; ++i) h_first[i] = first[i];
+        return SC_OK;
+    } catch (const sc::Error& e) {
+        return e.code;
+    }
+}
+int32_t sc_op_last_vocoder_packed_groups(sc_model* m) { return m ? m->m.last_vocoder_packed_groups : -1; }
 
 int sc_op_force_general_gemm(int on) {
     sc::g_force_general_gemm.store(on ? 1 : 0);
diff --git a/seamless_communication_amd/csrc/common.cpp b/seamless_communication_amd/csrc/common.cpp
--- a/seamless_communication_amd/csrc/common.cpp
+++ b/seamless_communication_amd/csrc/common.cpp
@@ -44,6 +44,8 @@
     {"SC_VOC_PS", 0, "0: vocoder wide stages on the register-staged convolution"}, {"SC_VOC_MRF", 0, "0: narrow vocoder stages as nine pair launches"},
     {"SC_VOC_GROUPS", 0, "vocoder: length buckets"}, {"SC_VOC_GROUP_OVERHEAD", 0, "vocoder: bucket planning overhead rows"},
     {"SC_VOC_STREAMS", 0, "vocoder: side chains"},
+    {"SC_VOC_PACKED", 0, "0: ragged vocoder batches in length buckets on side chains instead of the packed pass"},
+    {"SC_VOC_PACK_ROWS", 0, "vocoder: unit rows per packed group"},
     {"SC_ENGINE_RG_SMALL", 0, "decode engine: rows per row group, N = 1024 products"},
     {"SC_BEAM_COMPACT", 2, "0: beam search keeps finished utterances' slots"},
     {"SC_GREEDY_COMPACT", 2, "0: greedy generation keeps finished rows in their slots"}, {"SC_GREEDY_POLL", 2, "steps between looks at the finished flags"},
diff --git a/seamless_communication_amd/csrc/k_gemm.hip b/seamless_communication_amd/csrc/k_gemm.hip
--- a/seamless_communication_amd/csrc/k_gemm.hip
+++ b/seamless_communication_amd/csrc/k_gemm.hip
@@ -52,17 +52,24 @@
 
     const int a_kq = tid & 7;
     const int a_r = tid >> 3;
-    int a_n[A_IT], a_q[A_IT], a_len[A_IT];
+    int a_row0[A_IT], a_q[A_IT], a_len[A_IT];
+    GemmItemCursor cur;
+    if (p.item_off && m0 + a_r < p.M) cur.init(p, m0 + a_r);
 #pragma unroll
     for (int i = 0; i < A_IT; ++i) {
         const int m = m0 + a_r + 32 * i;
-        if (m < p.M) {
+        if (m < p.M && p.item_off) {
+            cur.seek(p, m);
+            a_row0[i] = cur.in_row0(p);
+            a_q[i] = cur.q(m);
+            a_len[i] = cur.t_in(p);
+        } else if (m < p.M) {
             const int n = m / p.rows_per_batch;
-            a_n[i] = n;
+            a_row0[i] = n * p.t_in;
             a_q[i] = m - n * p.rows_per_batch;
             a_len[i] = p.in_lens ? min(p.in_lens[n], p.t_in) : p.t_in;
         } else {
-            a_n[i] = 0;
+            a_row0[i] = 0;
             a_q[i] = 0;
             a_len[i] = -1;
         }
@@ -84,7 +91,7 @@
                 float4 v = make_float4(0.f, 0.f, 0.f, 0.f);
                 if (tap_ok && src_t >= 0 && src_t < a_len[i]) {
                     v = *reinterpret_cast<const float4*>(
-                        p.A + ((int64_t)a_n[i] * p.t_in + src_t) * p.lda + c0);
+                        p.A + ((int64_t)a_row0[i] + src_t) * p.lda + c0);
                 }
                 a_reg[i] = v;
             }
@@ -99,7 +106,7 @@
                 float4 v = make_float4(0.f, 0.f, 0.f, 0.f);
                 if (tap_ok && src_t >= 0 && src_t < a_len[i]) {
                     v = *reinterpret_cast<const float4*>(
-                        p.A + ((int64_t)a_n[i] * p.t_in + src_t) * p.lda + c0);
+                        p.A + ((int64_t)a_row0[i] + src_t) * p.lda + c0);
                 }
                 a_reg[i] = v;
             }
@@ -115,7 +122,7 @@
                     const int src_t = a_q[i] * p.stride + tap * p.dil - p.pad;
                     float v = 0.f;
                     if (tap < p.taps && src_t >= 0 && src_t < a_len[i]) {
-                        v = p.A[((int64_t)a_n[i] * p.t_in + src_t) * p.lda + c];
+                        v = p.A[((int64_t)a_row0[i] + src_t) * p.lda + c];
                     }
                     e[j] = v;
                 }
@@ -198,7 +205,8 @@
         __syncthreads();
     }
 
-    const bool plain_rows = (p.rows_per_batch == p.M) && p.out_mul == 1 && out_off == 0 && p.t_out == p.M;
+    const bool plain_rows = !p.item_off && (p.rows_per_batch == p.M) && p.out_mul == 1 && out_off == 0 && p.t_out == p.M;
+    if (p.item_off && m0 + wm * WM + 4 * (lane >> 5) < p.M) cur.init(p, m0 + wm * WM + 4 * (lane >> 5));
 #pragma unroll
     for (int i = 0; i < TM; ++i) {
 #pragma unroll
@@ -208,6 +216,11 @@
             int64_t row;
             if (plain_rows) {
                 row = m;
+            } else if (p.item_off) {
+                cur.seek(p, m);
+                const int dst_t = cur.q(m) * p.out_mul + out_off;
+                if (dst_t < 0 || dst_t >= cur.t_out(p)) continue;
+                row = cur.out_row0(p) + dst_t;
             } else {
                 const int n = m / p.rows_per_batch;
                 const int q = m - n * p.rows_per_batch;
diff --git a/seamless_communication_amd/csrc/k_gemm2.hip b/seamless_communication_amd/csrc/k_gemm2.hip
--- a/seamless_communication_amd/csrc/k_gemm2.hip
+++ b/seamless_communication_amd/csrc/k_gemm2.hip
@@ -36,6 +36,8 @@
         col[j] = n0w + j * 32 + (lane & 31);
         bcol[j] = (p.bias && col[j] < p.N) ? p.bias[col[j]] : 0.f;
     }
+    GemmItemCursor cur;
+    if (p.item_off && m0w + 4 * (lane >> 5) < p.M) cur.init(p, m0w + 4 * (lane >> 5));
 #pragma unroll
     for (int i = 0; i < TM; ++i) {
 #pragma unroll
@@ -45,6 +47,11 @@
             int64_t row;
             if (plain_rows) {
                 row = m;
+            } else if (p.item_off) {
+                cur.seek(p, m);
+                const int dst_t = cur.q(m) * p.out_mul + out_off;
+                if (dst_t < 0 || dst_t >= cur.t_out(p)) continue;
+                row = cur.out_row0(p) + dst_t;
             } else {
                 const int n = m / p.rows_per_batch;
                 const int q = m - n * p.rows_per_batch;
@@ -83,6 +90,8 @@
 #pragma unroll
         for (int e = 0; e < 4; ++e) b4[e] = (col + e < p.N) ? p.bias[col + e] : 0.f;
     }
+    GemmItemCursor cur;
+    if (p.item_off && m0w + row_in < p.M) cur.init(p, m0w + row_in);
 #pragma unroll
     for (int i = 0; i < TM; ++i) {
 #pragma unroll
@@ -98,6 +107,11 @@
             int64_t row;
             if (plain_rows) {
                 row = m;
+            } else if (p.item_off) {
+                cur.seek(p, m);
+                const int dst_t = cur.q(m) * p.out_mul + out_off;
+                if (dst_t < 0 || dst_t >= cur.t_out(p)) continue;
+                row = cur.out_row0(p) + dst_t;
             } else {
                 const int n = m / p.rows_per_batch;
                 const int q = m - n * p.rows_per_batch;
@@ -167,10 +181,17 @@
     const int a_r = tid >> 3;
     const float* a_base[A_IT];
     int a_t0[A_IT], a_len[A_IT];
+    GemmItemCursor cur;
+    if (p.item_off && m0 + a_r < p.M) cur.init(p, m0 + a_r);
 #pragma unroll
     for (int i = 0; i < A_IT; ++i) {
         const int m = m0 + a_r + 32 * i;
-        if (m < p.M) {
+        if (m < p.M && p.item_off) {
+            cur.seek(p, m);
+            a_base[i] = p.A + (int64_t)cur.in_row0(p) * p.lda + a_kq * 4;
+            a_t0[i] = cur.q(m) * p.stride - p.pad;
+            a_len[i] = cur.t_in(p);
+        } else if (m < p.M) {
             const int n = m / p.rows_per_batch;
             const int q = m - n * p.rows_per_batch;
             a_base[i] = p.A + (int64_t)n * p.t_in * p.lda + a_kq * 4;
@@ -295,7 +316,7 @@
 #undef SC_STORE_SLAB
 #undef SC_COMPUTE_SLAB
 
-    const bool plain_rows = (p.rows_per_batch == p.M) && p.out_mul == 1 && out_off == 0 && p.t_out == p.M;
+    const bool plain_rows = !p.item_off && (p.rows_per_batch == p.M) && p.out_mul == 1 && out_off == 0 && p.t_out == p.M;
     const int m0w = m0 + wm * WM, n0w = n0 + wn * WN;
 #define SC_EPI(ACT)                                                                               \
     do {                                                                                          \
@@ -351,10 +372,17 @@
     const int a_kq = tid & 7;
     const int a_r = tid >> 3;
     int a_row0[A_IT], a_t0[A_IT], a_len[A_IT];
+    GemmItemCursor cur;
+    if (p.item_off && m0 + a_r < p.M) cur.init(p, m0 + a_r);
 #pragma unroll
     for (int i = 0; i < A_IT; ++i) {
         const int m = m0 + a_r + 32 * i;
-        if (m < p.M) {
+        if (m < p.M && p.item_off) {
+            cur.seek(p, m);
+            a_row0[i] = cur.in_row0(p);
+            a_t0[i] = cur.q(m) * p.stride - p.pad;
+            a_len[i] = cur.t_in(p);
+        } else if (m < p.M) {
             const int n = m / p.rows_per_batch;
             const int q = m - n * p.rows_per_batch;
             a_row0[i] = n * p.t_in;
@@ -486,7 +514,7 @@
 #undef SC2_STORE
 #undef SC2_COMPUTE
 
-    const bool plain_rows = (p.rows_per_batch == p.M) && p.out_mul == 1 && out_off == 0 && p.t_out == p.M;
+    const bool plain_rows = !p.item_off && (p.rows_per_batch == p.M) && p.out_mul == 1 && out_off == 0 && p.t_out == p.M;
     const int m0w = m0 + wm * WM, n0w = n0 + wn * WN;
     float* ep = reinterpret_cast<float*>(smem_all) + wave * (32 * EP_LD);
 #define SC_EPI(ACT)                                                                                             \
@@ -518,9 +546,9 @@
     prof::Scope scope(name, flops, bytes, s);
     const dim3 grid(tiles_per_xcd * 8);
     static const int env_pf2 = knob::value("SC_GEMM_PF2", GEMM_PF2_DEFAULT);
-    const int64_t a_bytes64 = (int64_t)(a.M / a.rows_per_batch) * a.t_in * a.lda * 4;
+    const int64_t a_bytes64 = (a.item_off ? (int64_t)a.M - (int64_t)a.n_items * a.item_extra : (int64_t)(a.M / a.rows_per_batch) * a.t_in) * a.lda * 4;
     const int64_t w_bytes64 = (int64_t)a.N * a.ldw * 2;
-    if (env_pf2 && a.K % (2 * FBK) == 0 && a.M % a.rows_per_batch == 0 && a_bytes64 < (1ll << 31) && w_bytes64 < (1ll << 31)) {
+    if (env_pf2 && a.K % (2 * FBK) == 0 && (a.item_off || a.M % a.rows_per_batch == 0) && a_bytes64 < (1ll << 31) && w_bytes64 < (1ll << 31)) {
         const float slope = a.in_act == IN_LRELU_01 ? 0.1f : a.in_act == IN_LRELU_001 ? 0.01f : 0.f;
         if (a.in_act == IN_NONE)
             hipLaunchKernelGGL((gemm_fast2_kernel<BM, BN, WGM, WGN, false>), grid, dim3(256), 0, s, a, tiles_n, tiles_mn,
diff --git a/seamless_communication_amd/csrc/k_misc.hip b/seamless_communication_amd/csrc/k_misc.hip
--- a/seamless_communication_amd/csrc/k_misc.hip
+++ b/seamless_communication_amd/csrc/k_misc.hip
@@ -366,9 +366,9 @@
                                                             const int* __restrict__ lang_idx,
                                                             const __half* __restrict__ spkr, int Sp,
                                                             const int* __restrict__ spkr_idx,
-                                                            float* __restrict__ out) {
+                                                            float* __restrict__ out, const int* __restrict__ item_off, int n_items) {
     const int row = blockIdx.x;
-    const int n = row / T;
+    const int n = item_off ? item_search(n_items, row, [&](int i) { return item_off[i]; }) : row / T;
     const int C = Lg + E + Sp;
     const __half* l = lang + (int64_t)lang_idx[n] * Lg;
     const __half* d = dict + (int64_t)units[row] * E;
@@ -384,10 +384,11 @@
 }
 void launch_vocoder_embed(const int* units, int nb, int T, const __half* dict, int E, const __half* lang, int Lg,
                           const int* lang_idx, const __half* spkr, int Sp, const int* spkr_idx, float* out,
-                          hipStream_t s) {
-    if (nb * T <= 0) return;
-    hipLaunchKernelGGL(vocoder_embed_kernel, dim3(nb * T), dim3(256), 0, s, units, T, dict, E, lang, Lg, lang_idx, spkr,
-                       Sp, spkr_idx, out);
+                          hipStream_t s, const int* item_off, int rows_total) {
+    const int rows = item_off ? rows_total : nb * T;
+    if (rows <= 0) return;
+    hipLaunchKernelGGL(vocoder_embed_kernel, dim3(rows), dim3(256), 0, s, units, T, dict, E, lang, Lg, lang_idx, spkr,
+                       Sp, spkr_idx, out, item_off, nb);
     SC_LAUNCH_CHECK();
 }
 
@@ -441,14 +442,21 @@
 
 template <int C, int K>
 __global__ __launch_bounds__(256) void conv_to_mono_kernel(const float* __restrict__ x, const __half* __restrict__ w, const float* __restrict__ bias,
-                                                           float slope, int act, float* __restrict__ y, int T) {
+                                                           float slope, int act, float* __restrict__ y, int T,
+                                                           const int* __restrict__ item_off, int item_mul) {
     constexpr int RS = C + 4, ROWS = 256 + K - 1, VPR = C / 4;
     typedef float f4_t __attribute__((ext_vector_type(4)));
     __shared__ __attribute__((aligned(16))) float tile[ROWS * RS];
     __shared__ __attribute__((aligned(16))) float sw[K * C];
     const int tid = threadIdx.x, n = blockIdx.y;
     const int t0 = blockIdx.x * 256;
-    const float* __restrict__ xn = x + (int64_t)n * T * C;
+    int64_t row0 = (int64_t)n * T;
+    if (item_off) {
+        row0 = (int64_t)item_off[n] * item_mul;
+        T = (item_off[n + 1] - item_off[n]) * item_mul;
+        if (t0 >= T) return;
+    }
+    const float* __restrict__ xn = x + row0 * C;
     for (int i = tid; i < ROWS * VPR; i += 256) {
         const int r = i / VPR, c4 = i - r * VPR;
         const int t = t0 - K / 2 + r;
@@ -473,7 +481,7 @@
             for (int j = 0; j < 4; ++j) acc = fmaf(xv[j], wv[j], acc);
         }
     acc += bias ? bias[0] : 0.f;
-    y[(int64_t)n * T + t] = act == ACT_TANH ? tanhf(acc) : acc;
+    y[row0 + t] = act == ACT_TANH ? tanhf(acc) : acc;
 }
 
 bool conv_to_mono_supported(int cin, int cout, int k, int stride, int pad, int dil, int act) {
@@ -481,11 +489,41 @@
 }
 
 void launch_conv_to_mono(const float* x, const __half* w_packed, const float* bias, int nb, int T, int cin, int k, float in_slope, int act,
-                         float* y, hipStream_t s) {
+                         float* y, hipStream_t s, const int* item_off, int item_mul, int64_t rows_total) {
     SC_CHECK(conv_to_mono_supported(cin, 1, k, 1, (k - 1) / 2, 1, act), "conv_to_mono: unsupported cin=%d k=%d act=%d", cin, k, act);
     if (nb <= 0 || T <= 0) return;
-    prof::Scope scope("conv_to_mono", 2.0 * nb * (double)T * cin * k, 4.0 * nb * (double)T * (cin + 1), s);
-    hipLaunchKernelGGL((conv_to_mono_kernel<16, 7>), dim3(cdiv(T, 256), nb), dim3(256), 0, s, x, w_packed, bias, in_slope, act, y, T);
+    const double rows = item_off ? (double)rows_total : nb * (double)T;
+    prof::Scope scope("conv_to_mono", 2.0 * rows * cin * k, 4.0 * rows * (cin + 1), s);
+    hipLaunchKernelGGL((conv_to_mono_kernel<16, 7>), dim3(cdiv(T, 256), nb), dim3(256), 0, s, x, w_packed, bias, in_slope, act, y, T, item_off,
+                       item_mul);
+    SC_LAUNCH_CHECK();
+}
+
+__global__ void item_row_pos_kernel(const int* __restrict__ item_off, int n_items, int mul, int rows, int2* __restrict__ row_pos) {
+    for (int r = blockIdx.x * blockDim.x + threadIdx.x; r < rows; r += gridDim.x * blockDim.x) {
+        const int n = item_search(n_items, r, [&](int i) { return item_off[i] * mul; });
+        row_pos[r] = make_int2(r - item_off[n] * mul, (item_off[n + 1] - item_off[n]) * mul);
+    }
+}
+void launch_item_row_pos(const int* item_off, int n_items, int mul, int rows, int2* row_pos, hipStream_t s) {
+    if (rows <= 0) return;
+    hipLaunchKernelGGL(item_row_pos_kernel, dim3(grid_for(rows)), dim3(256), 0, s, item_off, n_items, mul, rows, row_pos);
+    SC_LAUNCH_CHECK();
+}
+
+__global__ void scatter_items_kernel(const float* __restrict__ src, const int* __restrict__ item_off, const int* __restrict__ item_of, int mul,
+                                     int64_t dst_stride, float* __restrict__ dst) {
+    const int i = blockIdx.y;
+    const int len = (item_off[i + 1] - item_off[i]) * mul;
+    const float* __restrict__ s = src + (int64_t)item_off[i] * mul;
+    float* __restrict__ d = dst + (int64_t)item_of[i] * dst_stride;
+    for (int t = blockIdx.x * blockDim.x + threadIdx.x; t < len; t += gridDim.x * blockDim.x) d[t] = s[t];
+}
+void launch_scatter_items(const float* src, const int* item_off, const int* item_of, int n_items, int mul, int longest, int64_t dst_stride,
+                          float* dst, hipStream_t s) {
+    if (n_items <= 0 || longest <= 0) return;
+    hipLaunchKernelGGL(scatter_items_kernel, dim3(std::min(cdiv(longest, 256), 256), n_items), dim3(256), 0, s, src, item_off, item_of, mul,
+                       dst_stride, dst);
     SC_LAUNCH_CHECK();
 }
 
diff --git a/seamless_communication_amd/csrc/k_resblock.hip b/seamless_communication_amd/csrc/k_resblock.hip
--- a/seamless_communication_amd/csrc/k_resblock.hip
+++ b/seamless_communication_amd/csrc/k_resblock.hip
@@ -137,7 +137,8 @@
     constexpr int VPR = C / 4;
     extern __shared__ __attribute__((aligned(16))) unsigned char rb_smem[];
 
-    const int k = p.k, dil = p.dil, T = p.T;
+    const int k = p.k, dil = p.dil;
+    int T = p.T;
     const int H2 = (k - 1) / 2, H1 = dil * (k - 1) / 2;
     const int TT = RB_M1 - 2 * H2;
     const int R0 = RB_M1 + 2 * H1;
@@ -150,9 +151,20 @@
     const int ldb = (PER_TAP ? C : k * C) + 8;
 
     const int tid = threadIdx.x, lane = tid & 63, wave = tid >> 6;
-    const int n = blockIdx.x / tiles;
-    const int t0 = (blockIdx.x - n * tiles) * TT;
-    const float* __restrict__ xn = p.x + (int64_t)n * T * C;
+    int n, tile;
+    int64_t row0;
+    if (p.item_off) {
+        n = item_search(p.nb, (int)blockIdx.x, [&](int i) { return p.tile_first[i]; });
+        tile = blockIdx.x - p.tile_first[n];
+        row0 = (int64_t)p.item_off[n] * p.item_mul;
+        T = (p.item_off[n + 1] - p.item_off[n]) * p.item_mul;
+    } else {
+        n = blockIdx.x / tiles;
+        tile = blockIdx.x - n * tiles;
+        row0 = (int64_t)n * T;
+    }
+    const int t0 = tile * TT;
+    const float* __restrict__ xn = p.x + row0 * C;
     const float slope = p.slope;
 
     for (int i = tid; i < R0 * VPR; i += 256) {
@@ -247,7 +259,7 @@
             }
         }
         __syncthreads();
-        float* __restrict__ outn = p.out + (int64_t)n * T * C;
+        float* __restrict__ outn = p.out + row0 * C;
         for (int idx = tid; idx < TT * VPR; idx += 256) {
             const int i = idx / VPR, c4 = idx - i * VPR;
             const int t = t0 + i;
@@ -255,7 +267,7 @@
             const int64_t off = (int64_t)t * C + c4 * 4;
             f32x4_t v = *reinterpret_cast<const f32x4_t*>(ep + i * EPS + c4 * 4) + *reinterpret_cast<const f32x4_t*>(xn + off);
             if (p.avg_a) {
-                const int64_t g = (int64_t)n * T * C + off;
+                const int64_t g = row0 * C + off;
                 v = ((*reinterpret_cast<const f32x4_t*>(p.avg_a + g) + *reinterpret_cast<const f32x4_t*>(p.avg_b + g)) + v) / 3.0f;
             }
             *reinterpret_cast<f32x4_t*>(outn + off) = v;
@@ -336,12 +348,13 @@
 
 template <int C, bool EDGE, bool SINGLE>
 __device__ __forceinline__ void mrf_tile(const MrfArgs& p, _Float16* __restrict__ ph, _Float16* __restrict__ pl, _Float16* __restrict__ sW1,
-                                         _Float16* __restrict__ sW2, const float* __restrict__ sBias, int n, int t_first, int lane, int wave) {
+                                         _Float16* __restrict__ sW2, const float* __restrict__ sBias, int64_t row0, int T, int t_first, int lane,
+                                         int wave) {
     constexpr int CS = C + 8;
-    const int T = p.T, halo = p.halo;
+    const int halo = p.halo;
     const int TT = MRF_R - 2 * halo;
     const float slope = p.slope;
-    const float* __restrict__ xn = p.x + (int64_t)n * T * C;
+    const float* __restrict__ xn = p.x + row0 * C;
     const int col = lane & 31;
     const bool colok = col < C;
     const int jbase = 32 * wave + 4 * (lane >> 5);
@@ -450,7 +463,7 @@
     }
 
     if (colok) {
-        float* __restrict__ outb = p.out + (int64_t)n * T * C + (int64_t)(t_first + jbase) * C + col;
+        float* __restrict__ outb = p.out + row0 * C + (int64_t)(t_first + jbase) * C + col;
 #pragma unroll
         for (int r = 0; r < 16; ++r) {
             const int j = jbase + (r & 3) + 8 * (r >> 2);
@@ -478,8 +491,18 @@
 
     const int tid = threadIdx.x, lane = tid & 63;
     const int wave = __builtin_amdgcn_readfirstlane(tid >> 6);
-    const int n = blockIdx.x / tiles;
-    const int tile = blockIdx.x - n * tiles;
+    int n, tile, T = p.T;
+    int64_t row0;
+    if (p.item_off) {
+        n = item_search(p.nb, (int)blockIdx.x, [&](int i) { return p.tile_first[i]; });
+        tile = blockIdx.x - p.tile_first[n];
+        row0 = (int64_t)p.item_off[n] * p.item_mul;
+        T = (p.item_off[n + 1] - p.item_off[n]) * p.item_mul;
+    } else {
+        n = blockIdx.x / tiles;
+        tile = blockIdx.x - n * tiles;
+        row0 = (int64_t)n * T;
+    }
     const int t_first = tile * (MRF_R - 2 * p.halo) - p.halo;
 
     mrf_w_dma<C>(p.w1[0], p.ldw1[0], p.k[0], sW1, lane, wave);
@@ -500,8 +523,8 @@
     }
     asm volatile("s_waitcnt vmcnt(0)" ::: "memory");
     __syncthreads();
-    if (t_first < 0 || t_first + MRF_R > p.T) mrf_tile<C, true, SINGLE>(p, ph, pl, sW1, sW2, sBias, n, t_first, lane, wave);
-    else mrf_tile<C, false, SINGLE>(p, ph, pl, sW1, sW2, sBias, n, t_first, lane, wave);
+    if (t_first < 0 || t_first + MRF_R > T) mrf_tile<C, true, SINGLE>(p, ph, pl, sW1, sW2, sBias, row0, T, t_first, lane, wave);
+    else mrf_tile<C, false, SINGLE>(p, ph, pl, sW1, sW2, sBias, row0, T, t_first, lane, wave);
 }
 
 }
@@ -520,7 +543,7 @@
     }
     const int H2 = (a.k - 1) / 2, H1 = a.dil * (a.k - 1) / 2;
     const int TT = RB_M1 - 2 * H2;
-    const int tiles = cdiv(a.T, TT);
+    const int tiles = a.item_off ? 0 : cdiv(a.T, TT);
     const size_t act_halfs = SINGLE ? std::max<size_t>((size_t)(RB_M1 + 2 * H1) * (C + 8), (size_t)RB_M1 * (C + 4) * 2)
                                     : (size_t)2 * (RB_M1 + 2 * H1) * (C + 8);
     const size_t lds = act_halfs * sizeof(_Float16) + weights_lds_bytes(C, a.k);
@@ -530,7 +553,7 @@
     const double rows = (double)a.nb * a.T;
     prof::Scope scope(name, 2.0 * 2.0 * rows * C * (double)C * a.k,
                       4.0 * rows * C * (a.avg_a ? 4.0 : 2.0) + 2.0 * 2.0 * C * (double)C * a.k, s);
-    hipLaunchKernelGGL((resblock_pair_kernel<C, SINGLE>), dim3((unsigned)(a.nb * tiles)), dim3(256), lds, s, a, tiles);
+    hipLaunchKernelGGL((resblock_pair_kernel<C, SINGLE>), dim3((unsigned)(a.item_off ? a.total_tiles : a.nb * tiles)), dim3(256), lds, s, a, tiles);
 }
 
 }
@@ -542,7 +565,10 @@
     return RB_M1 - (k - 1) >= 32 && lds <= 120 * 1024;
 }
 
+int resblock_pair_tile_rows(int k) { return RB_M1 - 2 * ((k - 1) / 2); }
+
 void launch_resblock_pair(const ResPairArgs& a, hipStream_t s) {
+    SC_CHECK(!a.item_off || (a.tile_first && a.total_tiles > 0 && a.item_mul > 0), "resblock pair: packed items without a tile table");
     SC_CHECK(resblock_pair_supported(a.C, a.k, a.dil), "resblock pair: unsupported C=%d k=%d dil=%d", a.C, a.k, a.dil);
     SC_CHECK(a.nb > 0 && a.T > 0, "resblock pair: empty problem");
     SC_CHECK(a.ldw1 % 8 == 0 && a.ldw2 % 8 == 0 && a.ldw1 >= (int64_t)a.k * a.C && a.ldw2 >= (int64_t)a.k * a.C,
@@ -594,7 +620,7 @@
     }
     a.halo = mrf_halo(a);
     const int TT = MRF_R - 2 * a.halo;
-    const int tiles = cdiv(a.T, TT);
+    const int tiles = a.item_off ? 0 : cdiv(a.T, TT);
     SC_CHECK((int64_t)a.nb * tiles < (1ll << 31), "mrf: grid too large");
     char name[48];
     snprintf(name, sizeof(name), "mrf_fused_c%d", C);
@@ -605,11 +631,19 @@
         wbytes += 3.0 * 2.0 * 2.0 * C * (double)C * a.k[j];
     }
     prof::Scope scope(name, flops, 4.0 * rows * C * 2.0 + wbytes, s);
-    hipLaunchKernelGGL((mrf_fused_kernel<C, SINGLE>), dim3((unsigned)(a.nb * tiles)), dim3(MRF_THREADS), LDS, s, a, tiles);
-}
+    hipLaunchKernelGGL((mrf_fused_kernel<C, SINGLE>), dim3((unsigned)(a.item_off ? a.total_tiles : a.nb * tiles)), dim3(MRF_THREADS), LDS, s, a, tiles);
+}
+}
+
+int mrf_tile_rows(const int* k, const int* dil) {
+    MrfArgs a;
+    for (int j = 0; j < 3; ++j) a.k[j] = k[j];
+    for (int q = 0; q < 9; ++q) a.dil[q] = dil[q];
+    return MRF_R - 2 * mrf_halo(a);
 }
 
 void launch_mrf_fused(const MrfArgs& a, hipStream_t s) {
+    SC_CHECK(!a.item_off || (a.tile_first && a.total_tiles > 0 && a.item_mul > 0), "mrf: packed items without a tile table");
     SC_CHECK(mrf_fused_supported(a.C, a.k, a.dil), "mrf: unsupported C=%d k=(%d,%d,%d)", a.C, a.k[0], a.k[1], a.k[2]);
     SC_CHECK(a.nb > 0 && a.T > 0 && a.x && a.out && a.x != a.out, "mrf: empty problem or in-place call");
     for (int q = 0; q < 9; ++q) {
diff --git a/seamless_communication_amd/csrc/kernels.h b/seamless_communication_amd/csrc/kernels.h
--- a/seamless_communication_amd/csrc/kernels.h
+++ b/seamless_communication_amd/csrc/kernels.h
@@ -35,7 +35,44 @@
     int phases = 1;
     int split = 1;
     double algo_flops = 0;
-};
+    const int* item_off = nullptr;
+    int n_items = 0, item_mul = 1, item_extra = 0, item_out_mul = 1;
+};
+
+#if defined(__HIPCC__)
+template <typename F>
+__device__ __forceinline__ int item_search(int n, int key, F first) {
+    int lo = 0, hi = n - 1;
+    while (lo < hi) {
+        const int mid = (lo + hi + 1) >> 1;
+        if (first(mid) <= key) lo = mid;
+        else hi = mid - 1;
+    }
+    return lo;
+}
+
+struct GemmItemCursor {
+    int n = 0, start = 0, next = 0x7fffffff;
+    __device__ __forceinline__ static int first(const GemmArgs& p, int i) { return p.item_off[i] * p.item_mul + i * p.item_extra; }
+    __device__ __forceinline__ void init(const GemmArgs& p, int m) {
+        n = item_search(p.n_items, m, [&](int i) { return first(p, i); });
+        start = first(p, n);
+        next = first(p, n + 1);
+    }
+    __device__ __forceinline__ void seek(const GemmArgs& p, int m) {
+        while (m >= next) {
+            ++n;
+            start = next;
+            next = first(p, n + 1);
+        }
+    }
+    __device__ __forceinline__ int q(int m) const { return m - start; }
+    __device__ __forceinline__ int in_row0(const GemmArgs& p) const { return start - n * p.item_extra; }
+    __device__ __forceinline__ int t_in(const GemmArgs& p) const { return next - start - p.item_extra; }
+    __device__ __forceinline__ int t_out(const GemmArgs& p) const { return t_in(p) * p.item_out_mul; }
+    __device__ __forceinline__ int64_t out_row0(const GemmArgs& p) const { return (int64_t)in_row0(p) * p.item_out_mul; }
+};
+#endif
 
 void launch_gemm(const GemmArgs& a, hipStream_t s);
 extern std::atomic<int> g_force_general_gemm;
@@ -85,8 +122,12 @@
     const float* avg_a = nullptr;
     const float* avg_b = nullptr;
     int single = 0;
+    const int* item_off = nullptr;
+    const int* tile_first = nullptr;
+    int item_mul = 1, total_tiles = 0;
 };
 bool resblock_pair_supported(int C, int k, int dil);
+int resblock_pair_tile_rows(int k);
 void launch_resblock_pair(const ResPairArgs& a, hipStream_t s);
 
 struct MrfArgs {
@@ -104,8 +145,12 @@
     const float* b1[9] = {};
     const float* b2[9] = {};
     int single = 0;
+    const int* item_off = nullptr;
+    const int* tile_first = nullptr;
+    int item_mul = 1, total_tiles = 0;
 };
 bool mrf_fused_supported(int C, const int* k, const int* dil);
+int mrf_tile_rows(const int* k, const int* dil);
 void launch_mrf_fused(const MrfArgs& a, hipStream_t s);
 
 void launch_gemv(const float* x, int64_t ldx, const __half* W, int64_t ldw, const float* bias,
@@ -459,11 +504,16 @@
                       int min_dur, int* durations, hipStream_t s);
 void launch_vocoder_embed(const int* units, int nb, int T, const __half* dict, int E,
                           const __half* lang, int Lg, const int* lang_idx, const __half* spkr, int Sp,
-                          const int* spkr_idx, float* out , hipStream_t s);
+                          const int* spkr_idx, float* out , hipStream_t s,
+                          const int* item_off = nullptr , int rows_total = 0);
 void launch_avg3(const float* a, const float* b, const float* c, float* out, int64_t n, hipStream_t s);
 bool conv_to_mono_supported(int cin, int cout, int k, int stride, int pad, int dil, int act);
 void launch_conv_to_mono(const float* x, const __half* w_packed, const float* bias, int nb, int T, int cin, int k, float in_slope, int act,
-                         float* y, hipStream_t s);
+                         float* y, hipStream_t s, const int* item_off = nullptr ,
+                         int item_mul = 1, int64_t rows_total = 0);
+void launch_item_row_pos(const int* item_off, int n_items, int mul, int rows, int2* row_pos, hipStream_t s);
+void launch_scatter_items(const float* src, const int* item_off, const int* item_of, int n_items, int mul, int longest, int64_t dst_stride,
+                          float* dst, hipStream_t s);
 void launch_fill_i32(int* p, int v, int n, hipStream_t s);
 void launch_add_i32(int* p, int v, hipStream_t s);
 
diff --git a/seamless_communication_amd/csrc/model.h b/seamless_communication_amd/csrc/model.h
--- a/seamless_communication_amd/csrc/model.h
+++ b/seamless_communication_amd/csrc/model.h
@@ -1,4 +1,5 @@
 #pragma once
+#include <algorithm>
 #include <map>
 #include <functional>
 #include <memory>
@@ -238,6 +239,7 @@
     int last_n = 0, last_su = 0, last_sc = 0;
     int64_t last_padded_unit_rows = 0;
     int64_t last_vocoder_unit_rows = 0;
+    int last_vocoder_packed_groups = 0;
 
     std::unique_ptr<MmaState> mma;
 
@@ -330,8 +332,27 @@
 }
 void layernorm(Model& m, const float* x, const LNorm& L, float* y, int rows, int act = ACT_NONE,
                const int* lens = nullptr, int t_per_batch = 1);
+struct PackedItems {
+    std::vector<int> off;
+    const int* d_off = nullptr;
+    int n = 0;
+    std::vector<int> tabs;
+    const int* d_tabs = nullptr;
+    const int* d_tab(int idx) const { return d_tabs + (size_t)idx * (n + 1); }
+    int tab_total(int idx) const { return tabs[(size_t)idx * (n + 1) + n]; }
+    int rows() const { return off.empty() ? 0 : off.back(); }
+    int longest() const {
+        int l = 0;
+        for (int i = 0; i < n; ++i) l = std::max(l, off[i + 1] - off[i]);
+        return l;
+    }
+};
+std::vector<int> plan_packed_groups(const std::vector<int>& need, int64_t budget_rows);
+std::vector<int> packed_tile_first(const std::vector<int>& off, int mul, int tile_rows);
+
 void conv1d(Model& m, const float* x, const Conv& c, const float* res, float* y, int nb, int t_in, int stride, int pad,
-            int dil, const int* d_in_lens, int in_act, int act);
-void conv_transpose1d(Model& m, const float* x, const ConvT& c, float* y, int nb, int t_in, int in_act);
+            int dil, const int* d_in_lens, int in_act, int act, const PackedItems* pk = nullptr, int mul = 1);
+void conv_transpose1d(Model& m, const float* x, const ConvT& c, float* y, int nb, int t_in, int in_act, const PackedItems* pk = nullptr,
+                      int mul = 1);
 
 }
diff --git a/seamless_communication_amd/csrc/model_load.hip b/seamless_communication_amd/csrc/model_load.hip
--- a/seamless_communication_amd/csrc/model_load.hip
+++ b/seamless_communication_amd/csrc/model_load.hip
@@ -664,13 +664,20 @@
 }
 
 void conv1d(Model& m, const float* x, const Conv& c, const float* res, float* y, int nb, int t_in, int stride, int pad,
-            int dil, const int* d_in_lens, int in_act, int act) {
+            int dil, const int* d_in_lens, int in_act, int act, const PackedItems* pk, int mul) {
+    if (pk) {
+        SC_CHECK(stride == 1 && 2 * pad == dil * (c.k - 1) && !d_in_lens && mul >= 1 && (int64_t)pk->rows() * mul < (1ll << 31),
+                 "conv1d: packed items need stride 1 and 'same' padding");
+        nb = pk->n;
+        t_in = pk->longest() * mul;
+    }
     const int t_out = (t_in + 2 * pad - dil * (c.k - 1) - 1) / stride + 1;
     if (nb <= 0 || t_out <= 0) return;
     if (!res && !d_in_lens && g_force_general_gemm.load(std::memory_order_relaxed) == 0 &&
         conv_to_mono_supported(c.cin, c.cout, c.k, stride, pad, dil, act)) {
         const float slope = in_act == IN_LRELU_01 ? 0.1f : in_act == IN_LRELU_001 ? 0.01f : 1.0f;
-        launch_conv_to_mono(x, c.w, c.b, nb, t_in, c.cin, c.k, slope, act, y, m.stream);
+        launch_conv_to_mono(x, c.w, c.b, nb, t_in, c.cin, c.k, slope, act, y, m.stream, pk ? pk->d_off : nullptr, mul,
+                            pk ? (int64_t)pk->rows() * mul : 0);
         return;
     }
     GemmArgs a;
@@ -697,6 +704,12 @@
     a.in_lens = d_in_lens;
     a.in_act = in_act;
     a.act = act;
+    if (pk) {
+        a.M = pk->rows() * mul;
+        a.item_off = pk->d_off;
+        a.n_items = pk->n;
+        a.item_mul = mul;
+    }
     launch_gemm(a, m.stream);
 }
 
@@ -735,7 +748,12 @@
     launch_gemm_presplit(a, m.stream);
 }
 
-void conv_transpose1d(Model& m, const float* x, const ConvT& c, float* y, int nb, int t_in, int in_act) {
+void conv_transpose1d(Model& m, const float* x, const ConvT& c, float* y, int nb, int t_in, int in_act, const PackedItems* pk, int mul) {
+    if (pk) {
+        SC_CHECK(mul >= 1 && ((int64_t)pk->rows() * mul + pk->n) * c.stride < (1ll << 31), "conv_transpose1d: packed items too long");
+        nb = pk->n;
+        t_in = pk->longest() * mul;
+    }
     if (nb <= 0 || t_in <= 0) return;
     GemmArgs a;
     a.A = x;
@@ -763,6 +781,15 @@
     a.phases = c.stride;
     a.in_act = in_act;
     a.algo_flops = 2.0 * nb * (double)t_in * c.cin * c.cout * c.k;
+    if (pk) {
+        a.M = pk->rows() * mul + pk->n;
+        a.item_off = pk->d_off;
+        a.n_items = pk->n;
+        a.item_mul = mul;
+        a.item_extra = 1;
+        a.item_out_mul = c.stride;
+        a.algo_flops = 2.0 * pk->rows() * (double)mul * c.cin * c.cout * c.k;
+    }
     launch_gemm(a, m.stream);
 }
 
diff --git a/seamless_communication_amd/csrc/model_t2u.hip b/seamless_communication_amd/csrc/model_t2u.hip
--- a/seamless_communication_amd/csrc/model_t2u.hip
+++ b/seamless_communication_amd/csrc/model_t2u.hip
@@ -456,17 +456,21 @@
 
 namespace {
 
-void vocode_batch(Model& m, const int* d_units, const int* d_lang, const int* d_spkr, int n, int T, float* d_wav) {
+void vocode_batch(Model& m, const int* d_units, const int* d_lang, const int* d_spkr, int n, int T, float* d_wav,
+                  const PackedItems* pk = nullptr) {
     const sc_config& c = m.cfg;
     const int E = c.voc_embedding_dim, Lg = c.voc_lang_embedding_dim, Sp = c.voc_spkr_embedding_dim;
     int ch = c.voc_upsample_initial_channel;
     int t = T;
+    int rate = 1;
+    const size_t rows0 = pk ? (size_t)pk->rows() : (size_t)n * T;
     Buf<float> x;
     {
-        Buf<float> in(m.pp(), (size_t)n * T * (E + Lg + Sp));
-        launch_vocoder_embed(d_units, n, T, m.voc_dict, E, m.voc_lang, Lg, d_lang, m.voc_spkr, Sp, d_spkr, in, m.stream);
-        x = Buf<float>(m.pp(), (size_t)n * T * ch);
-        conv1d(m, in, m.voc_pre, nullptr, x, n, T, 1, 3, 1, nullptr, IN_NONE, ACT_NONE);
+        Buf<float> in(m.pp(), rows0 * (E + Lg + Sp));
+        launch_vocoder_embed(d_units, n, T, m.voc_dict, E, m.voc_lang, Lg, d_lang, m.voc_spkr, Sp, d_spkr, in, m.stream, pk ? pk->d_off : nullptr,
+                             (int)rows0);
+        x = Buf<float>(m.pp(), rows0 * ch);
+        conv1d(m, in, m.voc_pre, nullptr, x, n, T, 1, 3, 1, nullptr, IN_NONE, ACT_NONE, pk, 1);
     }
     const int nk = c.voc_num_resblock_kernels;
     SC_CHECK(nk == 3, "sc_vocode: %d resblock kernels (only 3 is implemented)", nk);
@@ -475,16 +479,21 @@
     for (int i = 0; i < c.voc_num_upsamples; ++i) {
         const ConvT& up = m.voc_ups[i];
         const int t2 = t * up.stride;
+        const int rate2 = rate * up.stride;
         ch = up.cout;
-        const size_t sz = (size_t)n * t2 * ch;
-        Buf<float> y(m.pp(), sz), tmp(m.pp(), sz), ra(m.pp(), sz), rb(m.pp(), sz);
-        Buf<float> rout[3] = {Buf<float>(m.pp(), sz), Buf<float>(m.pp(), sz), Buf<float>(m.pp(), sz)};
-        conv_transpose1d(m, x, up, y, n, t, IN_LRELU_01);
+        const size_t rows = rows0 * rate2;
+        const size_t sz = rows * ch;
+        Buf<float> y(m.pp(), sz), tmp, ra, rb, rout[3];
+        const auto need = [&](Buf<float>& b) -> float* {
+            if (!b.get()) b = Buf<float>(m.pp(), sz);
+            return b.get();
+        };
+        conv_transpose1d(m, x, up, y, n, t, IN_LRELU_01, pk, rate);
         bool fused_avg = false;
         x = Buf<float>(m.pp(), sz);
         static const bool voc_ps = knob::value("SC_VOC_PS", 1) != 0;
         bool wide_ps = voc_ps && g_force_general_gemm.load(std::memory_order_relaxed) == 0 && ch >= 128 && ch % 32 == 0 &&
-                       (int64_t)n * t2 * ch * 2 < (1ll << 31);
+                       (int64_t)sz * 2 < (1ll << 31);
         for (int j = 0; j < nk && wide_ps; ++j) {
             const ResBlock& r = m.voc_res[i * nk + j];
             for (size_t d = 0; d < r.dil.size(); ++d)
@@ -502,6 +511,13 @@
             __half* pt_l = one_plane ? nullptr : py_l + sz;
             __half* pn_l = one_plane ? nullptr : pt_l + sz;
             launch_lrelu_split_f32(y, 0.1f, py_h, py_l, (int64_t)sz, m.stream);
+            Buf<int2> row_pos;
+            if (pk) {
+                row_pos = Buf<int2>(m.pp(), rows);
+                launch_item_row_pos(pk->d_off, pk->n, rate2, (int)rows, row_pos.get(), m.stream);
+            }
+            for (int j = 0; j < nk; ++j) need(rout[j]);
+            need(ra), need(rb);
             for (int j = 0; j < nk; ++j) {
                 const ResBlock& r = m.voc_res[i * nk + j];
                 const float* cur = y;
@@ -513,9 +529,9 @@
                     float* dst = last ? rout[j].get() : ((d & 1) ? rb.get() : ra.get());
                     const int split = one_plane ? 0 : 1;
                     conv1d_presplit(m, ch_, cl_, r.convs1[d], nullptr, nullptr, pt_h, pt_l, n, t2, (k * r.dil[d] - r.dil[d]) / 2, r.dil[d], nullptr,
-                                    ACT_NONE, 0, nullptr, 0.1f, split);
+                                    ACT_NONE, (int)rows, row_pos.get(), 0.1f, split);
                     conv1d_presplit(m, pt_h, pt_l, r.convs2[d], cur, dst, last ? nullptr : pn_h, last ? nullptr : pn_l, n, t2, (k2 - 1) / 2, 1,
-                                    nullptr, ACT_NONE, 0, nullptr, 0.1f, split);
+                                    nullptr, ACT_NONE, (int)rows, row_pos.get(), 0.1f, split);
                     cur = dst;
                     ch_ = pn_h;
                     cl_ = pn_l;
@@ -523,6 +539,7 @@
             }
             launch_avg3(rout[0], rout[1], rout[2], x, (int64_t)sz, m.stream);
             t = t2;
+            rate = rate2;
             continue;
         }
         static const bool voc_mrf = knob::value("SC_VOC_MRF", 1) != 0;
@@ -546,12 +563,19 @@
                 a.x = y.get();
                 a.out = x.get();
                 a.nb = n;
-                a.T = t2;
+                a.T = pk ? (int)((rows + n - 1) / n) : t2;
                 a.C = ch;
                 a.slope = 0.1f;
                 a.single = (voc_single & 4) ? 1 : 0;
+                if (pk) {
+                    a.item_off = pk->d_off;
+                    a.item_mul = rate2;
+                    a.tile_first = pk->d_tab(4 * i + 3);
+                    a.total_tiles = pk->tab_total(4 * i + 3);
+                }
                 launch_mrf_fused(a, m.stream);
                 t = t2;
+                rate = rate2;
                 continue;
             }
         }
@@ -561,10 +585,12 @@
             const int nd = (int)r.dil.size();
             for (int d = 0; d < nd; ++d) {
                 const int k = r.convs1[d].k;
-                float* dst = (d == nd - 1) ? rout[j].get() : ((d & 1) ? rb.get() : ra.get());
                 const bool fuse = g_force_general_gemm.load(std::memory_order_relaxed) == 0 && r.convs2[d].k == k &&
                                   r.convs1[d].cin == ch && r.convs1[d].cout == ch && r.convs2[d].cin == ch &&
                                   r.convs2[d].cout == ch && resblock_pair_supported(ch, k, r.dil[d]);
+                SC_CHECK(fuse || !pk, "sc_vocode: packed items on a ResBlock shape the pair kernel does not take");
+                const bool avg_here = fuse && j == nk - 1 && d == nd - 1;
+                float* dst = avg_here ? x.get() : (d == nd - 1) ? need(rout[j]) : ((d & 1) ? need(rb) : need(ra));
                 if (fuse) {
                     ResPairArgs a;
                     a.x = cur;
@@ -575,22 +601,27 @@
                     a.ldw2 = r.convs2[d].kpad;
                     a.b2 = r.convs2[d].b;
                     a.nb = n;
-                    a.T = t2;
+                    a.T = pk ? (int)((rows + n - 1) / n) : t2;
                     a.C = ch;
                     a.k = k;
                     a.dil = r.dil[d];
                     a.slope = 0.1f;
                     a.single = (voc_single & 4) ? 1 : 0;
-                    if (j == nk - 1 && d == nd - 1) {
+                    if (pk) {
+                        a.item_off = pk->d_off;
+                        a.item_mul = rate2;
+                        a.tile_first = pk->d_tab(4 * i + j);
+                        a.total_tiles = pk->tab_total(4 * i + j);
+                    }
+                    if (avg_here) {
                         a.avg_a = rout[0];
                         a.avg_b = rout[1];
-                        dst = x.get();
                         fused_avg = true;
                     }
                     a.out = dst;
                     launch_resblock_pair(a, m.stream);
                 } else {
-                    conv1d(m, cur, r.convs1[d], nullptr, tmp, n, t2, 1, (k * r.dil[d] - r.dil[d]) / 2, r.dil[d], nullptr,
+                    conv1d(m, cur, r.convs1[d], nullptr, need(tmp), n, t2, 1, (k * r.dil[d] - r.dil[d]) / 2, r.dil[d], nullptr,
                            IN_LRELU_01, ACT_NONE);
                     conv1d(m, tmp, r.convs2[d], cur, dst, n, t2, 1, (k - 1) / 2, 1, nullptr, IN_LRELU_01, ACT_NONE);
                 }
@@ -599,8 +630,9 @@
         }
         if (!fused_avg) launch_avg3(rout[0], rout[1], rout[2], x, (int64_t)sz, m.stream);
         t = t2;
-    }
-    conv1d(m, x, m.voc_post, nullptr, d_wav, n, t, 1, 3, 1, nullptr, IN_LRELU_001, ACT_TANH);
+        rate = rate2;
+    }
+    conv1d(m, x, m.voc_post, nullptr, d_wav, n, t, 1, 3, 1, nullptr, IN_LRELU_001, ACT_TANH, pk, rate);
 }
 
 int vocoder_halo_units(const Model& m) {
@@ -623,6 +655,103 @@
     return (int)halo + 8;
 }
 
+int64_t vocoder_packed_row_cap(const Model& m, int hop) {
+    const sc_config& c = m.cfg;
+    const int nk = c.voc_num_resblock_kernels;
+    if (nk != 3) return 0;
+    static const bool voc_ps = knob::value("SC_VOC_PS", 1) != 0;
+    static const bool voc_mrf = knob::value("SC_VOC_MRF", 1) != 0;
+    int64_t per_row = (int64_t)hop * 4;
+    per_row = std::max<int64_t>(per_row, (int64_t)(c.voc_embedding_dim + c.voc_lang_embedding_dim + c.voc_spkr_embedding_dim) * 4);
+    int rate = 1;
+    for (int i = 0; i < c.voc_num_upsamples; ++i) {
+        const ConvT& up = m.voc_ups[i];
+        rate *= up.stride;
+        const int ch = up.cout;
+        per_row = std::max<int64_t>(per_row, (int64_t)(rate + 1) * std::max(ch, 2) * 4);
+        bool same = true, pairs = true;
+        for (int j = 0; j < nk; ++j) {
+            const ResBlock& r = m.voc_res[i * nk + j];
+            for (size_t d = 0; d < r.dil.size(); ++d) {
+                const Conv &c1 = r.convs1[d], &c2 = r.convs2[d];
+                same = same && c1.cin == ch && c1.cout == ch && c2.cin == ch && c2.cout == ch && (c1.k & 1) && (c2.k & 1);
+                pairs = pairs && c2.k == c1.k && resblock_pair_supported(ch, c1.k, r.dil[d]);
+            }
+        }
+        if (!same) return 0;
+        bool wide = voc_ps && ch >= 128 && ch % 32 == 0;
+        for (int j = 0; j < nk && wide; ++j) {
+            const ResBlock& r = m.voc_res[i * nk + j];
+            for (size_t d = 0; d < r.dil.size(); ++d) wide = wide && r.convs1[d].kpad == ch * r.convs1[d].k && r.convs2[d].kpad == ch * r.convs2[d].k;
+        }
+        if (wide) continue;
+        int k[3], dil[9];
+        bool mrf = voc_mrf;
+        for (int j = 0; j < nk && mrf; ++j) {
+            const ResBlock& r = m.voc_res[i * nk + j];
+            mrf = r.dil.size() == 3;
+            for (int d = 0; d < 3 && mrf; ++d) {
+                mrf = r.convs1[d].k == r.convs1[0].k && r.convs2[d].k == r.convs1[d].k;
+                dil[j * 3 + d] = r.dil[d];
+            }
+            if (mrf) k[j] = r.convs1[0].k;
+        }
+        if (mrf && mrf_fused_supported(ch, k, dil)) continue;
+        if (!pairs) return 0;
+    }
+    return ((1ll << 31) - 1) / per_row - c.voc_num_upsamples - 64;
+}
+
+void vocoder_tile_tables(const Model& m, PackedItems& pk) {
+    const sc_config& c = m.cfg;
+    const int nk = c.voc_num_resblock_kernels;
+    pk.tabs.assign((size_t)4 * c.voc_num_upsamples * (pk.n + 1), 0);
+    int rate = 1;
+    for (int i = 0; i < c.voc_num_upsamples; ++i) {
+        rate *= m.voc_ups[i].stride;
+        int k[3] = {1, 1, 1}, dil[9] = {1, 1, 1, 1, 1, 1, 1, 1, 1};
+        bool mrf = nk == 3;
+        for (int j = 0; j < nk && j < 3; ++j) {
+            const ResBlock& r = m.voc_res[i * nk + j];
+            if (r.convs1.empty()) continue;
+            k[j] = r.convs1[0].k;
+            mrf = mrf && r.dil.size() == 3;
+            for (size_t d = 0; d < r.dil.size() && d < 3; ++d) dil[j * 3 + d] = r.dil[d];
+            if ((k[j] & 1) == 0 || resblock_pair_tile_rows(k[j]) < 1) continue;
+            const std::vector<int> t = packed_tile_first(pk.off, rate, resblock_pair_tile_rows(k[j]));
+            std::copy(t.begin(), t.end(), pk.tabs.begin() + (size_t)(4 * i + j) * (pk.n + 1));
+        }
+        if (mrf && mrf_fused_supported(m.voc_ups[i].cout, k, dil)) {
+            const std::vector<int> t = packed_tile_first(pk.off, rate, mrf_tile_rows(k, dil));
+            std::copy(t.begin(), t.end(), pk.tabs.begin() + (size_t)(4 * i + 3) * (pk.n + 1));
+        }
+    }
+}
+
+}
+
+std::vector<int> plan_packed_groups(const std::vector<int>& need, int64_t budget_rows) {
+    std::vector<int> first;
+    int64_t rows = 0;
+    for (int i = 0; i < (int)need.size(); ++i) {
+        if (i == 0 || rows + need[i] > budget_rows) {
+            first.push_back(i);
+            rows = 0;
+        }
+        rows += need[i];
+    }
+    first.push_back((int)need.size());
+    return first;
+}
+
+std::vector<int> packed_tile_first(const std::vector<int>& off, int mul, int tile_rows) {
+    std::vector<int> first(off.size(), 0);
+    for (size_t i = 0; i + 1 < off.size(); ++i) {
+        const int64_t tiles = ((int64_t)(off[i + 1] - off[i]) * mul + tile_rows - 1) / tile_rows;
+        SC_CHECK(first[i] + tiles < (1ll << 31), "packed items: %lld tiles", (long long)(first[i] + tiles));
+        first[i + 1] = first[i] + (int)tiles;
+    }
+    return first;
 }
 
 __global__ void embed_rows_f16_kernel(const int* __restrict__ idx, const __half* __restrict__ table, int E, float* __restrict__ out) {
@@ -659,6 +788,7 @@
     const sc_config& c = m.cfg;
     SC_CHECK(c.has_vocoder, "sc_vocode: the model was loaded without a vocoder");
     prof::set_tag("voc");
+    m.last_vocoder_packed_groups = 0;
     SC_CHECK(n > 0 && T > 0, "sc_vocode: empty batch");
     for (int i = 0; i < n; ++i) {
         SC_CHECK(h_lang[i] >= 0 && h_lang[i] < c.voc_num_langs, "sc_vocode: lang index %d out of range", h_lang[i]);
@@ -685,6 +815,54 @@
     const int halo = vocoder_halo_units(m);
     std::vector<int> need(n);
     for (int i = 0; i < n; ++i) need[i] = std::min(T, h_unit_lens[i] + halo);
+    {
+        static const bool want_packed = knob::value("SC_VOC_PACKED", 1) != 0;
+        static const int pack_rows = std::max(1, knob::value("SC_VOC_PACK_ROWS", 49152));
+        const int64_t cap = vocoder_packed_row_cap(m, hop);
+        const int64_t budget = std::min<int64_t>(pack_rows, cap);
+        bool packed = want_packed && cap > 0 && g_force_general_gemm.load(std::memory_order_relaxed) == 0;
+        for (int i = 0; i < n && packed; ++i) packed = need[i] <= cap;
+        if (packed) {
+            SC_HIP(hipMemsetAsync(d_wav, 0, (size_t)n * T * hop * sizeof(float), m.stream));
+            const std::vector<int> first = plan_packed_groups(need, budget);
+            std::vector<std::vector<int32_t>> staging;
+            staging.reserve(first.size() - 1);
+            int64_t rows_done = 0;
+            for (size_t g = 0; g + 1 < first.size(); ++g) {
+                const int i0 = first[g], ng = first[g + 1] - first[g];
+                PackedItems pk;
+                pk.n = ng;
+                pk.off.assign(ng + 1, 0);
+                for (int gi = 0; gi < ng; ++gi) pk.off[gi + 1] = pk.off[gi] + need[i0 + gi];
+                const int R = pk.rows();
+                rows_done += R;
+                vocoder_tile_tables(m, pk);
+                const size_t n_tab = pk.tabs.size();
+                staging.emplace_back((size_t)(ng + 1) + n_tab + 3 * (size_t)ng + R);
+                std::vector<int32_t>& h = staging.back();
+                int32_t* w = h.data();
+                w = std::copy(pk.off.begin(), pk.off.end(), w);
+                w = std::copy(pk.tabs.begin(), pk.tabs.end(), w);
+                for (int gi = 0; gi < ng; ++gi) w[gi] = h_lang[i0 + gi], w[ng + gi] = h_spkr[i0 + gi], w[2 * ng + gi] = i0 + gi;
+                w += 3 * ng;
+                for (int gi = 0; gi < ng; ++gi) w = std::copy(h_units + (size_t)(i0 + gi) * T, h_units + (size_t)(i0 + gi) * T + need[i0 + gi], w);
+                Buf<int> d_all(m.pp(), h.size());
+                SC_HIP(hipMemcpyAsync(d_all.get(), h.data(), h.size() * 4, hipMemcpyHostToDevice, m.stream));
+                pk.d_off = d_all.get();
+                pk.d_tabs = pk.d_off + (ng + 1);
+                const int* d_lang = pk.d_tabs + n_tab;
+                const int* d_item = d_lang + 2 * ng;
+                const int* d_units = d_item + ng;
+                Buf<float> gw(m.pp(), (size_t)R * hop);
+                vocode_batch(m, d_units, d_lang, d_lang + ng, ng, pk.longest(), gw, &pk);
+                launch_scatter_items(gw, pk.d_off, d_item, ng, hop, pk.longest() * hop, (int64_t)T * hop, d_wav, m.stream);
+            }
+            m.last_vocoder_unit_rows = rows_done;
+            m.last_vocoder_packed_groups = (int)first.size() - 1;
+            SC_HIP(hipStreamSynchronize(m.stream));
+            return;
+        }
+    }
     static const int group_overhead = std::max(0, knob::value("SC_VOC_GROUP_OVERHEAD", 250));
     const std::vector<std::vector<int>> groups = plan_length_groups(need, group_overhead, max_groups);
     SC_HIP(hipMemsetAsync(d_wav, 0, (size_t)n * T * hop * sizeof(float), m.stream));
```
